# wildsonbbl/gnnepcsaft

Hardware: AMD Instinct MI355X
Metric: molecular graphs/sec (fwd+bwd) (higher is better)
Workload: dtype f32; 1 GPU; BASELINE configs[1]: PNA hidden=128 L=6 towers=1 pre=2 post=4, 4096 graphs/GPU (81920 atoms, 163840 directed bonds), fwd+loss+bwd incl. CSR packing; graphs_per_gpu=4096, parallelism=dp1, hip_graph=False, launch=auto, grad_allreduce_bytes=0, grad_exchange=none (1 rank)

## Files before the change

### gnnepcsaft_amd/_lib.py

```python
from __future__ import annotations

import ctypes as C
from pathlib import Path
from typing import Dict, Optional

import torch

_LIB_PATH = Path(__file__).resolve().parent / "libgnnepcsaft_hip.so"

ABI_VERSION = 7
GNX_OK, GNX_E_INVALID, GNX_E_HIP, GNX_E_RANGE, GNX_E_WORKSPACE = 0, -1, -2, -3, -4
OPT_GEMM_SPLIT, OPT_WGRAD_WGS, OPT_EMBED_BWD_MFMA, OPT_STD_BWD_CENTERED, OPT_GEMM_PIPE, OPT_WGRAD_PIPE, OPT_GEMM_AS, \
    OPT_GEMM_WS_FAST, OPT_GEMM_TILE_ROWS, OPT_GEMM_MID = range(10)
GEMM_RELU, GEMM_ACCUMULATE, GEMM_B_TRANS, GEMM_SPLIT_ONLY, GEMM_PRESPLIT = 1, 2, 4, 8, 16
POOL_ADD, POOL_MEAN, POOL_MAX = 0, 1, 2
K_NONE, K_PNA_AGG_FWD, K_PNA_AGG_BWD, K_GEMM_WS, K_GEMM_WGRAD, K_GINE_AGG_FWD, K_GINE_AGG_BWD, K_EDGE_COMBINE_FWD, \
    K_EDGE_COMBINE_BWD, K_BN_FWD, K_BN_BWD, K_GEMM_TILED, K_GEMM_SMALL, K_GEMM_WGRAD_BATCHED, K_KEY_SEGMENT_SUM, \
    K_EMBED, K_PNA_EDGE_FWD, K_PNA_EDGE_BWD, K_ATTN_FWD, K_ATTN_BWD, K_PCSAFT_RHO, K_PCSAFT_VP, \
    K_PCSAFT_MIX_STATE, K_PCSAFT_MIX_RHO = range(24)
K_COUNT = 24
KERNEL_GROUPS = {K_PNA_AGG_FWD: "pna_aggregate_fwd", K_PNA_AGG_BWD: "pna_aggregate_bwd", K_GEMM_WS: "gemm_weights_stationary",
                 K_GEMM_WGRAD: "weight_gradient", K_GINE_AGG_FWD: "gine_aggregate_fwd", K_GINE_AGG_BWD: "gine_aggregate_bwd",
                 K_EDGE_COMBINE_FWD: "edge_combine_fwd", K_EDGE_COMBINE_BWD: "edge_combine_bwd", K_BN_FWD: "batchnorm_fwd",
                 K_BN_BWD: "batchnorm_bwd", K_GEMM_TILED: "gemm_tiled", K_GEMM_SMALL: "gemm_small",
                 K_GEMM_WGRAD_BATCHED: "weight_gradient_batched", K_KEY_SEGMENT_SUM: "key_segment_sum", K_EMBED: "embedding",
                 K_PNA_EDGE_FWD: "pna_edge_fused_fwd", K_PNA_EDGE_BWD: "pna_edge_fused_bwd",
                 K_ATTN_FWD: "transformer_attn_fwd", K_ATTN_BWD: "transformer_attn_bwd",
                 K_PCSAFT_RHO: "pcsaft_density", K_PCSAFT_VP: "pcsaft_vapor_pressure",
                 K_PCSAFT_MIX_STATE: "pcsaft_mix_state", K_PCSAFT_MIX_RHO: "pcsaft_mix_density"}


class GnxError(RuntimeError):
    def __init__(self, status: int, msg: str):
        super().__init__(f"gnx status {status}: {msg}")
        self.status = status


class GemmSeg(C.Structure):
    _fields_ = [("a", C.c_void_p), ("lda", C.c_int64), ("rowscale", C.c_void_p), ("b", C.c_void_p),
                ("ldb", C.c_int64), ("k", C.c_int32), ("_pad", C.c_int32)]


class WgradProb(C.Structure):
    _fields_ = [("dC", C.c_void_p), ("lddc", C.c_int64), ("A", C.c_void_p), ("lda", C.c_int64),
                ("rowscale", C.c_void_p), ("dW", C.c_void_p), ("lddw", C.c_int64), ("dbias", C.c_void_p),
                ("M", C.c_int64), ("N", C.c_int32), ("K", C.c_int32)]


_vp, _i32, _i64, _f32, _sz = C.c_void_p, C.c_int32, C.c_int64, C.c_float, C.c_size_t

PNA_MAX_LAYERS, PNA_MAX_TOWERS = 8, 8
PNA_BWD_DEFER_SMALL, PNA_BWD_LAST_OF_PASS = 1, 2


class PnaFwdArgs(C.Structure):
    _fields_ = [("N", _i64), ("E", _i64), ("T", _i32), ("F", _i32), ("pre_layers", _i32), ("post_layers", _i32),
                ("D", _i32), ("merged", _i32),
                ("rowptr", _vp), ("src", _vp), ("dst", _vp), ("code", _vp), ("dperm", _vp), ("tiles", _vp), ("ntiles", _vp),
                ("max_tiles", _i64), ("x", _vp), ("Te", _vp), ("weff", _vp * PNA_MAX_TOWERS), ("Wm", _vp), ("bm", _vp),
                ("params", C.POINTER(_vp)), ("P", _vp), ("Q", _vp), ("A", _vp), ("hs", _vp * PNA_MAX_LAYERS),
                ("zs", _vp * PNA_MAX_LAYERS), ("ws", _vp), ("ws_bytes", _sz), ("out", _vp), ("etile_info", _vp),
                ("etile_w", _i32), ("tile_rows", _i32)]


class PnaBwdArgs(C.Structure):
    _fields_ = [("N", _i64), ("E", _i64), ("T", _i32), ("F", _i32), ("pre_layers", _i32), ("post_layers", _i32),
                ("R", _i32), ("D", _i32), ("avg_deg_log", _f32), ("merged", _i32), ("acc_first", _i32),
                ("use_side_streams", _i32), ("n_h", _i32), ("n_z", _i32),
                ("rowptr", _vp), ("colptr", _vp), ("cpos", _vp), ("code", _vp), ("code_pos", _vp), ("dperm", _vp),
                ("tiles", _vp), ("ntiles", _vp), ("chunks", _vp), ("nchunks", _vp),
                ("max_tiles", _i64), ("max_chunks", _i64),
                ("x", _vp), ("BE", _vp), ("EE", _vp), ("A", _vp),
                ("hs", _vp * PNA_MAX_LAYERS), ("zs", _vp * PNA_MAX_LAYERS), ("weff", _vp * PNA_MAX_TOWERS), ("Wm", _vp),
                ("params", C.POINTER(_vp)), ("grads", C.POINTER(_vp)), ("dout", _vp),
                ("gbuf", _vp * PNA_MAX_LAYERS), ("dA", _vp), ("gebuf", _vp * PNA_MAX_LAYERS), ("dP", _vp), ("dQ", _vp),
                ("dTe", _vp), ("dEE", _vp), ("dWm", _vp), ("dbm", _vp), ("dWeff", _vp), ("ws", _vp), ("ws_bytes", _sz),
                ("acc_buf", _vp), ("dx", _vp), ("flags", _i32), ("etile_w", _i32), ("etile_info", _vp)]


class PnaFinishArgs(C.Structure):
    _fields_ = [("L", _i32), ("T", _i32), ("F", _i32), ("pre_layers", _i32), ("post_layers", _i32), ("R", _i32), ("D", _i32),
                ("merged", _i32), ("use_side_streams", _i32), ("_pad", _i32),
                ("BE", _vp), ("acc_buf", _vp), ("ones", _vp), ("avg_deg_log", C.POINTER(_f32)),
                ("params", C.POINTER(_vp)), ("grads", C.POINTER(_vp)), ("EE", C.POINTER(_vp)), ("dTe", C.POINTER(_vp)),
                ("dEE", C.POINTER(_vp)), ("dWm", C.POINTER(_vp)), ("dbm", C.POINTER(_vp)), ("dWeff", C.POINTER(_vp))]


class SmallProb(C.Structure):
    _fields_ = [("A", _vp), ("lda", _i64), ("B", _vp), ("ldb", _i64), ("bias", _vp), ("C", _vp), ("ldc", _i64),
                ("M", _i32), ("N", _i32), ("K", _i32), ("flags", _i32)]


SB_A_TRANS, SB_B_TRANS, SB_ACCUMULATE, SB_ATOMIC, SB_RELU = 1, 2, 4, 8, 16

SIGNATURES = {
    "gnx_create": (_i32, [C.POINTER(_vp), _i32]),
    "gnx_destroy": (_i32, [_vp]),
    "gnx_set_stream": (_i32, [_vp, _vp]),
    "gnx_last_error": (C.c_char_p, []),
    "gnx_abi_version": (_i32, []),
    "gnx_set_option": (_i32, [_vp, _i32, _i32]),
    "gnx_get_option": (_i32, [_vp, _i32, C.POINTER(_i32)]),
    "gnx_prof_begin": (_i32, [_vp, C.c_uint32]),
    "gnx_prof_read": (_i32, [_vp, _i32, C.POINTER(_i64), C.POINTER(C.c_double), C.POINTER(C.c_double),
                             C.POINTER(C.c_double), C.POINTER(C.c_double)]),
    "gnx_prof_end": (_i32, [_vp]),
    "gnx_pack_csr_workspace_bytes": (_sz, [_i64, _i64]),
    "gnx_pack_csr": (_i32, [_vp, _vp, _i64, _i64, _vp, _vp, _vp, _vp, _vp, _vp, _vp, _sz]),
    "gnx_feature_code": (_i32, [_vp, _vp, _i64, _i32, C.POINTER(_i32), _vp, _vp, _vp, _sz]),
    "gnx_graph_ptr": (_i32, [_vp, _vp, _i64, _i64, _vp, _vp, _sz]),
    "gnx_degree_scalers": (_i32, [_vp, _vp, _i64, _f32, _vp, _vp]),
    "gnx_embed_sum_fwd": (_i32, [_vp, _vp, _i64, _i32, C.POINTER(_i32), _vp, _i32, _vp]),
    "gnx_table_scatter_workspace_bytes": (_sz, [_i64, _i32, _i32]),
    "gnx_embed_sum_bwd": (_i32, [_vp, _vp, _i64, _i32, C.POINTER(_i32), _i32, _vp, _i32, _vp, _vp, _sz]),
    "gnx_check_range": (_i32, [_vp]),
    "gnx_collate_ptr": (_i32, [_vp, _vp, _vp, _i64, _vp, _i64, _vp, _vp]),
    "gnx_collate_gather": (_i32, [_vp, _vp, _vp, _i64, _vp, _vp, _vp, _i64, _vp, _i64, _vp, _vp, _i64, _i64, _vp, _vp,
                                  _vp, _vp]),
    "gnx_collate_rows": (_i32, [_vp, _vp, _i64, _vp, _i64, _i32, _i32, _vp]),
    "gnx_gemm_workspace_bytes": (_sz, [_vp, _i32, C.POINTER(GemmSeg), C.POINTER(_i64), _i32, _i64, _i32, _vp, _i32,
                                       _i32]),
    "gnx_gemm": (_i32, [_vp, _i32, C.POINTER(GemmSeg), _i64, _i32, _vp, _vp, _i64, _vp, _i64, _i32, _vp, _sz]),
    "gnx_gemm_wgrad": (_i32, [_vp, _vp, _i64, _vp, _i64, _vp, _i64, _i32, _i32, _vp, _i64, _vp]),
    "gnx_gemm_wgrad_batched": (_i32, [_vp, _i32, C.POINTER(WgradProb)]),
    "gnx_degree_max": (_i32, [_vp, _vp, _i64, C.POINTER(_i32)]),
    "gnx_degree_classes_workspace_bytes": (_sz, [_i64, _i32]),
    "gnx_degree_classes": (_i32, [_vp, _vp, _i64, _i32, _vp, _vp, _vp, _sz]),
    "gnx_class_tiles": (_i32, [_vp, _vp, _i32, _i32, _vp, _vp]),
    "gnx_gemm_grouped": (_i32, [_vp, _i32, C.POINTER(GemmSeg), C.POINTER(_i64), _i32, _i64, _i32, _vp, _vp, _i64, _vp,
                                _i64, _i32, _vp, _vp, _vp, _i64, _vp, _sz]),
    "gnx_gemm_tile_rows": (_i32, [_vp, _i64, _i32]),
    "gnx_gemm_grouped_rows": (_i32, [_vp, _i32, C.POINTER(GemmSeg), C.POINTER(_i64), _i32, _i64, _i32, _vp, _vp, _i64, _vp,
                                     _i64, _i32, _vp, _vp, _vp, _i64, _vp, _sz, _i32]),
    "gnx_gemm_wgrad_grouped": (_i32, [_vp, _vp, _i64, _vp, _i64, _i64, _i32, _i32, _vp, _i64, _i64, _vp, _vp, _vp,
                                      _i64]),
    "gnx_pna_weff": (_i32, [_vp, _vp, _i64, _i32, _i32, _f32, _vp]),
    "gnx_pna_weff_bwd": (_i32, [_vp, _vp, _i32, _i32, _f32, _vp, _i64]),
    "gnx_group_by_small_key": (_i32, [_vp, _vp, _i64, _i32, _vp, _vp, _vp, _sz]),
    "gnx_key_segment_sum": (_i32, [_vp, _vp, _vp, _vp, _i64, _i32, _vp]),
    "gnx_edge_combine_fwd": (_i32, [_vp, _vp, _vp, _vp, _vp, _vp, _vp, _i64, _i32, _i32, _vp]),
    "gnx_edge_combine_bwd": (_i32, [_vp, _vp, _vp, _vp, _vp, _vp, _i64, _i64, _i32, _i32, _vp, _vp, _vp, _vp, _sz]),
    "gnx_pna_aggregate_fwd": (_i32, [_vp, _vp, _vp, _i64, _i64, _i32, _i32, _vp]),
    "gnx_pna_aggregate_bwd": (_i32, [_vp, _vp, _vp, _vp, _vp, _i64, _i64, _i32, _i32, _vp]),
    "gnx_edge_tiles_count": (_i32, [_i64, _i32]),
    "gnx_edge_tiles": (_i32, [_vp, _vp, _i64, _i64, _i32, _vp]),
    "gnx_pna_edge_fwd": (_i32, [_vp, _vp, _vp, _vp, _vp, _vp, _vp, _vp, _vp, _i32, _i64, _i64, _i32, _i32, C.POINTER(_vp),
                                C.POINTER(_vp), _vp, _vp, _vp]),
    "gnx_pna_edge_bwd": (_i32, [_vp, _vp, _vp, _vp, _vp, _vp, _i32, _i64, _i64, _i32, _i32, _i32, C.POINTER(_vp), _vp, _vp,
                                _vp]),
    "gnx_gine_aggregate_fwd": (_i32, [_vp, _vp, _vp, _vp, _vp, _vp, _i64, _i64, _i32, _f32, _vp]),
    "gnx_gine_aggregate_bwd": (_i32, [_vp, _vp, _vp, _vp, _vp, _vp, _vp, _vp, _vp, _vp, _i64, _i64, _i32, _i32, _f32,
                                      _vp, _vp]),
    "gnx_gine_dle": (_i32, [_vp, _vp, _vp, _vp, _vp, _vp, _vp, _vp, _i64, _i32, _i32, _vp]),
    "gnx_transformer_attn_fwd": (_i32, [_vp, _vp, _vp, _vp, _vp, _vp, _i64, _i64, _i32, _i32, _f32, C.c_uint64,
                                        C.c_uint64, _vp, _vp, _vp]),
    "gnx_transformer_attn_bwd": (_i32, [_vp, _vp, _vp, _vp, _vp, _vp, _vp, _vp, _vp, _vp, _vp, _vp, _i64, _i64, _i32,
                                        _i32, _i32, _f32, C.c_uint64, C.c_uint64, _vp, _vp, _vp]),
    "gnx_transformer_attn_dle": (_i32, [_vp, _vp, _vp, _vp, _vp, _vp, _vp, _i64, _i32, _i32, _i32, _vp]),
    "gnx_pcsaft_density": (_i32, [_vp, _vp, _i64, _vp, _vp, _vp, _i64, _vp, _vp]),
    "gnx_pcsaft_vapor_pressure": (_i32, [_vp, _vp, _i64, _vp, _vp, _i64, _vp, _vp, _vp, _vp]),
    "gnx_pcsaft_mix_state": (_i32, [_vp, _vp, _i64, _vp, _vp, _vp, _i64, _i32, _vp, _vp, _vp, _vp, _i64, _vp, _vp, _vp,
                                    _vp]),
    "gnx_pcsaft_mix_density": (_i32, [_vp, _vp, _i64, _vp, _vp, _vp, _i64, _i32, _vp, _vp, _vp, _vp, _i64, _vp, _vp]),
    "gnx_segment_pool_fwd": (_i32, [_vp, _vp, _vp, _i64, _i32, _i32, _vp]),
    "gnx_segment_pool_bwd": (_i32, [_vp, _vp, _vp, _vp, _vp, _i64, _i32, _i32, _vp]),
    "gnx_batchnorm_workspace_bytes": (_sz, [_i64, _i32]),
    "gnx_batchnorm_fwd": (_i32, [_vp, _vp, _i64, _i32, _vp, _vp, _vp, _vp, _vp, _f32, _f32, _i32, _i32, _vp, _vp, _vp,
                                 _vp, _sz]),
    "gnx_batchnorm_bwd": (_i32, [_vp, _vp, _vp, _vp, _i64, _i32, _vp, _vp, _vp, _i32, _vp, _vp, _vp, _vp, _sz]),
    "gnx_dropout": (_i32, [_vp, _vp, _i64, _f32, C.c_uint64, C.c_uint64, _vp]),
    "gnx_huber_ape": (_i32, [_vp, _vp, _vp, _i64, _f32, _vp, _vp]),
    "gnx_adamw_amsgrad": (_i32, [_vp, _vp, _vp, _vp, _vp, _vp, _i64, _f32, _f32, _f32, _f32, _f32, _i64]),
    "gnx_sgd": (_i32, [_vp, _vp, _vp, _i64, _f32]),
    "gnx_pna_weight_only": (_i32, [_vp, _vp, _i32, _i32, _i32, _i32, _i32, _i32, _f32, C.POINTER(_vp), _i32, _vp, _vp,
                                   C.POINTER(_vp), _vp, _vp]),
    "gnx_pna_conv_fwd": (_i32, [_vp, C.POINTER(PnaFwdArgs)]),
    "gnx_pna_weight_only_all": (_i32, [_vp, _i32, _vp, _i32, _i32, _i32, _i32, _i32, _i32, C.POINTER(_f32), C.POINTER(_vp),
                                       _i32, C.POINTER(_vp), C.POINTER(_vp), C.POINTER(_vp), C.POINTER(_vp), C.POINTER(_vp)]),
    "gnx_pna_stack_finish": (_i32, [_vp, C.POINTER(PnaFinishArgs)]),
    "gnx_gemm_small_batched": (_i32, [_vp, _i32, C.POINTER(SmallProb)]),
    "gnx_pna_weff_batched": (_i32, [_vp, _i32, C.POINTER(_vp), _i64, _i32, _i32, C.POINTER(_f32), C.POINTER(_vp)]),
    "gnx_pna_weff_bwd_batched": (_i32, [_vp, _i32, C.POINTER(_vp), _i32, _i32, C.POINTER(_f32), C.POINTER(_vp), _i64]),
    "gnx_pna_conv_bwd_workspace_bytes": (_sz, [_i32, _i32, _i32]),
    "gnx_pna_conv_bwd": (_i32, [_vp, C.POINTER(PnaBwdArgs)]),
    "gnx_fill": (_i32, [_vp, _vp, _i64, _f32]),
    "gnx_scale": (_i32, [_vp, _vp, _i64, _f32]),
    "gnx_axpy": (_i32, [_vp, _vp, _vp, _i64, _f32]),
    "gnx_side_stream": (_i32, [_vp, C.POINTER(_vp)]),
    "gnx_side_begin": (_i32, [_vp]),
    "gnx_side_end": (_i32, [_vp]),
    "gnx_side_join": (_i32, [_vp]),
    "gnx_side_stream_n": (_i32, [_vp, _i32, C.POINTER(_vp)]),
    "gnx_side_begin_n": (_i32, [_vp, _i32]),
    "gnx_side_join_n": (_i32, [_vp, _i32]),
    "gnx_clip_rows": (_i32, [_vp, _vp, _i64, _i32, _vp, _vp, _vp]),
}

_lib: Optional[C.CDLL] = None
_handles: Dict[int, int] = {}


def lib_path() -> Path:
    return _LIB_PATH


def load() -> C.CDLL:
    global _lib
    if _lib is not None:
        return _lib
    if not _LIB_PATH.exists():
        raise ImportError(f"{_LIB_PATH} is missing: build it with `python -m gnnepcsaft_amd.build` "
                          "(hipcc --offload-arch=gfx950). There is no CPU fallback.")
    lib = C.CDLL(str(_LIB_PATH))
    for name, (res, args) in SIGNATURES.items():
        fn = getattr(lib, name)
        fn.restype = res
        fn.argtypes = args
    if lib.gnx_abi_version() != ABI_VERSION:
        raise ImportError(f"ABI version mismatch: library {lib.gnx_abi_version()} != binding {ABI_VERSION}")
    _lib = lib
    return lib


def last_error() -> str:
    return load().gnx_last_error().decode(errors="replace")


def check(status: int) -> None:
    if status != GNX_OK:
        raise GnxError(status, last_error())


_bound_stream: dict = {}
try:
    _raw_stream = torch._C._cuda_getCurrentRawStream
except AttributeError:
    def _raw_stream(idx: int) -> int:
        return torch.cuda.current_stream(idx).cuda_stream


def handle(device: torch.device) -> int:
    if device.type != "cuda":
        raise GnxError(GNX_E_INVALID, f"gnnepcsaft_amd kernels need a HIP device tensor, got {device}; there is no CPU "
                                      "fallback")
    idx = device.index if device.index is not None else torch.cuda.current_device()
    lib = load()
    h = _handles.get(idx)
    if h is None:
        out = _vp()
        check(lib.gnx_create(C.byref(out), idx))
        h = out.value
        _handles[idx] = h
    stream = _raw_stream(idx)
    if _bound_stream.get(idx) != stream:
        check(lib.gnx_set_stream(h, stream))
        _bound_stream[idx] = stream
    return h
```

### gnnepcsaft_amd/csrc/gnx_pack.hip

```cpp
#include "gnx_common.hpp"

#define SCAN_ITEMS 4
#define SCAN_BLOCK 256
#define SCAN_TILE (SCAN_ITEMS * SCAN_BLOCK)

__global__ void __launch_bounds__(SCAN_BLOCK) k_scan_tile(const int* __restrict__ in, int* __restrict__ out,
                                                          int* __restrict__ sums, int64_t n) {
  __shared__ int s[SCAN_BLOCK];
  int64_t base = (int64_t)blockIdx.x * SCAN_TILE + (int64_t)threadIdx.x * SCAN_ITEMS;
  int v[SCAN_ITEMS];
  int t = 0;
#pragma unroll
  for (int i = 0; i < SCAN_ITEMS; ++i) {
    v[i] = (base + i < n) ? in[base + i] : 0;
    t += v[i];
  }
  s[threadIdx.x] = t;
  __syncthreads();
  for (int off = 1; off < SCAN_BLOCK; off <<= 1) {
    int add = (threadIdx.x >= off) ? s[threadIdx.x - off] : 0;
    __syncthreads();
    s[threadIdx.x] += add;
    __syncthreads();
  }
  int excl = s[threadIdx.x] - t;
#pragma unroll
  for (int i = 0; i < SCAN_ITEMS; ++i) {
    if (base + i < n) out[base + i] = excl;
    excl += v[i];
  }
  if (threadIdx.x == SCAN_BLOCK - 1) sums[blockIdx.x] = s[SCAN_BLOCK - 1];
}

__global__ void k_scan_add(int* __restrict__ out, const int* __restrict__ offs, int64_t n) {
  int64_t i = (int64_t)blockIdx.x * SCAN_TILE + threadIdx.x;
  int o = offs[blockIdx.x];
  for (int k = 0; k < SCAN_ITEMS; ++k, i += SCAN_BLOCK)
    if (i < n) out[i] += o;
}

__global__ void k_set_total(int* __restrict__ out, const int* __restrict__ in, int64_t n) {
  if (threadIdx.x == 0 && blockIdx.x == 0) out[n] = (n > 0) ? out[n - 1] + in[n - 1] : 0;
}

static int32_t exclusive_scan(gnx_handle* h, const int* in, int* out, int64_t n, int* ws, bool write_total) {
  if (n > 0) {
    int64_t blocks = gnx_cdiv(n, SCAN_TILE);
    hipLaunchKernelGGL(k_scan_tile, dim3((unsigned)blocks), dim3(SCAN_BLOCK), 0, h->stream, in, out, ws, n);
    GNX_LAUNCH_CHECK();
    if (blocks > 1) {
      int* sums_scanned = ws + blocks + 1;
      int32_t st = exclusive_scan(h, ws, sums_scanned, blocks, sums_scanned + blocks + 1, false);
      if (st != GNX_OK) return st;
      hipLaunchKernelGGL(k_scan_add, dim3((unsigned)blocks), dim3(SCAN_BLOCK), 0, h->stream, out, sums_scanned, n);
      GNX_LAUNCH_CHECK();
    }
  }
  if (write_total) {
    hipLaunchKernelGGL(k_set_total, dim3(1), dim3(64), 0, h->stream, out, in, n);
    GNX_LAUNCH_CHECK();
  }
  return GNX_OK;
}

static size_t scan_ws_ints_total(int64_t n) {
  size_t tot = 0;
  int64_t m = n;
  while (m > 1) {
    int64_t b = gnx_cdiv(m, SCAN_TILE);
    tot += 2 * ((size_t)b + 1);
    m = b;
  }
  return tot + 16;
}

__global__ void k_convert_edges(const int64_t* __restrict__ ei, int64_t E, int64_t N, int* __restrict__ src0,
                                int* __restrict__ dst0, int* __restrict__ flag) {
  int64_t e = (int64_t)blockIdx.x * blockDim.x + threadIdx.x;
  if (e >= E) return;
  int64_t s = ei[e], d = ei[E + e];
  bool bad = (s < 0) | (s >= N) | (d < 0) | (d >= N);
  if (bad) {
    atomicOr(flag, 1);
    s = 0;
    d = 0;
  }
  src0[e] = (int)s;
  dst0[e] = (int)d;
}

__global__ void k_count_keys(const int* __restrict__ key, int64_t E, int* __restrict__ counts) {
  int64_t e = (int64_t)blockIdx.x * blockDim.x + threadIdx.x;
  if (e < E) atomicAdd(&counts[key[e]], 1);
}

__global__ void k_fill_groups(const int* __restrict__ key, int64_t E, const int* __restrict__ ptr,
                              int* __restrict__ cursor, int* __restrict__ items) {
  int64_t e = (int64_t)blockIdx.x * blockDim.x + threadIdx.x;
  if (e >= E) return;
  int k = key[e];
  int pos = ptr[k] + atomicAdd(&cursor[k], 1);
  items[pos] = (int)e;
}

__global__ void k_sort_groups(const int* __restrict__ ptr, int64_t N, int* __restrict__ items) {
  int64_t i = (int64_t)blockIdx.x * blockDim.x + threadIdx.x;
  if (i >= N) return;
  int b = ptr[i], e = ptr[i + 1];
  for (int a = b + 1; a < e; ++a) {
    int v = items[a];
    int c = a - 1;
    while (c >= b && items[c] > v) {
      items[c + 1] = items[c];
      --c;
    }
    items[c + 1] = v;
  }
}

__global__ void k_gather_endpoints(const int* __restrict__ perm, const int* __restrict__ src0,
                                   const int* __restrict__ dst0, int64_t E, int* __restrict__ src,
                                   int* __restrict__ dst) {
  int64_t p = (int64_t)blockIdx.x * blockDim.x + threadIdx.x;
  if (p >= E) return;
  int e = perm[p];
  src[p] = src0[e];
  dst[p] = dst0[e];
}

static int32_t group_by_key(gnx_handle* h, const int* key, int64_t E, int64_t N, int* ptr, int* items, int* cursor,
                            int* scan_ws) {
  gnx_zero_ints(h, cursor, N > 0 ? N : 1);
  if (E > 0) {
    hipLaunchKernelGGL(k_count_keys, dim3((unsigned)gnx_cdiv(E, 256)), dim3(256), 0, h->stream, key, E, cursor);
    GNX_LAUNCH_CHECK();
  }
  int32_t st = exclusive_scan(h, cursor, ptr, N, scan_ws, true);
  if (st != GNX_OK) return st;
  gnx_zero_ints(h, cursor, N > 0 ? N : 1);
  if (E > 0) {
    hipLaunchKernelGGL(k_fill_groups, dim3((unsigned)gnx_cdiv(E, 256)), dim3(256), 0, h->stream, key, E, ptr, cursor,
                       items);
    GNX_LAUNCH_CHECK();
    hipLaunchKernelGGL(k_sort_groups, dim3((unsigned)gnx_cdiv(N, 256)), dim3(256), 0, h->stream, ptr, N, items);
    GNX_LAUNCH_CHECK();
  }
  return GNX_OK;
}

extern "C" size_t gnx_pack_csr_workspace_bytes(int64_t N, int64_t E) {
  if (N < 0) N = 0;
  if (E < 0) E = 0;
  size_t ints = 2 * (size_t)E + (size_t)N + 1 + scan_ws_ints_total(N) + 64;
  return ints * sizeof(int);
}

extern "C" int32_t gnx_pack_csr(gnx_handle* h, const int64_t* edge_index, int64_t E, int64_t N, int32_t* rowptr,
                                int32_t* perm, int32_t* src, int32_t* dst, int32_t* colptr, int32_t* cpos, void* ws,
                                size_t ws_bytes) {
  GNX_CHECK_ARG(h != nullptr, "gnx_pack_csr: handle is NULL");
  GNX_CHECK_ARG(N >= 0 && E >= 0 && N < (1ll << 31) - 1 && E < (1ll << 31) - 1, "gnx_pack_csr: N=%lld E=%lld out of int32 range",
                (long long)N, (long long)E);
  GNX_CHECK_ARG(rowptr && colptr, "gnx_pack_csr: rowptr/colptr NULL");
  GNX_CHECK_ARG(E == 0 || (edge_index && perm && src && dst && cpos), "gnx_pack_csr: NULL edge array with E>0");
  if (ws_bytes < gnx_pack_csr_workspace_bytes(N, E) || (!ws && ws_bytes)) {
    gnx_set_error("gnx_pack_csr: workspace %zu < %zu", ws_bytes, gnx_pack_csr_workspace_bytes(N, E));
    return GNX_E_WORKSPACE;
  }
  GNX_CHECK_ARG(ws != nullptr, "gnx_pack_csr: workspace is NULL");
  int* w = reinterpret_cast<int*>(ws);
  int* src0 = w;
  int* dst0 = src0 + E;
  int* cursor = dst0 + E;
  int* scan_ws = cursor + N + 1;
  if (E > 0) {
    hipLaunchKernelGGL(k_convert_edges, dim3((unsigned)gnx_cdiv(E, 256)), dim3(256), 0, h->stream, edge_index, E, N,
                       src0, dst0, h->d_flag);
    GNX_LAUNCH_CHECK();
  }
  int32_t st = group_by_key(h, dst0, E, N, rowptr, perm, cursor, scan_ws);
  if (st != GNX_OK) return st;
  if (E > 0) {
    hipLaunchKernelGGL(k_gather_endpoints, dim3((unsigned)gnx_cdiv(E, 256)), dim3(256), 0, h->stream, perm, src0,
                       dst0, E, src, dst);
    GNX_LAUNCH_CHECK();
  }
  return group_by_key(h, src, E, N, colptr, cpos, cursor, scan_ws);
}

struct dims_t {
  int d[16];
};

__global__ void k_feature_code(const int64_t* __restrict__ feat, int64_t rows, int K, dims_t dims,
                               const int* __restrict__ perm, int* __restrict__ code, int* __restrict__ flag) {
  int64_t p = (int64_t)blockIdx.x * blockDim.x + threadIdx.x;
  if (p >= rows) return;
  int64_t r = perm ? perm[p] : p;
  int c = 0;
  bool bad = false;
  for (int k = 0; k < K; ++k) {
    int64_t f = feat[r * K + k];
    if (f < 0 || f >= dims.d[k]) {
      bad = true;
      f = 0;
    }
    c = c * dims.d[k] + (int)f;
  }
  if (bad) atomicOr(flag, 2);
  code[p] = c;
}

extern "C" int32_t gnx_feature_code(gnx_handle* h, const int64_t* feat, int64_t rows, int32_t K, const int32_t* dims,
                                    const int32_t* perm, int32_t* code, void* ws, size_t ws_bytes) {
  (void)ws;
  (void)ws_bytes;
  GNX_CHECK_ARG(h && dims && K > 0 && K <= 16 && rows >= 0, "gnx_feature_code: bad argument");
  GNX_CHECK_ARG(rows == 0 || (feat && code), "gnx_feature_code: NULL array with rows>0");
  dims_t d;
  int64_t prod = 1;
  for (int k = 0; k < 16; ++k) d.d[k] = (k < K) ? dims[k] : 1;
  for (int k = 0; k < K; ++k) {
    GNX_CHECK_ARG(dims[k] > 0, "gnx_feature_code: dims[%d] <= 0", k);
    prod *= dims[k];
  }
  GNX_CHECK_ARG(prod < (1ll << 31), "gnx_feature_code: code space overflows int32");
  if (rows > 0) {
    hipLaunchKernelGGL(k_feature_code, dim3((unsigned)gnx_cdiv(rows, 256)), dim3(256), 0, h->stream, feat, rows, (int)K,
                       d, perm, code, h->d_flag);
    GNX_LAUNCH_CHECK();
  }
  return GNX_OK;
}

__global__ void k_graph_ptr(const int64_t* __restrict__ batch, int64_t N, int64_t B, int* __restrict__ ptr,
                            int* __restrict__ flag) {
  int64_t n = (int64_t)blockIdx.x * blockDim.x + threadIdx.x;
  if (n > N) return;
  int64_t prev = (n == 0) ? -1 : batch[n - 1];
  int64_t cur = (n == N) ? B : batch[n];
  if (n < N && (cur < 0 || cur >= B)) {
    atomicOr(flag, 4);
    return;
  }
  if (cur < prev) {
    atomicOr(flag, 8);
    return;
  }
  for (int64_t g = prev + 1; g <= cur; ++g) ptr[g] = (int)n;
}

extern "C" int32_t gnx_graph_ptr(gnx_handle* h, const int64_t* batch, int64_t N, int64_t B, int32_t* graph_ptr,
                                 void* ws, size_t ws_bytes) {
  (void)ws;
  (void)ws_bytes;
  GNX_CHECK_ARG(h && graph_ptr && N >= 0 && B >= 0 && (batch || N == 0), "gnx_graph_ptr: bad argument");
  hipLaunchKernelGGL(k_graph_ptr, dim3((unsigned)gnx_cdiv(N + 1, 256)), dim3(256), 0, h->stream, batch, N, B,
                     graph_ptr, h->d_flag);
  GNX_LAUNCH_CHECK();
  return GNX_OK;
}

__global__ void k_degree_scalers(const int* __restrict__ rowptr, int64_t N, float avg_log, float* __restrict__ amp,
                                 float* __restrict__ att) {
  int64_t n = (int64_t)blockIdx.x * blockDim.x + threadIdx.x;
  if (n >= N) return;
  float d = (float)(rowptr[n + 1] - rowptr[n]);
  amp[n] = logf(d + 1.0f) / avg_log;
  att[n] = avg_log / logf(fmaxf(d, 1.0f) + 1.0f);
}

extern "C" int32_t gnx_degree_scalers(gnx_handle* h, const int32_t* rowptr, int64_t N, float avg_deg_log, float* amp,
                                      float* att) {
  GNX_CHECK_ARG(h && N >= 0 && (N == 0 || (rowptr && amp && att)), "gnx_degree_scalers: bad argument");
  if (N == 0) return GNX_OK;
  hipLaunchKernelGGL(k_degree_scalers, dim3((unsigned)gnx_cdiv(N, 256)), dim3(256), 0, h->stream, rowptr, N,
                     avg_deg_log, amp, att);
  GNX_LAUNCH_CHECK();
  return GNX_OK;
}

struct weff_batch_args {
  const float* W[GNX_SMALL_BATCH];
  float* out[GNX_SMALL_BATCH];
  float avg_log[GNX_SMALL_BATCH];
  int64_t ldw;
  int F, D;
};

__global__ void k_pna_weff_batched(weff_batch_args a) {
  const int b = blockIdx.y;
  const int F = a.F;
  int64_t i = (int64_t)blockIdx.x * blockDim.x + threadIdx.x;
  int64_t per = (int64_t)F * 4 * F;
  if (i >= per * a.D) return;
  int d = (int)(i / per);
  int o = (int)((i % per) / (4 * F)), j = (int)(i % (4 * F));
  float dd = (float)d;
  float amp = logf(dd + 1.0f) / a.avg_log[b];
  float att = a.avg_log[b] / logf(fmaxf(dd, 1.0f) + 1.0f);
  const float* w = a.W[b] + (int64_t)o * a.ldw;
  a.out[b][i] = w[F + j] + amp * w[5 * F + j] + att * w[9 * F + j];
}

struct weff_bwd_batch_args {
  const float* dWeff[GNX_SMALL_BATCH];
  float* dW[GNX_SMALL_BATCH];
  float avg_log[GNX_SMALL_BATCH];
  int64_t lddw;
  int F, D;
};

__global__ void k_pna_weff_bwd_batched(weff_bwd_batch_args a) {
  const int b = blockIdx.y;
  const int F = a.F;
  int64_t i = (int64_t)blockIdx.x * blockDim.x + threadIdx.x;
  int64_t per = (int64_t)F * 4 * F;
  if (i >= per) return;
  int o = (int)(i / (4 * F)), j = (int)(i % (4 * F));
  float s1 = 0.f, s2 = 0.f, s3 = 0.f;
  const float avg_log = a.avg_log[b];
  const float* dWeff = a.dWeff[b];
  for (int d = 0; d < a.D; ++d) {
    float dd = (float)d;
    float amp = logf(dd + 1.0f) / avg_log;
    float att = avg_log / logf(fmaxf(dd, 1.0f) + 1.0f);
    float v = dWeff[(int64_t)d * per + i];
    s1 += v;
    s2 += amp * v;
    s3 += att * v;
  }
  float* w = a.dW[b] + (int64_t)o * a.lddw;
  w[F + j] += s1;
  w[5 * F + j] += s2;
  w[9 * F + j] += s3;
}

extern "C" int32_t gnx_pna_weff_bwd_batched(gnx_handle* h, int32_t n, const float* const* dWeff, int32_t F, int32_t D,
                                            const float* avg_deg_log, float* const* dW, int64_t lddw) {
  GNX_CHECK_ARG(h && dWeff && dW && avg_deg_log && n >= 0 && F > 0 && D > 0 && lddw >= 13 * F,
                "gnx_pna_weff_bwd_batched: bad argument");
  const int64_t cnt = (int64_t)F * 4 * F;
  for (int32_t i0 = 0; i0 < n; i0 += GNX_SMALL_BATCH) {
    weff_bwd_batch_args a;
    const int m = n - i0 < GNX_SMALL_BATCH ? n - i0 : GNX_SMALL_BATCH;
    for (int i = 0; i < GNX_SMALL_BATCH; ++i) {
      const int k = i < m ? i0 + i : i0;
      a.dWeff[i] = dWeff[k];
      a.dW[i] = dW[k];
      a.avg_log[i] = avg_deg_log[k];
      GNX_CHECK_ARG(a.dWeff[i] && a.dW[i], "gnx_pna_weff_bwd_batched: NULL pointer at %d", k);
    }
    a.lddw = lddw;
    a.F = F;
    a.D = D;
    hipLaunchKernelGGL(k_pna_weff_bwd_batched, dim3((unsigned)gnx_cdiv(cnt, 256), (unsigned)m), dim3(256), 0, h->stream, a);
    GNX_LAUNCH_CHECK();
  }
  return GNX_OK;
}

extern "C" int32_t gnx_pna_weff_batched(gnx_handle* h, int32_t n, const float* const* W, int64_t ldw, int32_t F, int32_t D,
                                        const float* avg_deg_log, float* const* Weff) {
  GNX_CHECK_ARG(h && W && Weff && avg_deg_log && n >= 0 && F > 0 && D > 0 && ldw >= 13 * F, "gnx_pna_weff_batched: bad argument");
  const int64_t cnt = (int64_t)F * 4 * F * D;
  for (int32_t i0 = 0; i0 < n; i0 += GNX_SMALL_BATCH) {
    weff_batch_args a;
    const int m = n - i0 < GNX_SMALL_BATCH ? n - i0 : GNX_SMALL_BATCH;
    for (int i = 0; i < GNX_SMALL_BATCH; ++i) {
      const int k = i < m ? i0 + i : i0;
      a.W[i] = W[k];
      a.out[i] = Weff[k];
      a.avg_log[i] = avg_deg_log[k];
      GNX_CHECK_ARG(a.W[i] && a.out[i], "gnx_pna_weff_batched: NULL pointer at %d", k);
    }
    a.ldw = ldw;
    a.F = F;
    a.D = D;
    hipLaunchKernelGGL(k_pna_weff_batched, dim3((unsigned)gnx_cdiv(cnt, 256), (unsigned)m), dim3(256), 0, h->stream, a);
    GNX_LAUNCH_CHECK();
  }
  return GNX_OK;
}

extern "C" int32_t gnx_pna_weff(gnx_handle* h, const float* W, int64_t ldw, int32_t F, int32_t D, float avg_deg_log,
                                float* Weff) {
  GNX_CHECK_ARG(h && W && Weff && F > 0 && D > 0 && ldw >= 13 * F, "gnx_pna_weff: bad argument");
  return gnx_pna_weff_batched(h, 1, &W, ldw, F, D, &avg_deg_log, &Weff);
}

extern "C" int32_t gnx_pna_weff_bwd(gnx_handle* h, const float* dWeff, int32_t F, int32_t D, float avg_deg_log,
                                    float* dW, int64_t lddw) {
  GNX_CHECK_ARG(h && dWeff && dW && F > 0 && D > 0 && lddw >= 13 * F, "gnx_pna_weff_bwd: bad argument");
  return gnx_pna_weff_bwd_batched(h, 1, &dWeff, F, D, &avg_deg_log, &dW, lddw);
}

__global__ void k_degree_max(const int* __restrict__ rowptr, int64_t N, int* __restrict__ out) {
  int64_t n = (int64_t)blockIdx.x * blockDim.x + threadIdx.x;
  int d = (n < N) ? rowptr[n + 1] - rowptr[n] : 0;
  for (int off = 32; off > 0; off >>= 1) d = max(d, __shfl_xor(d, off));
  if ((threadIdx.x & 63) == 0) atomicMax(out, d);
}

extern "C" int32_t gnx_degree_max(gnx_handle* h, const int32_t* rowptr, int64_t N, int32_t* max_degree_host) {
  GNX_CHECK_ARG(h && max_degree_host && N >= 0 && (N == 0 || rowptr), "gnx_degree_max: bad argument");
  int* d_out = h->d_flag + 8;
  gnx_zero_ints(h, d_out, 1);
  if (N > 0) {
    hipLaunchKernelGGL(k_degree_max, dim3((unsigned)gnx_cdiv(N, 256)), dim3(256), 0, h->stream, rowptr, N, d_out);
    GNX_LAUNCH_CHECK();
  }
  int v = 0;
  GNX_HIP(hipMemcpyAsync(&v, d_out, sizeof(int), hipMemcpyDeviceToHost, h->stream));
  GNX_HIP(hipStreamSynchronize(h->stream));
  *max_degree_host = v;
  return GNX_OK;
}

#define DC_BLOCK 256
#define DC_MAX_CLASSES 64

__global__ void __launch_bounds__(DC_BLOCK) k_dc_hist(const int* __restrict__ rowptr, const int* __restrict__ keys,
                                                       int64_t N, int D, int nblocks, int* __restrict__ blockhist,
                                                       int* __restrict__ flag) {
  __shared__ int hist[DC_MAX_CLASSES];
  if (threadIdx.x < DC_MAX_CLASSES) hist[threadIdx.x] = 0;
  __syncthreads();
  int64_t n = (int64_t)blockIdx.x * DC_BLOCK + threadIdx.x;
  if (n < N) {
    int d = keys ? keys[n] : rowptr[n + 1] - rowptr[n];
    if (d < 0) d = 0;
    if (d >= D) {
      atomicOr(flag, 32);
      d = D - 1;
    }
    atomicAdd(&hist[d], 1);
  }
  __syncthreads();
  if (threadIdx.x < D) blockhist[threadIdx.x * nblocks + blockIdx.x] = hist[threadIdx.x];
}

__global__ void __launch_bounds__(DC_BLOCK) k_dc_fill(const int* __restrict__ rowptr, const int* __restrict__ keys,
                                                       int64_t N, int D, int nblocks,
                                                       const int* __restrict__ blockoff, int* __restrict__ dperm,
                                                       int* __restrict__ cls_ptr) {
  __shared__ int degs[DC_BLOCK];
  int64_t n = (int64_t)blockIdx.x * DC_BLOCK + threadIdx.x;
  int d = -1;
  if (n < N) {
    d = keys ? keys[n] : rowptr[n + 1] - rowptr[n];
    if (d < 0) d = 0;
    if (d >= D) d = D - 1;
  }
  degs[threadIdx.x] = d;
  __syncthreads();
  if (n < N) {
    int rank = 0;
    for (int t = 0; t < (int)threadIdx.x; ++t) rank += (degs[t] == d) ? 1 : 0;
    dperm[blockoff[d * nblocks + blockIdx.x] + rank] = (int)n;
  }
  if (blockIdx.x == 0 && (int)threadIdx.x <= D)
    cls_ptr[threadIdx.x] = ((int)threadIdx.x == D) ? (int)N : blockoff[threadIdx.x * nblocks];
}

extern "C" size_t gnx_degree_classes_workspace_bytes(int64_t N, int32_t D) {
  if (N < 0) N = 0;
  int64_t nblocks = gnx_cdiv(N > 0 ? N : 1, DC_BLOCK);
  size_t ints = 2 * (size_t)(D * nblocks + 1) + scan_ws_ints_total(D * nblocks) + 64;
  return ints * sizeof(int);
}

extern "C" int32_t gnx_degree_classes(gnx_handle* h, const int32_t* rowptr, int64_t N, int32_t D, int32_t* dperm,
                                      int32_t* cls_ptr, void* ws, size_t ws_bytes) {
  GNX_CHECK_ARG(h && rowptr && cls_ptr && N >= 0 && D >= 1 && D <= DC_MAX_CLASSES && (N == 0 || dperm),
                "gnx_degree_classes: bad argument (D must be in [1,%d])", DC_MAX_CLASSES);
  if (ws_bytes < gnx_degree_classes_workspace_bytes(N, D) || !ws) {
    gnx_set_error("gnx_degree_classes: workspace %zu < %zu", ws_bytes, gnx_degree_classes_workspace_bytes(N, D));
    return GNX_E_WORKSPACE;
  }
  int nblocks = (int)gnx_cdiv(N > 0 ? N : 1, DC_BLOCK);
  int* blockhist = reinterpret_cast<int*>(ws);
  int* blockoff = blockhist + (size_t)D * nblocks + 1;
  int* scan_ws = blockoff + (size_t)D * nblocks + 1;
  hipLaunchKernelGGL(k_dc_hist, dim3(nblocks), dim3(DC_BLOCK), 0, h->stream, rowptr, (const int*)nullptr, N, (int)D,
                     nblocks, blockhist, h->d_flag);
  GNX_LAUNCH_CHECK();
  int32_t st = exclusive_scan(h, blockhist, blockoff, (int64_t)D * nblocks, scan_ws, false);
  if (st != GNX_OK) return st;
  hipLaunchKernelGGL(k_dc_fill, dim3(nblocks), dim3(DC_BLOCK), 0, h->stream, rowptr, (const int*)nullptr, N, (int)D,
                     nblocks, blockoff, dperm, cls_ptr);
  GNX_LAUNCH_CHECK();
  return GNX_OK;
}

extern "C" int32_t gnx_group_by_small_key(gnx_handle* h, const int32_t* keys, int64_t E, int32_t R, int32_t* pos,
                                          int32_t* ptr, void* ws, size_t ws_bytes) {
  GNX_CHECK_ARG(h && ptr && E >= 0 && R >= 1 && R <= DC_MAX_CLASSES && (E == 0 || (keys && pos)),
                "gnx_group_by_small_key: bad argument (R must be in [1,%d])", DC_MAX_CLASSES);
  if (ws_bytes < gnx_degree_classes_workspace_bytes(E, R) || !ws) {
    gnx_set_error("gnx_group_by_small_key: workspace %zu < %zu", ws_bytes, gnx_degree_classes_workspace_bytes(E, R));
    return GNX_E_WORKSPACE;
  }
  int nblocks = (int)gnx_cdiv(E > 0 ? E : 1, DC_BLOCK);
  int* blockhist = reinterpret_cast<int*>(ws);
  int* blockoff = blockhist + (size_t)R * nblocks + 1;
  int* scan_ws = blockoff + (size_t)R * nblocks + 1;
  hipLaunchKernelGGL(k_dc_hist, dim3(nblocks), dim3(DC_BLOCK), 0, h->stream, (const int*)nullptr, keys, E, (int)R,
                     nblocks, blockhist, h->d_flag);
  GNX_LAUNCH_CHECK();
  int32_t st = exclusive_scan(h, blockhist, blockoff, (int64_t)R * nblocks, scan_ws, false);
  if (st != GNX_OK) return st;
  hipLaunchKernelGGL(k_dc_fill, dim3(nblocks), dim3(DC_BLOCK), 0, h->stream, (const int*)nullptr, keys, E, (int)R,
                     nblocks, blockoff, pos, ptr);
  GNX_LAUNCH_CHECK();
  return GNX_OK;
}

__global__ void __launch_bounds__(256) k_class_tiles(const int* __restrict__ cls_ptr, int D, int tile_rows,
                                                     int* __restrict__ tile_info, int* __restrict__ ntiles) {
  int total = 0;
  for (int c = 0; c < D; ++c) total += (cls_ptr[c + 1] - cls_ptr[c] + tile_rows - 1) / tile_rows;
  if (blockIdx.x == 0 && threadIdx.x == 0) ntiles[0] = total;
  for (int t = blockIdx.x * blockDim.x + threadIdx.x; t < total; t += gridDim.x * blockDim.x) {
    int first = 0, c = 0;
    for (; c < D; ++c) {
      const int nt = (cls_ptr[c + 1] - cls_ptr[c] + tile_rows - 1) / tile_rows;
      if (t < first + nt) break;
      first += nt;
    }
    const int r = cls_ptr[c] + (t - first) * tile_rows;
    const int rows = cls_ptr[c + 1] - r;
    tile_info[3 * t + 0] = r;
    tile_info[3 * t + 1] = rows < tile_rows ? rows : tile_rows;
    tile_info[3 * t + 2] = c;
  }
}

extern "C" int32_t gnx_class_tiles(gnx_handle* h, const int32_t* cls_ptr, int32_t D, int32_t tile_rows,
                                   int32_t* tile_info, int32_t* ntiles) {
  GNX_CHECK_ARG(h && cls_ptr && tile_info && ntiles && D >= 1 && tile_rows > 0, "gnx_class_tiles: bad argument");
  hipLaunchKernelGGL(k_class_tiles, dim3(16), dim3(256), 0, h->stream, cls_ptr, (int)D, (int)tile_rows, tile_info, ntiles);
  GNX_LAUNCH_CHECK();
  return GNX_OK;
}
```

### gnnepcsaft_amd/functional.py

```python
from __future__ import annotations

from typing import Optional, Sequence

import torch

from . import ops
from .ops import GraphPack


_GRAD_IN_PLACE = False
_USE_DEGREE_CLASSES = True
_NATIVE_LAYER_BWD = True
_FUSED_EDGE = True
_BATCH_WEIGHT_ONLY = True


def set_grad_in_place(enabled: bool) -> None:
    global _GRAD_IN_PLACE
    _GRAD_IN_PLACE = bool(enabled)


def grad_in_place_enabled() -> bool:
    return _GRAD_IN_PLACE


def set_degree_classes(enabled: bool) -> None:
    global _USE_DEGREE_CLASSES
    _USE_DEGREE_CLASSES = bool(enabled)


def degree_classes_enabled() -> bool:
    return _USE_DEGREE_CLASSES


def set_native_layer_backward(enabled: bool) -> None:
    global _NATIVE_LAYER_BWD
    _NATIVE_LAYER_BWD = bool(enabled)


def set_fused_edge(enabled: bool) -> None:
    global _FUSED_EDGE
    _FUSED_EDGE = bool(enabled)


def set_batch_weight_only(enabled: bool) -> None:
    global _BATCH_WEIGHT_ONLY
    _BATCH_WEIGHT_ONLY = bool(enabled)


def batch_weight_only_enabled() -> bool:
    return _BATCH_WEIGHT_ONLY


def grad_sinks(params: Sequence[torch.Tensor]) -> tuple:
    if not _GRAD_IN_PLACE:
        return tuple(None for _ in params)
    out = []
    for p in params:
        g = p.grad
        ok = g is not None and g.dtype == torch.float32 and g.is_contiguous() and g.shape == p.shape and \
            g.device == p.device
        out.append(g if ok else None)
    return tuple(out)


def _tower_slices(T: int, F: int):
    return [None] if T == 1 else [slice(t * F, (t + 1) * F) for t in range(T)]


def _cols(t: torch.Tensor, sl_t):
    return t if sl_t is None else t[:, sl_t]


def _empty(rows: int, cols: int, like: torch.Tensor) -> torch.Tensor:
    return torch.empty(rows, cols, dtype=torch.float32, device=like.device)


def _zeros_like(t: torch.Tensor) -> torch.Tensor:
    return ops.zeros(*t.shape, device=t.device)


def adjacent_rows(tensors: Sequence[torch.Tensor]) -> Optional[torch.Tensor]:
    t0 = tensors[0]
    if t0.dim() != 2 or t0.dtype is not torch.float32 or not t0.is_contiguous():
        return None
    H = t0.size(1)
    ptr, rows = t0.data_ptr(), 0
    for t in tensors:
        if t.dim() != 2 or t.size(1) != H or t.dtype is not torch.float32 or not t.is_contiguous() or \
                t.device != t0.device or t.data_ptr() != ptr + rows * H * 4:
            return None
        rows += t.size(0)
    if t0.untyped_storage().nbytes() - t0.storage_offset() * 4 < rows * H * 4:
        return None
    return torch.as_strided(t0.detach(), (rows, H), (H, 1))


class EmbedSumFn(torch.autograd.Function):

    @staticmethod
    def forward(ctx, idx, offsets, *weights):
        table = adjacent_rows(weights)
        if table is None:
            table = torch.cat([w.detach() for w in weights], dim=0)
        ctx.save_for_backward(idx)
        ctx.offsets = tuple(offsets)
        ctx.sinks = grad_sinks(weights)
        return ops.embed_sum_fwd(idx, table, offsets)

    @staticmethod
    def backward(ctx, dout):
        (idx,) = ctx.saved_tensors
        sinks, offs = ctx.sinks, ctx.offsets
        if all(g is not None for g in sinks):
            gtable = adjacent_rows(sinks)
            if gtable is not None:
                ops.embed_sum_bwd(idx, offs, dout.contiguous(), out=gtable)
                return (None, None) + (None,) * len(sinks)
        dtable = ops.embed_sum_bwd(idx, offs, dout.contiguous())
        return (None, None) + tuple(dtable[offs[k]:offs[k + 1]] for k in range(len(sinks)))


class DropoutFn(torch.autograd.Function):

    @staticmethod
    def forward(ctx, x, p, seed, offset):
        ctx.key = (float(p), int(seed), int(offset))
        return ops.dropout(x, p, seed, offset)

    @staticmethod
    def backward(ctx, dy):
        p, seed, offset = ctx.key
        return ops.dropout(dy, p, seed, offset), None, None, None


class LinearFn(torch.autograd.Function):

    @staticmethod
    def forward(ctx, x, weight, bias):
        x = x.contiguous()
        ctx.save_for_backward(x, weight)
        ctx.has_bias = bias is not None
        ctx.sinks = grad_sinks([weight] + ([bias] if bias is not None else []))
        y = _empty(x.size(0), weight.size(0), x)
        return ops.gemm([(x, None, weight)], y, bias=bias)

    @staticmethod
    def backward(ctx, dy):
        x, weight = ctx.saved_tensors
        dy = dy.contiguous()
        sw = ctx.sinks[0]
        sb = ctx.sinks[1] if ctx.has_bias else None
        dw = sw if sw is not None else _zeros_like(weight)
        db = None
        if ctx.has_bias:
            db = sb if sb is not None else ops.zeros(weight.size(0), device=dy.device)
        ops.gemm_wgrad(dy, x, dw, dbias=db)
        dx = None
        if ctx.needs_input_grad[0]:
            dx = ops.gemm([(dy, None, weight)], _empty(x.size(0), x.size(1), x), b_trans=False)
        ops.finish_backward(dy.device, sw is not None and (sb is not None or not ctx.has_bias), ctx.sinks)
        return dx, (None if sw is not None else dw), (None if (sb is not None or not ctx.has_bias) else db)


class BatchNormFn(torch.autograd.Function):

    @staticmethod
    def forward(ctx, x, gamma, beta, running_mean, running_var, momentum, eps, training, relu, nbt=None):
        x = x.contiguous()
        y, mean, rstd = ops.batchnorm_fwd(x, gamma, beta, running_mean, running_var, momentum, eps, training, relu,
                                          num_batches_tracked=nbt)
        ctx.save_for_backward(x, y, gamma, mean, rstd)
        ctx.relu, ctx.training = relu, training
        ctx.sinks = grad_sinks([gamma, beta])
        return y

    @staticmethod
    def backward(ctx, dy):
        x, y, gamma, mean, rstd = ctx.saved_tensors
        if not ctx.training:
            raise NotImplementedError("BatchNorm backward in eval mode is not on the reference's training path")
        sg, sb = ctx.sinks
        dx, dgamma, dbeta = ops.batchnorm_bwd(dy.contiguous(), x, y, gamma, mean, rstd, ctx.relu, dgamma=sg, dbeta=sb)
        return dx, (None if sg is not None else dgamma), (None if sb is not None else dbeta), None, None, None, None, \
            None, None, None


class SegmentPoolFn(torch.autograd.Function):

    @staticmethod
    def forward(ctx, x, ptr, B, mode):
        x = x.contiguous()
        out = ops.segment_pool_fwd(x, ptr, B, mode)
        ctx.save_for_backward(x, out, ptr)
        ctx.B, ctx.mode = B, mode
        return out

    @staticmethod
    def backward(ctx, dout):
        x, out, ptr = ctx.saved_tensors
        return ops.segment_pool_bwd(dout.contiguous(), x, out, ptr, ctx.B, ctx.mode), None, None, None


class HuberAPEFn(torch.autograd.Function):

    @staticmethod
    def forward(ctx, pred, target, delta):
        out2, dpred = ops.huber_ape(pred, target, delta, need_grad=True)
        ctx.save_for_backward(dpred)
        ctx.mark_non_differentiable(out2)
        return out2[0], out2

    @staticmethod
    def backward(ctx, dloss, _):
        (dpred,) = ctx.saved_tensors
        return dpred * dloss, None, None


def _pna_weight_only(BE, T, F, pre_layers, post_layers, avg_deg_log, params, D):
    R, H = BE.size(0), T * F
    merged = post_layers > 1
    if _NATIVE_LAYER_BWD and BE.is_cuda and T <= 8:
        import ctypes as C
        from . import _lib
        EE, Te = _empty(R, F, BE), _empty(R, H, BE)
        weffs = [torch.empty(D, F, 4 * F, dtype=torch.float32, device=BE.device) for _ in range(T)] if D > 0 else []
        Wm = _empty(H, H, BE) if merged else None
        bm = torch.empty(H, dtype=torch.float32, device=BE.device) if merged else None
        n = len(params)
        parr = (C.c_void_p * n)(*[p.data_ptr() for p in params])
        warr = (C.c_void_p * max(T, 1))(*[w.data_ptr() for w in weffs]) if weffs else None
        ops.check(_lib.load().gnx_pna_weight_only(
            _lib.handle(BE.device), BE.data_ptr(), R, T, F, pre_layers, post_layers, D, float(avg_deg_log),
            C.cast(parr, C.POINTER(C.c_void_p)), int(merged), EE.data_ptr(), Te.data_ptr(),
            None if warr is None else C.cast(warr, C.POINTER(C.c_void_p)), None if Wm is None else Wm.data_ptr(),
            None if bm is None else bm.data_ptr()))
        return EE, Te, weffs, Wm, bm
    enc_w, enc_b, lin_w, lin_b = params[:4]
    per = 2 * (pre_layers + post_layers)
    sl = _tower_slices(T, F)
    EE = ops.gemm([(BE, None, enc_w)], _empty(R, F, BE), bias=enc_b)
    Te = _empty(R, H, BE)
    weffs, last = [], []
    for t in range(T):
        W0, b0 = params[4 + t * per], params[4 + t * per + 1]
        ops.gemm([(EE, None, W0[:, 2 * F:3 * F])], _cols(Te, sl[t]), bias=b0)
        Wp = params[4 + t * per + 2 * pre_layers]
        if D > 0:
            weffs.append(ops.pna_weff(Wp, F, D, avg_deg_log))
        k = 4 + t * per + 2 * (pre_layers + post_layers - 1)
        last.append((params[k], params[k + 1]))
    Wm = bm = None
    if merged:
        Wm, bm = _merge_last_post_with_lin(lin_w, lin_b, last, sl, BE)
    return EE, Te, weffs, Wm, bm


class BondGradAccumulator:

    def __init__(self, R: int, H: int, device, depth: int):
        self.buf = torch.empty(R, H, dtype=torch.float32, device=device)
        self.depth = depth
        self.encoder = None
        self.defer = False
        self.slab = None
        self.deferred = []

    def layer_slab(self, layer_index: int, R: int, H: int, F: int, T: int, D: int, device):
        per = R * H + R * F + H * H + H + T * D * F * 4 * F
        if self.slab is None:
            self.slab = ops.zeros(R * H + self.depth * per, device=device)
            self.buf = self.slab[:R * H].view(R, H)
        o = R * H + layer_index * per
        out = []
        for n in (R * H, R * F, H * H, H, T * D * F * 4 * F):
            out.append(self.slab[o:o + n])
            o += n
        return out

    def finish_deferred(self, device) -> None:
        if not self.deferred:
            return
        import ctypes as C
        from . import _lib
        d0 = self.deferred[0]
        L = len(self.deferred)
        T, F, pre, post, R, D, merged = d0["T"], d0["F"], d0["pre"], d0["post"], d0["R"], d0["D"], d0["merged"]
        np_ = 4 + T * 2 * (pre + post)
        a = _lib.PnaFinishArgs()
        a.L, a.T, a.F, a.pre_layers, a.post_layers, a.R, a.D, a.merged = L, T, F, pre, post, R, D, int(merged)
        a.use_side_streams = int(ops.wgrad_stream_enabled())
        ones = ops.ones_vector(device, max(R, 1))
        a.BE, a.acc_buf, a.ones = d0["BE"].data_ptr(), self.buf.data_ptr(), ones.data_ptr()
        avg = (C.c_float * L)(*[d["avg"] for d in self.deferred])
        vp = C.c_void_p
        params = (vp * (L * np_))(*[p.data_ptr() for d in self.deferred for p in d["params"]])
        grads = (vp * (L * np_))(*[g.data_ptr() for d in self.deferred for g in d["sinks"]])
        EE = (vp * L)(*[d["EE"].data_ptr() for d in self.deferred])
        dTe = (vp * L)(*[d["dTe"].data_ptr() for d in self.deferred])
        dEE = (vp * L)(*[d["dEE"].data_ptr() for d in self.deferred])
        dWm = (vp * L)(*[d["dWm"].data_ptr() for d in self.deferred])
        dbm = (vp * L)(*[d["dbm"].data_ptr() for d in self.deferred])
        per_w = D * F * 4 * F
        dWeff = (vp * (L * T))(*[d["dWeff"].data_ptr() + 4 * t * per_w for d in self.deferred for t in range(T)])
        a.avg_deg_log = C.cast(avg, C.POINTER(C.c_float))
        for name, arr in (("params", params), ("grads", grads), ("EE", EE), ("dTe", dTe), ("dEE", dEE), ("dWm", dWm),
                          ("dbm", dbm), ("dWeff", dWeff)):
            setattr(a, name, C.cast(arr, C.POINTER(vp)))
        ops.check(_lib.load().gnx_pna_stack_finish(_lib.handle(device), C.byref(a)))
        ops.keep_until_join(device, [self.slab, ones] + [t for d in self.deferred for t in (d["BE"], d["EE"], *d["params"], *d["sinks"])])
        self.deferred = []

    def first_in_backward(self, layer_index: int) -> bool:
        return layer_index == self.depth - 1

    def handoff(self, device) -> Optional[torch.Tensor]:
        if self.encoder is not None:
            idx, offs, weights = self.encoder
            sinks = grad_sinks(weights)
            gtable = adjacent_rows(sinks) if all(g is not None for g in sinks) else None
            if gtable is not None:
                buf = self.buf
                ops.run_on_second_side_stream(buf, [buf, idx, gtable], lambda: ops.embed_sum_bwd(idx, offs, buf, out=gtable))
                return None
        ops.join_side_stream(device, 1)
        return self.buf


class WeightOnlyAhead:

    def __init__(self, BE, T, F, pre_layers, post_layers, avg_deg_log, params, D):
        self.device = BE.device
        box = []
        ops.run_after_wgrads(BE, (), lambda: box.append(_pna_weight_only(BE, T, F, pre_layers, post_layers, avg_deg_log,
                                                                        params, D)))
        self.value = box[0]

    def wait(self):
        ops.join_side_stream(self.device)
        return self.value


class WeightOnlyAll:

    def __init__(self, BE, T, F, pre_layers, post_layers, layers, D):
        import ctypes as C
        from . import _lib
        self.device = BE.device
        L, R, H = len(layers), BE.size(0), T * F
        merged = post_layers > 1
        f32 = dict(dtype=torch.float32, device=BE.device)
        EE = torch.empty(L, R, F, **f32)
        Te = torch.empty(L, R, H, **f32)
        weff = torch.empty(L, T, D, F, 4 * F, **f32) if D > 0 else None
        Wm = torch.empty(L, H, H, **f32) if merged else None
        bm = torch.empty(L, H, **f32) if merged else None
        vp = C.c_void_p
        np_ = len(layers[0][1])
        avg = (C.c_float * L)(*[float(a_) for a_, _ in layers])
        params = (vp * (L * np_))(*[p.data_ptr() for _, ps in layers for p in ps])
        ptrs = lambda t_, n: (vp * n)(*[t_[i].data_ptr() for i in range(n)]) if t_ is not None else None
        a_EE, a_Te, a_Wm, a_bm = ptrs(EE, L), ptrs(Te, L), ptrs(Wm, L), ptrs(bm, L)
        a_weff = (vp * (L * T))(*[weff[l, t].data_ptr() for l in range(L) for t in range(T)]) if weff is not None else None
        cast = lambda arr: None if arr is None else C.cast(arr, C.POINTER(vp))

        def launch():
            ops.check(_lib.load().gnx_pna_weight_only_all(
                _lib.handle(BE.device), L, BE.data_ptr(), R, T, F, pre_layers, post_layers, D,
                C.cast(avg, C.POINTER(C.c_float)), cast(params), int(merged), cast(a_EE), cast(a_Te), cast(a_weff),
                cast(a_Wm), cast(a_bm)))

        keep = [BE, EE, Te, weff, Wm, bm] + [p for _, ps in layers for p in ps]
        ops.run_after_wgrads(BE, keep, launch)
        self.values = [(EE[l], Te[l], [weff[l, t] for t in range(T)] if weff is not None else [],
                        Wm[l] if merged else None, bm[l] if merged else None) for l in range(L)]
        self._joined = False

    def get(self, l: int):
        if not self._joined:
            ops.join_side_stream(self.device)
            self._joined = True
        return self.values[l]


def _merge_last_post_with_lin(lin_w, lin_b, last, sl, like):
    H = lin_w.size(0)
    Wm, bm = _empty(H, H, like), _empty(1, H, like)
    for t, (Wt, _) in enumerate(last):
        ops.gemm([(_cols(lin_w, sl[t]), None, Wt)], _cols(Wm, sl[t]), b_trans=False)
    for t, (_, bt) in enumerate(last):
        ops.gemm([(bt.view(1, -1), None, _cols(lin_w, sl[t]))], bm, bias=lin_b if t == 0 else None, accumulate=t > 0)
    return Wm, bm.view(-1)


def _unmerge_last_post_and_lin(dWm, dbm, lin_w, d_lin_w, d_lin_b, last, last_bias, sl):
    row, col = dbm.view(1, -1), dbm.view(-1, 1)
    for t, (Wt, dWt, dbt) in enumerate(last):
        bt = last_bias[t]
        ops.gemm([(_cols(dWm, sl[t]), None, Wt)], _cols(d_lin_w, sl[t]), accumulate=True)
        ops.gemm([(col, None, bt.view(-1, 1))], _cols(d_lin_w, sl[t]), accumulate=True)
        ops.gemm_wgrad_inline(_cols(lin_w, sl[t]), _cols(dWm, sl[t]), dWt)
        ops.gemm([(row, None, _cols(lin_w, sl[t]))], dbt.view(1, -1), b_trans=False, accumulate=True)
    ops.axpy_(d_lin_b, dbm)


def _pna_forward_native(ctx, x, BE, pack, cfg, params, dc, prep):
    import ctypes as C
    from . import _lib
    T, F, pre_layers, post_layers, avg_deg_log = cfg[:5]
    EE, Te, weffs, Wm, bm = prep
    N, H = x.shape
    E, D = pack.E, dc.D
    dev = x.device
    merged = Wm is not None
    n_z = post_layers - 1 if merged else post_layers
    f32 = dict(dtype=torch.float32, device=dev)
    PQ = torch.empty(2, N, H, **f32)
    hs_all = torch.empty(pre_layers, max(E, 1), H, **f32)
    zs_all = torch.empty(max(n_z, 1), N, H, **f32)
    A = torch.empty(N, T * 4 * F, **f32)
    out = torch.empty(N, H, **f32)
    lib = _lib.load()
    ws_bytes = lib.gnx_pna_conv_bwd_workspace_bytes(T, F, D)
    ws = torch.empty(ws_bytes, dtype=torch.uint8, device=dev)
    a = _lib.PnaFwdArgs()
    a.N, a.E, a.T, a.F, a.pre_layers, a.post_layers, a.D, a.merged = N, E, T, F, pre_layers, post_layers, D, int(merged)
    a.rowptr, a.src, a.dst, a.code = pack.rowptr.data_ptr(), pack.src.data_ptr(), pack.dst.data_ptr(), pack.code.data_ptr()
    a.dperm, a.tiles, a.ntiles, a.max_tiles = dc.dperm.data_ptr(), dc.tiles_p.data_ptr(), dc.ntiles_p.data_ptr(), dc.max_tiles_p
    a.tile_rows = dc.tile_rows_p
    a.x, a.Te = x.data_ptr(), Te.data_ptr()
    for i, w in enumerate(weffs):
        a.weff[i] = w.data_ptr()
    a.Wm, a.bm = (Wm.data_ptr(), bm.data_ptr()) if merged else (None, None)
    n = len(params)
    parr = (C.c_void_p * n)(*[p.data_ptr() for p in params])
    a.params = C.cast(parr, C.POINTER(C.c_void_p))
    a.P, a.Q, a.A = PQ[0].data_ptr(), PQ[1].data_ptr(), A.data_ptr()
    hs = [hs_all[i][:E] if E != hs_all.size(1) else hs_all[i] for i in range(pre_layers)]
    zs = [zs_all[i] for i in range(n_z)]
    for i, t_ in enumerate(hs):
        a.hs[i] = t_.data_ptr()
    for i, t_ in enumerate(zs):
        a.zs[i] = t_.data_ptr()
    a.ws, a.ws_bytes, a.out = ws.data_ptr(), ws_bytes, out.data_ptr()
    etiles = pack.edge_tiles(D - 1) if (_FUSED_EDGE and pre_layers == 2) else None
    a.etile_info, a.etile_w = (etiles[0].data_ptr(), etiles[1]) if etiles is not None else (None, 0)
    ops.check(lib.gnx_pna_conv_fwd(_lib.handle(dev), C.byref(a)))
    amp, att = pack.degree_scalers(avg_deg_log)
    ctx.pack, ctx.cfg = pack, cfg[:5]
    ctx.n_h, ctx.n_z = len(hs), len(zs)
    ctx.sinks = grad_sinks(params)
    ctx.dc, ctx.weffs, ctx.Wm = dc, weffs, Wm
    ctx.save_for_backward(x, BE, EE, A, amp, att, *hs, *zs, *params)
    return out


def _pna_backward_native(ctx, dout, x, BE, EE, A, hs, zs, params, sinks, code_pos):
    import ctypes as C
    from . import _lib
    T, F, pre_layers, post_layers, avg_deg_log = ctx.cfg
    pack, dc, acc = ctx.pack, ctx.dc, ctx.bond_acc
    N, H = x.shape
    E, R, D = pack.E, BE.size(0), dc.D
    dev = x.device
    dout = dout.contiguous()
    merged = ctx.Wm is not None
    n_g = post_layers - 1 if merged else post_layers
    f32 = dict(dtype=torch.float32, device=dev)
    gbuf = torch.empty(max(n_g, 1), N, H, **f32)
    gebuf = torch.empty(pre_layers, max(E, 1), H, **f32)
    dA = torch.empty(N, T * 4 * F, **f32)
    pq = torch.empty(2, N, H, **f32)
    defer = _BATCH_WEIGHT_ONLY and acc is not None and not ops.wgrad_done_hook_set() and \
        (acc.slab is not None or acc.first_in_backward(ctx.layer_index))
    if defer:
        dTe_t, dEE_t, dWm_t, dbm_t, dWeff_t = acc.layer_slab(ctx.layer_index, R, H, F, T, D, dev)
        small = None
    else:
        small = torch.empty(R * H + R * F + H * H + H + T * D * F * 4 * F, **f32)
    dx = torch.empty(N, H, **f32)
    lib = _lib.load()
    ws_bytes = lib.gnx_pna_conv_bwd_workspace_bytes(T, F, D)
    ws = torch.empty(ws_bytes, dtype=torch.uint8, device=dev)
    a = _lib.PnaBwdArgs()
    a.N, a.E, a.T, a.F, a.pre_layers, a.post_layers, a.R, a.D = N, E, T, F, pre_layers, post_layers, R, D
    a.avg_deg_log, a.merged = float(avg_deg_log), int(merged)
    a.acc_first, a.use_side_streams = int(acc.first_in_backward(ctx.layer_index)), int(ops.wgrad_stream_enabled())
    a.n_h, a.n_z = len(hs), len(zs)
    a.rowptr, a.colptr, a.cpos, a.code = pack.rowptr.data_ptr(), pack.colptr.data_ptr(), pack.cpos.data_ptr(), pack.code.data_ptr()
    a.code_pos = None if code_pos is None else code_pos.data_ptr()
    a.dperm, a.tiles, a.ntiles = dc.dperm.data_ptr(), dc.tiles.data_ptr(), dc.ntiles.data_ptr()
    a.chunks, a.nchunks, a.max_tiles, a.max_chunks = dc.chunks.data_ptr(), dc.nchunks.data_ptr(), dc.max_tiles, dc.max_chunks
    a.x, a.BE, a.EE, a.A = x.data_ptr(), BE.data_ptr(), EE.data_ptr(), A.data_ptr()
    for i, t_ in enumerate(hs):
        a.hs[i] = t_.data_ptr()
    for i, t_ in enumerate(zs):
        a.zs[i] = t_.data_ptr()
    for i, t_ in enumerate(ctx.weffs):
        a.weff[i] = t_.data_ptr()
    a.Wm = ctx.Wm.data_ptr() if merged else None
    n = len(params)
    parr = (C.c_void_p * n)(*[p.data_ptr() for p in params])
    garr = (C.c_void_p * n)(*[g_.data_ptr() for g_ in sinks])
    a.params, a.grads, a.dout = C.cast(parr, C.POINTER(C.c_void_p)), C.cast(garr, C.POINTER(C.c_void_p)), dout.data_ptr()
    for i in range(gbuf.size(0)):
        a.gbuf[i] = gbuf[i].data_ptr()
    for i in range(pre_layers):
        a.gebuf[i] = gebuf[i].data_ptr()
    a.dA, a.dP, a.dQ = dA.data_ptr(), pq[0].data_ptr(), pq[1].data_ptr()
    if defer:
        a.dTe, a.dEE, a.dWm, a.dbm, a.dWeff = (t_.data_ptr() for t_ in (dTe_t, dEE_t, dWm_t, dbm_t, dWeff_t))
        a.flags = _lib.PNA_BWD_DEFER_SMALL
        acc.deferred.append(dict(T=T, F=F, pre=pre_layers, post=post_layers, R=R, D=D, merged=merged, avg=float(avg_deg_log),
                                 BE=BE, EE=EE, params=list(params), sinks=list(sinks), dTe=dTe_t, dEE=dEE_t, dWm=dWm_t,
                                 dbm=dbm_t, dWeff=dWeff_t))
    else:
        base, o = small.data_ptr(), 0
        a.dTe, o = base + 4 * o, o + R * H
        a.dEE, o = base + 4 * o, o + R * F
        a.dWm, o = base + 4 * o, o + H * H
        a.dbm, o = base + 4 * o, o + H
        a.dWeff = base + 4 * o
        a.flags = 0
    if ctx.layer_index == 0:
        a.flags |= _lib.PNA_BWD_LAST_OF_PASS
    a.ws, a.ws_bytes, a.acc_buf, a.dx = ws.data_ptr(), ws_bytes, acc.buf.data_ptr(), dx.data_ptr()
    etiles = pack.edge_tiles(D - 1) if (_FUSED_EDGE and pre_layers == 2) else None
    a.etile_info, a.etile_w = (etiles[0].data_ptr(), etiles[1]) if etiles is not None else (None, 0)
    ops.pna_conv_bwd(a, dev)
    ops.keep_until_join(dev, [dout, x, BE, EE, A, *hs, *zs, *ctx.weffs, ctx.Wm, gbuf, gebuf, dA, pq, small, ws, acc.buf,
                              acc.slab, *params, *sinks])
    dBE = None
    if ctx.layer_index == 0:
        acc.finish_deferred(dev)
        dBE = acc.handoff(dev)
    ops.finish_backward(dev, True, sinks)
    return (dx, dBE, None, None, *([None] * len(params)))


class PNAConvFn(torch.autograd.Function):

    @staticmethod
    def forward(ctx, x, BE, pack: GraphPack, cfg, *params):
        T, F, pre_layers, post_layers, avg_deg_log, prep = cfg[:6]
        ctx.bond_acc, ctx.layer_index = (cfg[6], cfg[7]) if len(cfg) > 6 else (None, 0)
        x = x.contiguous()
        N, H = x.shape
        E, R = pack.E, BE.size(0)
        enc_w, enc_b, lin_w, lin_b = params[:4]
        per = 2 * (pre_layers + post_layers)
        pre = [[(params[4 + t * per + 2 * i], params[4 + t * per + 2 * i + 1]) for i in range(pre_layers)]
               for t in range(T)]
        post = [[(params[4 + t * per + 2 * (pre_layers + i)], params[4 + t * per + 2 * (pre_layers + i) + 1])
                 for i in range(post_layers)] for t in range(T)]
        sl = _tower_slices(T, F)
        dc = pack.degree_classes(pack.max_degree_hint) if _USE_DEGREE_CLASSES else None
        if prep is None:
            prep = _pna_weight_only(BE, T, F, pre_layers, post_layers, avg_deg_log, params, dc.D if dc is not None else 0)
        EE, Te, weffs, Wm, bm = prep
        if _NATIVE_LAYER_BWD and dc is not None and x.is_cuda and pre_layers <= 8 and post_layers <= 8 and T <= 8:
            return _pna_forward_native(ctx, x, BE, pack, cfg, params, dc, prep)
        P, Q = _empty(N, H, x), _empty(N, H, x)
        for t in range(T):
            W0 = pre[t][0][0]
            xt = _cols(x, sl[t])
            ops.gemm([(xt, None, W0[:, 0:F])], _cols(P, sl[t]))
            ops.gemm([(xt, None, W0[:, F:2 * F])], _cols(Q, sl[t]))
        h = ops.edge_combine_fwd(P, Q, Te, pack, relu=pre_layers > 1)
        hs = [h]
        for i in range(1, pre_layers):
            hn = _empty(E, H, x)
            for t in range(T):
                Wi, bi = pre[t][i]
                ops.gemm([(_cols(h, sl[t]), None, Wi)], _cols(hn, sl[t]), bias=bi, relu=i < pre_layers - 1)
            h = hn
            hs.append(h)
        A = ops.pna_aggregate_fwd(h, pack, T, F)
        amp, att = pack.degree_scalers(avg_deg_log)
        z = _empty(N, H, x)
        for t in range(T):
            Wp, bp = post[t][0]
            At = A[:, t * 4 * F:(t + 1) * 4 * F]
            if dc is not None:
                ops.gemm_grouped([(_cols(x, sl[t]), None, Wp[:, 0:F], 0), (At, None, weffs[t][0], 4 * F * F)], _cols(z, sl[t]), dc,
                                 bias=bp, relu=post_layers > 1)
            else:
                ops.gemm([(_cols(x, sl[t]), None, Wp[:, 0:F]), (At, None, Wp[:, F:5 * F]), (At, amp, Wp[:, 5 * F:9 * F]),
                          (At, att, Wp[:, 9 * F:13 * F])], _cols(z, sl[t]), bias=bp, relu=post_layers > 1)
        zs = [z]
        merged = Wm is not None
        for i in range(1, post_layers - 1 if merged else post_layers):
            zn = _empty(N, H, x)
            for t in range(T):
                Wi, bi = post[t][i]
                ops.gemm([(_cols(z, sl[t]), None, Wi)], _cols(zn, sl[t]), bias=bi, relu=i < post_layers - 1)
            z = zn
            zs.append(z)
        if merged:
            out = ops.gemm([(z, None, Wm)], _empty(N, H, x), bias=bm)
        else:
            out = ops.gemm([(z, None, lin_w)], _empty(N, H, x), bias=lin_b)
        ctx.pack, ctx.cfg = pack, cfg[:5]
        ctx.n_h, ctx.n_z = len(hs), len(zs)
        ctx.sinks = grad_sinks(params)
        ctx.dc, ctx.weffs, ctx.Wm = dc, weffs, Wm
        ctx.save_for_backward(x, BE, EE, A, amp, att, *hs, *zs, *params)
        return out

    @staticmethod
    def backward(ctx, dout):
        T, F, pre_layers, post_layers, _ = ctx.cfg
        pack: GraphPack = ctx.pack
        saved = ctx.saved_tensors
        x, BE, EE, A, amp, att = saved[:6]
        hs = list(saved[6:6 + ctx.n_h])
        zs = list(saved[6 + ctx.n_h:6 + ctx.n_h + ctx.n_z])
        params = saved[6 + ctx.n_h + ctx.n_z:]
        N, H = x.shape
        E, R = pack.E, BE.size(0)
        enc_w, enc_b, lin_w, lin_b = params[:4]
        per = 2 * (pre_layers + post_layers)
        sinks = ctx.sinks
        if _NATIVE_LAYER_BWD and ctx.bond_acc is not None and ctx.dc is not None and x.is_cuda and \
                all(sk is not None for sk in sinks) and pre_layers <= 8 and post_layers <= 8 and T <= 8:
            code_pos = ops.bond_code_index(pack, R, H)
            if code_pos is not None or E == 0:
                return _pna_backward_native(ctx, dout, x, BE, EE, A, hs, zs, params, sinks, code_pos)
        grads = [sk if sk is not None else _zeros_like(p) for p, sk in zip(params, sinks)]
        d_enc_w, d_enc_b, d_lin_w, d_lin_b = grads[:4]

        def pidx(t, kind, i):
            return 4 + t * per + 2 * (i if kind == "pre" else pre_layers + i)

        sl = _tower_slices(T, F)
        dout = dout.contiguous()
        merged = None
        if ctx.Wm is not None:
            dWm, dbm = _zeros_like(ctx.Wm), ops.zeros(H, device=x.device)
            ops.queue_wgrad(dout, zs[-1], dWm, dbias=dbm)
            g = ops.gemm([(dout, None, ctx.Wm)], _empty(N, H, x), b_trans=False, mask=zs[-1])
            merged = (dWm, dbm)
            last_hidden = post_layers - 2
        else:
            ops.queue_wgrad(dout, zs[-1], d_lin_w, dbias=d_lin_b)
            g = ops.gemm([(dout, None, lin_w)], _empty(N, H, x), b_trans=False)
            last_hidden = post_layers - 1
        for i in range(last_hidden, 0, -1):
            a_prev = zs[i - 1]
            gn = _empty(N, H, x)
            for t in range(T):
                k = pidx(t, "post", i)
                ops.queue_wgrad(_cols(g, sl[t]), _cols(a_prev, sl[t]), grads[k], dbias=grads[k + 1])
                ops.gemm([(_cols(g, sl[t]), None, params[k])], _cols(gn, sl[t]), b_trans=False, mask=_cols(a_prev, sl[t]))
            g = gn
        dA = _empty(N, T * 4 * F, x)
        for t in range(T):
            k = pidx(t, "post", 0)
            Wp, dWp = params[k], grads[k]
            gt = _cols(g, sl[t])
            At = A[:, t * 4 * F:(t + 1) * 4 * F]
            ops.queue_wgrad(gt, _cols(x, sl[t]), dWp[:, 0:F], dbias=grads[k + 1])
            if ctx.dc is not None:
                ops.pna_post0_wgrad_classes(gt, At, ctx.dc, F, ctx.cfg[4], dWp)
                ops.gemm_grouped([(gt, None, ctx.weffs[t][0], 4 * F * F)], dA[:, t * 4 * F:(t + 1) * 4 * F], ctx.dc,
                                 b_trans=False)
            else:
                ops.queue_wgrad(gt, At, dWp[:, F:5 * F])
                ops.queue_wgrad(gt, At, dWp[:, 5 * F:9 * F], rowscale=amp)
                ops.queue_wgrad(gt, At, dWp[:, 9 * F:13 * F], rowscale=att)
                ops.gemm([(gt, None, Wp[:, F:5 * F]), (gt, amp, Wp[:, 5 * F:9 * F]), (gt, att, Wp[:, 9 * F:13 * F])],
                         dA[:, t * 4 * F:(t + 1) * 4 * F], b_trans=False)
        ge = ops.pna_aggregate_bwd(dA, hs[-1], A, pack, T, F)
        for i in range(pre_layers - 1, 0, -1):
            h_prev = hs[i - 1]
            gn = _empty(E, H, x)
            for t in range(T):
                k = pidx(t, "pre", i)
                ops.queue_wgrad(_cols(ge, sl[t]), _cols(h_prev, sl[t]), grads[k], dbias=grads[k + 1])
                ops.gemm([(_cols(ge, sl[t]), None, params[k])], _cols(gn, sl[t]), b_trans=False, mask=_cols(h_prev, sl[t]))
            ge = gn
        dP, dQ = ops.edge_combine_bwd_pq(ge, pack)
        dx = _empty(N, H, x)
        for t in range(T):
            k0 = pidx(t, "pre", 0)
            W0, dW0 = params[k0], grads[k0]
            kp = pidx(t, "post", 0)
            xt = _cols(x, sl[t])
            ops.queue_wgrad(_cols(dP, sl[t]), xt, dW0[:, 0:F])
            ops.queue_wgrad(_cols(dQ, sl[t]), xt, dW0[:, F:2 * F])
            ops.gemm([(_cols(g, sl[t]), None, params[kp][:, 0:F]), (_cols(dP, sl[t]), None, W0[:, 0:F]),
                      (_cols(dQ, sl[t]), None, W0[:, F:2 * F])], _cols(dx, sl[t]), b_trans=False)
        code_pos = ops.bond_code_index(pack, R, H)
        acc = ctx.bond_acc
        dBE_box = []
        keep = [ge, EE, BE] + ([acc.buf] if acc is not None else [])

        def bond_chain():
            dTe = ops.bond_table_grad(ge, pack, R, code_pos)
            dEE = _empty(R, F, x)
            for t in range(T):
                k0 = pidx(t, "pre", 0)
                ops.gemm_wgrad_inline(_cols(dTe, sl[t]), EE, grads[k0][:, 2 * F:3 * F], dbias=grads[k0 + 1])
                ops.gemm([(_cols(dTe, sl[t]), None, params[k0][:, 2 * F:3 * F])], dEE, b_trans=False, accumulate=t > 0)
            ops.gemm_wgrad_inline(dEE, BE, d_enc_w, dbias=d_enc_b)
            if acc is None:
                dBE_box.append(ops.gemm([(dEE, None, enc_w)], _empty(R, H, x), b_trans=False))
            else:
                if acc.first_in_backward(ctx.layer_index):
                    ops.zero_(acc.buf)
                ops.gemm([(dEE, None, enc_w)], acc.buf, b_trans=False, accumulate=True)
            keep.extend((dTe, dEE))

        if acc is None:
            bond_chain()
            dBE = dBE_box[0]
        else:
            ops.run_on_second_side_stream(ge, keep, bond_chain)
            dBE = None
            if ctx.layer_index == 0:
                dBE = acc.handoff(x.device)
        ops.flush_wgrads()
        if merged is not None:
            dWm, dbm = merged
            last = [(params[pidx(t, "post", post_layers - 1)], grads[pidx(t, "post", post_layers - 1)],
                     grads[pidx(t, "post", post_layers - 1) + 1]) for t in range(T)]
            last_bias = [params[pidx(t, "post", post_layers - 1) + 1] for t in range(T)]
            ops.run_after_wgrads(dout, (dWm, dbm, lin_w, d_lin_w, d_lin_b),
                                 lambda: _unmerge_last_post_and_lin(dWm, dbm, lin_w, d_lin_w, d_lin_b, last, last_bias, sl))
        ops.finish_backward(x.device, all(sk is not None for sk in sinks), sinks)
        return (dx, dBE, None, None, *[None if sk is not None else g_ for g_, sk in zip(grads, sinks)])


class GINEConvFn(torch.autograd.Function):

    @staticmethod
    def forward(ctx, x, BE, pack: GraphPack, eps, lin_w, lin_b, w0, b0, w2, b2, bond_acc=None, layer_index=0):
        ctx.bond_acc, ctx.layer_index = bond_acc, layer_index
        x = x.contiguous()
        N, H = x.shape
        R = BE.size(0)
        Le = ops.gemm([(BE, None, lin_w)], _empty(R, lin_w.size(0), x), bias=lin_b)
        agg = ops.gine_aggregate_fwd(x, Le, pack, eps)
        a1 = ops.gemm([(agg, None, w0)], _empty(N, w0.size(0), x), bias=b0, relu=True)
        out = ops.gemm([(a1, None, w2)], _empty(N, w2.size(0), x), bias=b2)
        ctx.pack, ctx.eps = pack, eps
        ctx.sinks = grad_sinks([lin_w, lin_b, w0, b0, w2, b2])
        ctx.save_for_backward(x, BE, Le, agg, a1, lin_w, w0, w2)
        return out

    @staticmethod
    def backward(ctx, dout):
        x, BE, Le, agg, a1, lin_w, w0, w2 = ctx.saved_tensors
        pack: GraphPack = ctx.pack
        dout = dout.contiguous()
        N, H = x.shape
        dev = dict(dtype=torch.float32, device=x.device)
        sk = ctx.sinks
        dlw = sk[0] if sk[0] is not None else _zeros_like(lin_w)
        dlb = sk[1] if sk[1] is not None else ops.zeros(lin_w.size(0), device=x.device)
        dw0 = sk[2] if sk[2] is not None else _zeros_like(w0)
        db0 = sk[3] if sk[3] is not None else ops.zeros(w0.size(0), device=x.device)
        dw2 = sk[4] if sk[4] is not None else _zeros_like(w2)
        db2 = sk[5] if sk[5] is not None else ops.zeros(w2.size(0), device=x.device)
        ops.gemm_wgrad(dout, a1, dw2, dbias=db2)
        g1 = ops.gemm([(dout, None, w2)], _empty(N, a1.size(1), x), b_trans=False, mask=a1)
        ops.gemm_wgrad(g1, agg, dw0, dbias=db0)
        dagg = ops.gemm([(g1, None, w0)], _empty(N, H, x), b_trans=False)
        acc = ctx.bond_acc
        if acc is None:
            dx, dLe = ops.gine_aggregate_bwd(dagg, x, Le, pack, ctx.eps)
            ops.gemm_wgrad(dLe, BE, dlw, dbias=dlb)
            dBE = ops.gemm([(dLe, None, lin_w)], _empty(BE.size(0), BE.size(1), x), b_trans=False)
        else:
            dx, _ = ops.gine_aggregate_bwd(dagg, x, Le, pack, ctx.eps, want_dle=False)
            code_pos = pack.code_index(Le.size(0)) if pack.E > 0 else None
            keep = [dagg, x, Le, BE, acc.buf]

            def bond_chain():
                dLe_ = ops.gine_dle(dagg, x, Le, pack, code_pos)
                ops.gemm_wgrad_inline(dLe_, BE, dlw, dbias=dlb)
                if acc.first_in_backward(ctx.layer_index):
                    ops.zero_(acc.buf)
                ops.gemm([(dLe_, None, lin_w)], acc.buf, b_trans=False, accumulate=True)
                keep.append(dLe_)

            ops.run_on_second_side_stream(dagg, keep, bond_chain)
            dBE = None
            if ctx.layer_index == 0:
                dBE = acc.handoff(x.device)
        ops.finish_backward(x.device, all(k is not None for k in sk), sk)
        outs = [None if k is not None else g_ for g_, k in zip((dlw, dlb, dw0, db0, dw2, db2), sk)]
        return (dx, dBE, None, None, *outs, None, None)


def _stacked(tensors: Sequence[torch.Tensor]) -> torch.Tensor:
    t = adjacent_rows(tensors)
    return t if t is not None else torch.cat([w.detach() for w in tensors], dim=0)


class TransformerConvFn(torch.autograd.Function):

    @staticmethod
    def forward(ctx, x, BE, pack: GraphPack, cfg, wq, bq, wk, bk, wv, bv, we, ws, bs):
        heads, p, seed, offset, bond_acc, layer_index = cfg
        x = x.contiguous()
        N, H = x.shape
        R = BE.size(0)
        Le = ops.gemm([(BE, None, we)], _empty(R, we.size(0), x))
        W4 = _stacked([wq, wk, wv, ws])
        b4 = _stacked([b.view(1, -1) for b in (bq, bk, bv, bs)])
        qkvs = ops.gemm([(x, None, W4)], _empty(N, 4 * H, x), bias=b4)
        out, alpha, _ = ops.transformer_attn_fwd(qkvs, Le, pack, heads, p, seed, offset)
        ctx.pack, ctx.key = pack, (int(heads), float(p), int(seed), int(offset))
        ctx.bond_acc, ctx.layer_index = bond_acc, layer_index
        ctx.sinks = grad_sinks([wq, bq, wk, bk, wv, bv, we, ws, bs])
        ctx.save_for_backward(x, BE, Le, qkvs, alpha, W4, we)
        return out

    @staticmethod
    def backward(ctx, dout):
        x, BE, Le, qkvs, alpha, W4, we = ctx.saved_tensors
        pack: GraphPack = ctx.pack
        heads, p, seed, offset = ctx.key
        dout = dout.contiguous()
        N, H = x.shape
        sk = ctx.sinks
        shapes = [(H, H), (H,), (H, H), (H,), (H, H), (H,), tuple(we.shape), (H, H), (H,)]
        grads = [g_ if g_ is not None else ops.zeros(*s, device=x.device) for g_, s in zip(sk, shapes)]
        acc = ctx.bond_acc
        dqkv, scratch, dLe = ops.transformer_attn_bwd(dout, qkvs, Le, alpha, pack, heads, p, seed, offset,
                                                      want_dle=acc is None)
        for t in range(3):
            ops.queue_wgrad(dqkv[:, t * H:(t + 1) * H], x, grads[2 * t], dbias=grads[2 * t + 1])
        ops.queue_wgrad(dout, x, grads[7], dbias=grads[8])
        ops.flush_wgrads()
        dx = None
        if ctx.needs_input_grad[0]:
            dx = ops.gemm([(dqkv, None, W4[:3 * H]), (dout, None, W4[3 * H:])], _empty(N, H, x), b_trans=False)
        if acc is None:
            ops.gemm_wgrad(dLe, BE, grads[6])
            dBE = ops.gemm([(dLe, None, we)], _empty(BE.size(0), BE.size(1), x), b_trans=False)
        else:
            code_pos = pack.code_index(Le.size(0)) if pack.E > 0 else None
            keep = [dout, qkvs, scratch, Le, BE, we, grads[6], acc.buf]

            def bond_chain():
                dLe_ = ops.transformer_attn_dle(dout, qkvs, scratch, Le, pack, heads, code_pos)
                ops.gemm_wgrad_inline(dLe_, BE, grads[6])
                if acc.first_in_backward(ctx.layer_index):
                    ops.zero_(acc.buf)
                ops.gemm([(dLe_, None, we)], acc.buf, b_trans=False, accumulate=True)
                keep.append(dLe_)

            ops.run_on_second_side_stream(dout, keep, bond_chain)
            dBE = None
            if ctx.layer_index == 0:
                dBE = acc.handoff(x.device)
        ops.finish_backward(x.device, all(k is not None for k in sk), sk)
        outs = [None if k is not None else g_ for g_, k in zip(grads, sk)]
        return (dx, dBE, None, None, *outs)
```

### gnnepcsaft_amd/ops.py

```python
from __future__ import annotations

import ctypes as C
import threading
from typing import List, Optional, Sequence, Tuple

import torch

from . import _lib
from ._lib import GemmSeg, check, handle

_I32 = C.c_int32


def _f32(t: torch.Tensor, name: str) -> torch.Tensor:
    if t.dtype != torch.float32:
        raise _lib.GnxError(_lib.GNX_E_INVALID, f"{name}: expected float32, got {t.dtype}")
    return t


def _mat(t: torch.Tensor, name: str) -> Tuple[int, int]:
    if t.dtype is not torch.float32:
        raise _lib.GnxError(_lib.GNX_E_INVALID, f"{name}: expected float32, got {t.dtype}")
    shape, strides = t.shape, t.stride()
    if len(shape) != 2 or (shape[1] > 1 and strides[1] != 1):
        raise _lib.GnxError(_lib.GNX_E_INVALID, f"{name}: need a 2-D view with unit column stride, got "
                                                f"shape {tuple(shape)} strides {strides}")
    ld = strides[0]
    return t.data_ptr(), (ld if ld > shape[1] else shape[1])


def _ptr(t: Optional[torch.Tensor]) -> Optional[int]:
    return None if t is None else t.data_ptr()


def _carr(vals: Sequence[int]):
    return (_I32 * len(vals))(*vals)


def zeros(*shape: int, device: torch.device) -> torch.Tensor:
    t = torch.empty(*shape, dtype=torch.float32, device=device)
    return zero_(t)


_ONES: dict = {}


def ones_vector(device: torch.device, n: int) -> torch.Tensor:
    key = device.index if device.index is not None else torch.cuda.current_device()
    t = _ONES.get(key)
    if t is None or t.numel() < n:
        t = torch.empty(max(n, 256), dtype=torch.float32, device=device)
        check(_lib.load().gnx_fill(handle(device), t.data_ptr(), t.numel(), 1.0))
        _ONES[key] = t
    return t


def zero_(t: torch.Tensor) -> torch.Tensor:
    if t.is_cuda and t.dtype is torch.float32 and t.is_contiguous():
        if t.numel():
            check(_lib.load().gnx_fill(handle(t.device), t.data_ptr(), t.numel(), 0.0))
        return t
    return t.zero_()


class GraphPack:

    __slots__ = ("N", "E", "B", "rowptr", "perm", "src", "dst", "colptr", "cpos", "code", "graph_ptr", "device",
                 "_scalers", "has_batch", "_classes", "_code_index", "max_degree_hint", "_edge_tiles")

    EDGE_TILE_ROWS = 64
    EDGE_TILE_MAX_DEG = 16

    def edge_tiles(self, max_degree: int) -> Optional[Tuple[torch.Tensor, int]]:
        if max_degree > GraphPack.EDGE_TILE_MAX_DEG or self.E == 0 or self.N == 0:
            return None
        w = GraphPack.EDGE_TILE_ROWS + 1 - max(int(max_degree), 1)
        hit = self._edge_tiles
        if hit is None or hit[1] != w:
            lib = _lib.load()
            count = lib.gnx_edge_tiles_count(self.E, w)
            info = torch.empty(2 * (count + 1), dtype=torch.int32, device=self.device)
            check(lib.gnx_edge_tiles(handle(self.device), self.rowptr.data_ptr(), self.N, self.E, w, info.data_ptr()))
            hit = self._edge_tiles = (info, w)
        return hit

    def code_index(self, R: int) -> Optional[torch.Tensor]:
        if R > 64:
            return None
        if self._code_index is None or self._code_index[0] != R:
            lib, h = _lib.load(), handle(self.device)
            pos = torch.empty(max(self.E, 1), dtype=torch.int32, device=self.device)
            ptr = torch.empty(R + 1, dtype=torch.int32, device=self.device)
            nbytes = lib.gnx_degree_classes_workspace_bytes(self.E, R)
            ws = torch.empty(nbytes, dtype=torch.uint8, device=self.device)
            check(lib.gnx_group_by_small_key(h, self.code.data_ptr(), self.E, R, pos.data_ptr(), ptr.data_ptr(),
                                             ws.data_ptr(), nbytes))
            self._code_index = (R, pos, ptr)
        return self._code_index[1]

    def degree_classes(self, max_degree_hint: Optional[int] = None) -> Optional["DegreeClasses"]:
        if self._classes is None:
            self._classes = DegreeClasses.build(self, max_degree_hint)
        return self._classes if self._classes.D <= DegreeClasses.MAX_D else None

    def degree_scalers(self, avg_deg_log: float) -> Tuple[torch.Tensor, torch.Tensor]:
        key = float(avg_deg_log)
        hit = self._scalers.get(key)
        if hit is None:
            amp = torch.empty(self.N, dtype=torch.float32, device=self.device)
            att = torch.empty(self.N, dtype=torch.float32, device=self.device)
            check(_lib.load().gnx_degree_scalers(handle(self.device), self.rowptr.data_ptr(), self.N, key,
                                                 amp.data_ptr(), att.data_ptr()))
            hit = (amp, att)
            self._scalers[key] = hit
        return hit


class DegreeClasses:
    MAX_D = 64
    GEMM_ROWS = 128
    WGRAD_ROWS = 1024

    __slots__ = ("D", "dperm", "cls_ptr", "tiles", "ntiles", "max_tiles", "chunks", "nchunks", "max_chunks",
                 "tiles_p", "ntiles_p", "max_tiles_p", "tile_rows_p")

    @staticmethod
    def build(g: "GraphPack", max_degree_hint: Optional[int] = None) -> "DegreeClasses":
        lib, h = _lib.load(), handle(g.device)
        dc = DegreeClasses()
        if max_degree_hint is None:
            mx = _I32(0)
            check(lib.gnx_degree_max(h, g.rowptr.data_ptr(), g.N, C.byref(mx)))
            dc.D = int(mx.value) + 1
        else:
            dc.D = int(max_degree_hint) + 1
        if dc.D > DegreeClasses.MAX_D:
            return dc
        i32 = dict(dtype=torch.int32, device=g.device)
        dc.dperm = torch.empty(max(g.N, 1), **i32)
        dc.cls_ptr = torch.empty(dc.D + 1, **i32)
        nbytes = lib.gnx_degree_classes_workspace_bytes(g.N, dc.D)
        ws = torch.empty(nbytes, dtype=torch.uint8, device=g.device)
        check(lib.gnx_degree_classes(h, g.rowptr.data_ptr(), g.N, dc.D, dc.dperm.data_ptr(), dc.cls_ptr.data_ptr(),
                                     ws.data_ptr(), nbytes))
        dc.max_tiles = g.N // DegreeClasses.GEMM_ROWS + dc.D
        dc.max_chunks = g.N // DegreeClasses.WGRAD_ROWS + dc.D
        dc.tiles = torch.empty(3 * dc.max_tiles, **i32)
        dc.chunks = torch.empty(3 * dc.max_chunks, **i32)
        dc.ntiles = torch.empty(1, **i32)
        dc.nchunks = torch.empty(1, **i32)
        check(lib.gnx_class_tiles(h, dc.cls_ptr.data_ptr(), dc.D, DegreeClasses.GEMM_ROWS, dc.tiles.data_ptr(),
                                  dc.ntiles.data_ptr()))
        check(lib.gnx_class_tiles(h, dc.cls_ptr.data_ptr(), dc.D, DegreeClasses.WGRAD_ROWS, dc.chunks.data_ptr(),
                                  dc.nchunks.data_ptr()))
        dc.tile_rows_p = int(lib.gnx_gemm_tile_rows(h, g.N, 128))
        if dc.tile_rows_p == DegreeClasses.GEMM_ROWS:
            dc.tiles_p, dc.ntiles_p, dc.max_tiles_p = dc.tiles, dc.ntiles, dc.max_tiles
        else:
            dc.max_tiles_p = g.N // dc.tile_rows_p + dc.D
            dc.tiles_p = torch.empty(3 * dc.max_tiles_p, **i32)
            dc.ntiles_p = torch.empty(1, **i32)
            check(lib.gnx_class_tiles(h, dc.cls_ptr.data_ptr(), dc.D, dc.tile_rows_p, dc.tiles_p.data_ptr(),
                                      dc.ntiles_p.data_ptr()))
        return dc


def set_option(device: torch.device, opt: int, value: int) -> int:
    lib, h = _lib.load(), handle(device)
    old = _I32(0)
    check(lib.gnx_get_option(h, opt, C.byref(old)))
    check(lib.gnx_set_option(h, opt, int(value)))
    return int(old.value)


def check_range(device: torch.device) -> None:
    check(_lib.load().gnx_check_range(handle(device)))


def pack_graph(edge_index: torch.Tensor, edge_attr: Optional[torch.Tensor], batch: Optional[torch.Tensor],
               num_nodes: int, num_graphs: Optional[int] = None, bond_dims: Sequence[int] = (5, 6, 2),
               validate: bool = True) -> GraphPack:
    dev = edge_index.device
    lib, h = _lib.load(), handle(dev)
    if edge_index.dtype != torch.int64 or edge_index.dim() != 2 or edge_index.size(0) != 2:
        raise _lib.GnxError(_lib.GNX_E_INVALID, f"edge_index must be int64[2,E], got {edge_index.dtype} "
                                                f"{tuple(edge_index.shape)}")
    edge_index = edge_index.contiguous()
    N, E = int(num_nodes), int(edge_index.size(1))
    i32 = dict(dtype=torch.int32, device=dev)
    g = GraphPack()
    g.N, g.E, g.device, g._scalers, g._classes, g._code_index = N, E, dev, {}, None, None
    g._edge_tiles = None
    g.max_degree_hint = None
    g.rowptr = torch.empty(N + 1, **i32)
    g.colptr = torch.empty(N + 1, **i32)
    g.perm = torch.empty(E, **i32)
    g.src = torch.empty(E, **i32)
    g.dst = torch.empty(E, **i32)
    g.cpos = torch.empty(E, **i32)
    ws_bytes = lib.gnx_pack_csr_workspace_bytes(N, E)
    ws = torch.empty(ws_bytes, dtype=torch.uint8, device=dev)
    check(lib.gnx_pack_csr(h, edge_index.data_ptr(), E, N, g.rowptr.data_ptr(), g.perm.data_ptr(), g.src.data_ptr(),
                           g.dst.data_ptr(), g.colptr.data_ptr(), g.cpos.data_ptr(), ws.data_ptr(), ws_bytes))
    g.code = torch.empty(E, **i32)
    if edge_attr is not None:
        if edge_attr.dtype != torch.int64 or edge_attr.dim() != 2 or edge_attr.size(0) != E or \
                edge_attr.size(1) != len(bond_dims):
            raise _lib.GnxError(_lib.GNX_E_INVALID, f"edge_attr must be int64[E,{len(bond_dims)}], got "
                                                    f"{edge_attr.dtype} {tuple(edge_attr.shape)}")
        edge_attr = edge_attr.contiguous()
        check(lib.gnx_feature_code(h, edge_attr.data_ptr(), E, len(bond_dims), _carr(list(bond_dims)),
                                   g.perm.data_ptr(), g.code.data_ptr(), None, 0))
    else:
        g.code.zero_()
    if batch is not None:
        if batch.dtype != torch.int64 or batch.dim() != 1 or batch.size(0) != N:
            raise _lib.GnxError(_lib.GNX_E_INVALID, f"batch must be int64[N], got {batch.dtype} {tuple(batch.shape)}")
        if num_graphs is None:
            num_graphs = int(batch.max()) + 1 if N > 0 else 0
        g.B = int(num_graphs)
        g.has_batch = True
        g.graph_ptr = torch.empty(g.B + 1, **i32)
        check(lib.gnx_graph_ptr(h, batch.contiguous().data_ptr(), N, g.B, g.graph_ptr.data_ptr(), None, 0))
    else:
        g.B = 1
        g.has_batch = False
        g.graph_ptr = torch.arange(2, **i32) * N
    if validate:
        check_range(dev)
    return g


def _i64c(t: torch.Tensor, name: str, shape: Sequence[Optional[int]]) -> torch.Tensor:
    if not isinstance(t, torch.Tensor) or t.dtype != torch.int64 or t.dim() != len(shape) or not t.is_contiguous() or \
            any(s is not None and int(d) != s for d, s in zip(t.shape, shape)):
        want = ",".join("*" if s is None else str(s) for s in shape)
        got = f"{t.dtype} {tuple(t.shape)}" if isinstance(t, torch.Tensor) else type(t).__name__
        raise _lib.GnxError(_lib.GNX_E_INVALID, f"{name}: expected contiguous int64[{want}], got {got}")
    return t


def _on(dev: torch.device, *tensors: torch.Tensor) -> None:
    for t in tensors:
        if t.device != dev:
            raise _lib.GnxError(_lib.GNX_E_INVALID, f"collate: every tensor must be on {dev}, got one on {t.device}")


def collate_ptr(node_ptr: torch.Tensor, edge_ptr: torch.Tensor, idx: torch.Tensor) -> Tuple[torch.Tensor, torch.Tensor]:
    _i64c(node_ptr, "node_ptr", (None,))
    G = node_ptr.size(0) - 1
    _i64c(edge_ptr, "edge_ptr", (G + 1,))
    _i64c(idx, "idx", (None,))
    B = idx.size(0)
    if G < 1 or B < 1:
        raise _lib.GnxError(_lib.GNX_E_INVALID, f"collate_ptr: need at least one graph and one index, got G={G} B={B}")
    dev = node_ptr.device
    _on(dev, edge_ptr, idx)
    out = torch.empty(2, B + 1, dtype=torch.int64, device=dev)
    check(_lib.load().gnx_collate_ptr(handle(dev), node_ptr.data_ptr(), edge_ptr.data_ptr(), G, idx.data_ptr(), B,
                                      out[0].data_ptr(), out[1].data_ptr()))
    return out[0], out[1]


def collate_gather(node_ptr: torch.Tensor, edge_ptr: torch.Tensor, x: torch.Tensor, edge_index: torch.Tensor,
                   edge_attr: torch.Tensor, idx: torch.Tensor, ptr: torch.Tensor, eptr: torch.Tensor, N: int, E: int
                   ) -> Tuple[torch.Tensor, torch.Tensor, torch.Tensor, torch.Tensor]:
    _i64c(node_ptr, "node_ptr", (None,))
    G = node_ptr.size(0) - 1
    _i64c(edge_ptr, "edge_ptr", (G + 1,))
    _i64c(x, "x", (None, 9))
    _i64c(edge_index, "edge_index", (2, None))
    E_src = edge_index.size(1)
    _i64c(edge_attr, "edge_attr", (E_src, 3))
    _i64c(idx, "idx", (None,))
    B = idx.size(0)
    _i64c(ptr, "ptr", (B + 1,))
    _i64c(eptr, "eptr", (B + 1,))
    N, E = int(N), int(E)
    if G < 1 or B < 1 or N < 0 or E < 0:
        raise _lib.GnxError(_lib.GNX_E_INVALID, f"collate_gather: bad sizes G={G} B={B} N={N} E={E}")
    dev = x.device
    _on(dev, node_ptr, edge_ptr, edge_index, edge_attr, idx, ptr, eptr)
    i64 = dict(dtype=torch.int64, device=dev)
    x_out, ei_out, ea_out = torch.empty(N, 9, **i64), torch.empty(2, E, **i64), torch.empty(E, 3, **i64)
    batch = torch.empty(N, **i64)
    check(_lib.load().gnx_collate_gather(handle(dev), node_ptr.data_ptr(), edge_ptr.data_ptr(), G, x.data_ptr(),
                                         edge_index.data_ptr(), edge_attr.data_ptr(), E_src, idx.data_ptr(), B,
                                         ptr.data_ptr(), eptr.data_ptr(), N, E, x_out.data_ptr(), ei_out.data_ptr(),
                                         ea_out.data_ptr(), batch.data_ptr()))
    return x_out, ei_out, ea_out, batch


def collate_rows(src: torch.Tensor, idx: torch.Tensor) -> torch.Tensor:
    if not isinstance(src, torch.Tensor) or src.dim() < 1 or not src.is_contiguous() or src.element_size() not in (4, 8):
        got = f"{src.dtype} {tuple(src.shape)}" if isinstance(src, torch.Tensor) else type(src).__name__
        raise _lib.GnxError(_lib.GNX_E_INVALID, f"collate_rows: expected a contiguous [G, ...] tensor of a 4- or 8-byte "
                                                f"dtype, got {got}")
    _i64c(idx, "idx", (None,))
    G, B = src.size(0), idx.size(0)
    if G < 1 or B < 1:
        raise _lib.GnxError(_lib.GNX_E_INVALID, f"collate_rows: need at least one row and one index, got G={G} B={B}")
    K = src.numel() // G
    _on(src.device, idx)
    dst = torch.empty((B,) + tuple(src.shape[1:]), dtype=src.dtype, device=src.device)
    check(_lib.load().gnx_collate_rows(handle(src.device), src.data_ptr(), G, idx.data_ptr(), B, src.element_size(), K,
                                       dst.data_ptr()))
    return dst


def embed_sum_fwd(idx: torch.Tensor, table: torch.Tensor, offsets: Sequence[int]) -> torch.Tensor:
    K = len(offsets) - 1
    if idx.dtype != torch.int64 or idx.dim() != 2 or idx.size(1) != K:
        raise _lib.GnxError(_lib.GNX_E_INVALID, f"embedding index must be int64[N,{K}], got {idx.dtype} "
                                                f"{tuple(idx.shape)}")
    idx = idx.contiguous()
    table = _f32(table, "table").contiguous()
    N, H = idx.size(0), table.size(1)
    out = torch.empty(N, H, dtype=torch.float32, device=table.device)
    check(_lib.load().gnx_embed_sum_fwd(handle(table.device), idx.data_ptr(), N, K, _carr(list(offsets)),
                                        table.data_ptr(), H, out.data_ptr()))
    return out


def embed_sum_bwd(idx: torch.Tensor, offsets: Sequence[int], dout: torch.Tensor,
                  out: Optional[torch.Tensor] = None) -> torch.Tensor:
    K, R = len(offsets) - 1, offsets[-1]
    dout = _f32(dout, "dout").contiguous()
    idx = idx.contiguous()
    H = dout.size(1)
    if out is not None:
        if out.shape != (R, H) or not out.is_contiguous() or out.dtype is not torch.float32:
            raise _lib.GnxError(_lib.GNX_E_INVALID, f"embed_sum_bwd: out must be contiguous fp32 [{R},{H}]")
        dtable = out
    else:
        dtable = zeros(R, H, device=dout.device)
    lib = _lib.load()
    nbytes = lib.gnx_table_scatter_workspace_bytes(idx.size(0), R, H)
    ws = torch.empty(max(nbytes, 1), dtype=torch.uint8, device=dout.device)
    check(lib.gnx_embed_sum_bwd(handle(dout.device), idx.data_ptr(), idx.size(0), K, _carr(list(offsets)), R,
                                dout.data_ptr(), H, dtable.data_ptr(), ws.data_ptr(), nbytes))
    return dtable


Seg = Tuple[torch.Tensor, Optional[torch.Tensor], torch.Tensor]


class _SegArrays(threading.local):

    def __init__(self):
        self.by_len = {n: (GemmSeg * n)() for n in range(1, 5)}


_SEG_ARRAYS = _SegArrays()


def gemm(segs: Sequence[Seg], out: torch.Tensor, *, bias: Optional[torch.Tensor] = None,
         mask: Optional[torch.Tensor] = None, relu: bool = False, accumulate: bool = False,
         b_trans: bool = True) -> torch.Tensor:
    M, N = out.shape
    if M == 0:
        return out
    cptr, ldc = _mat(out, "out")
    arr = _SEG_ARRAYS.by_len[len(segs)]
    for i, (a, rs, b) in enumerate(segs):
        ap, lda = _mat(a, "A")
        bp, ldb = _mat(b, "B")
        (am, k), (b0, b1) = a.shape, b.shape
        if am != M or (b_trans and (b0 != N or b1 != k)) or (not b_trans and (b0 != k or b1 != N)):
            raise _lib.GnxError(_lib.GNX_E_INVALID, f"gemm segment {i}: A {tuple(a.shape)} B {tuple(b.shape)} "
                                                    f"out {tuple(out.shape)} b_trans={b_trans}")
        e = arr[i]
        e.a, e.lda, e.rowscale = ap, lda, (None if rs is None else rs.data_ptr())
        e.b, e.ldb, e.k = bp, ldb, k
    flags = (_lib.GEMM_RELU if relu else 0) | (_lib.GEMM_ACCUMULATE if accumulate else 0) | \
            (_lib.GEMM_B_TRANS if b_trans else 0)
    mp, ldm = (None, 0) if mask is None else _mat(mask, "mask")
    lib, h = _lib.load(), handle(out.device)
    nbytes = lib.gnx_gemm_workspace_bytes(h, len(segs), arr, None, 1, M, N, mp, flags, 0) if M >= 4096 else 0
    ws = torch.empty(nbytes, dtype=torch.uint8, device=out.device) if nbytes else None
    check(lib.gnx_gemm(h, len(segs), arr, M, N, _ptr(bias), mp, ldm, cptr, ldc, flags, _ptr(ws), nbytes))
    return out


GSeg = Tuple[torch.Tensor, Optional[torch.Tensor], torch.Tensor, int]


def gemm_grouped(segs: Sequence[GSeg], out: torch.Tensor, dc: DegreeClasses, *, bias: Optional[torch.Tensor] = None,
                 mask: Optional[torch.Tensor] = None, relu: bool = False, b_trans: bool = True,
                 forward_tiles: bool = False) -> torch.Tensor:
    M, N = out.shape
    if M == 0:
        return out
    cptr, ldc = _mat(out, "out")
    arr = (GemmSeg * len(segs))()
    strides = (C.c_int64 * len(segs))()
    for i, (a, rs, b, stride) in enumerate(segs):
        ap, lda = _mat(a, f"A[{i}]")
        bp, ldb = _mat(b, f"B[{i}]")
        arr[i].a, arr[i].lda, arr[i].rowscale = ap, lda, _ptr(rs)
        arr[i].b, arr[i].ldb, arr[i].k = bp, ldb, a.size(1)
        strides[i] = stride
    flags = (_lib.GEMM_RELU if relu else 0) | (_lib.GEMM_B_TRANS if b_trans else 0)
    mp, ldm = (None, 0) if mask is None else _mat(mask, "mask")
    lib, h = _lib.load(), handle(out.device)
    nbytes = lib.gnx_gemm_workspace_bytes(h, len(segs), arr, strides, dc.D, M, N, mp, flags, 1)
    ws = torch.empty(nbytes, dtype=torch.uint8, device=out.device) if nbytes else None
    if forward_tiles:
        check(lib.gnx_gemm_grouped_rows(h, len(segs), arr, strides, dc.D, M, N, _ptr(bias), mp, ldm, cptr, ldc, flags,
                                        dc.dperm.data_ptr(), dc.tiles_p.data_ptr(), dc.ntiles_p.data_ptr(), dc.max_tiles_p,
                                        _ptr(ws), nbytes, dc.tile_rows_p))
        return out
    check(lib.gnx_gemm_grouped(h, len(segs), arr, strides, dc.D, M, N, _ptr(bias), mp, ldm, cptr, ldc, flags,
                               dc.dperm.data_ptr(), dc.tiles.data_ptr(), dc.ntiles.data_ptr(), dc.max_tiles, _ptr(ws),
                               nbytes))
    return out


def gemm_wgrad_grouped(dC: torch.Tensor, A: torch.Tensor, dW_cls: torch.Tensor, dc: DegreeClasses) -> None:
    M, N = dC.shape
    if M == 0:
        return
    xp, ldx = _mat(dC, "dC")
    ap, lda = _mat(A, "A")
    K = A.size(1)
    if dW_cls.shape != (dc.D, N, K) or not dW_cls.is_contiguous():
        raise _lib.GnxError(_lib.GNX_E_INVALID, f"dW_cls must be contiguous [{dc.D},{N},{K}], got {tuple(dW_cls.shape)}")
    check(_lib.load().gnx_gemm_wgrad_grouped(handle(dC.device), xp, ldx, ap, lda, M, N, K, dW_cls.data_ptr(), K, N * K,
                                             dc.dperm.data_ptr(), dc.chunks.data_ptr(), dc.nchunks.data_ptr(),
                                             dc.max_chunks))


def pna_weff(W: torch.Tensor, F: int, D: int, avg_deg_log: float) -> torch.Tensor:
    wp, ldw = _mat(W, "W")
    out = torch.empty(D, F, 4 * F, dtype=torch.float32, device=W.device)
    check(_lib.load().gnx_pna_weff(handle(W.device), wp, ldw, F, D, float(avg_deg_log), out.data_ptr()))
    return out


def pna_weff_bwd(dWeff: torch.Tensor, F: int, D: int, avg_deg_log: float, dW: torch.Tensor) -> None:
    wp, ldw = _mat(dW, "dW")
    check(_lib.load().gnx_pna_weff_bwd(handle(dW.device), dWeff.data_ptr(), F, D, float(avg_deg_log), wp, ldw))


_SIDE_ENABLED = False
_SIDE_PENDING = set()
_SIDE_KEEP: dict = {}


def set_wgrad_side_stream(enabled: bool) -> None:
    global _SIDE_ENABLED
    _SIDE_ENABLED = bool(enabled)


_JOIN_QUEUED = False


_SIDE_USED: dict = {}


def _join(idx: int, which: Optional[int] = None) -> None:
    dev = torch.device("cuda", idx)
    used = _SIDE_USED.get(idx, set())
    for w in sorted(used if which is None else (used & {which})):
        check(_lib.load().gnx_side_join_n(handle(dev), w))
        used.discard(w)
    if not used:
        _SIDE_PENDING.discard(idx)
        _SIDE_KEEP.pop(idx, None)


def _join_all_side_streams() -> None:
    global _JOIN_QUEUED
    _JOIN_QUEUED = False
    for idx in list(_SIDE_PENDING):
        _join(idx)


def join_side_stream_at_end_of_backward() -> None:
    global _JOIN_QUEUED
    if _SIDE_PENDING and not _JOIN_QUEUED:
        _JOIN_QUEUED = True
        torch.autograd.Variable._execution_engine.queue_callback(_join_all_side_streams)


_WGRAD_DONE_HOOK = None


def set_wgrad_done_hook(fn) -> None:
    global _WGRAD_DONE_HOOK
    _WGRAD_DONE_HOOK = fn


def wgrad_done_hook_set() -> bool:
    return _WGRAD_DONE_HOOK is not None


def side_stream(device: torch.device, which: int = 0) -> "torch.cuda.Stream":
    out = C.c_void_p()
    check(_lib.load().gnx_side_stream_n(handle(device), which, C.byref(out)))
    return torch.cuda.ExternalStream(out.value, device=device)


def second_side_stream_in_use(device: torch.device) -> bool:
    idx = device.index if device.index is not None else torch.cuda.current_device()
    return 1 in _SIDE_USED.get(idx, set())


def wgrad_stream_enabled() -> bool:
    return _SIDE_ENABLED


def scale_(t: torch.Tensor, v: float) -> torch.Tensor:
    if t.is_cuda and t.dtype is torch.float32 and t.is_contiguous():
        if t.numel():
            check(_lib.load().gnx_scale(handle(t.device), t.data_ptr(), t.numel(), float(v)))
        return t
    return t.mul_(v)


def finish_backward(device: torch.device, all_in_place: bool, sinks=None) -> None:
    if all_in_place:
        if _WGRAD_DONE_HOOK is not None and sinks:
            _WGRAD_DONE_HOOK(sinks)
        join_side_stream_at_end_of_backward()
    else:
        join_side_stream(device)


_WGRAD_QUEUE: List[tuple] = []
_WGRAD_BATCHING = True


def set_wgrad_batching(enabled: bool) -> None:
    global _WGRAD_BATCHING
    _WGRAD_BATCHING = bool(enabled)


def queue_wgrad(dC: torch.Tensor, A: torch.Tensor, dW: torch.Tensor, *, rowscale: Optional[torch.Tensor] = None,
                dbias: Optional[torch.Tensor] = None) -> None:
    if dC.size(0) == 0:
        return
    if not _WGRAD_BATCHING:
        gemm_wgrad(dC, A, dW, rowscale=rowscale, dbias=dbias)
        return
    _WGRAD_QUEUE.append((dC, A, dW, rowscale, dbias))


def flush_wgrads() -> None:
    global _WGRAD_QUEUE
    jobs, _WGRAD_QUEUE = _WGRAD_QUEUE, []
    if not jobs:
        return
    batchable, rest = [], []
    for j in jobs:
        dC, A, dW, rs, db = j
        ok = all(t is None or t.data_ptr() % 16 == 0 for t in (dC, A)) and dC.stride(0) % 4 == 0 and \
            A.stride(0) % 4 == 0 and dC.size(1) % 4 == 0 and A.size(1) % 4 == 0 and dC.size(0) > 1 and \
            (dC.size(1) == 1 or dC.stride(1) == 1) and (A.size(1) == 1 or A.stride(1) == 1)
        (batchable if ok else rest).append(j)
    for dC, A, dW, rs, db in rest:
        gemm_wgrad(dC, A, dW, rowscale=rs, dbias=db)
    batchable.sort(key=lambda j: -j[0].size(0))
    for i in range(0, len(batchable), 8):
        chunk = batchable[i:i + 8]
        arr = (_lib.WgradProb * len(chunk))()
        keep = []
        for k, (dC, A, dW, rs, db) in enumerate(chunk):
            xp, ldx = _mat(dC, "dC")
            ap, lda = _mat(A, "A")
            wp, ldw = _mat(dW, "dW")
            M, N = dC.shape
            K = A.size(1)
            if A.size(0) != M or dW.size(0) != N or dW.size(1) != K:
                raise _lib.GnxError(_lib.GNX_E_INVALID, f"wgrad shapes dC {tuple(dC.shape)} A {tuple(A.shape)} "
                                                        f"dW {tuple(dW.shape)}")
            arr[k].dC, arr[k].lddc, arr[k].A, arr[k].lda = xp, ldx, ap, lda
            arr[k].rowscale, arr[k].dW, arr[k].lddw, arr[k].dbias = _ptr(rs), wp, ldw, _ptr(db)
            arr[k].M, arr[k].N, arr[k].K = M, N, K
            keep += [dC, A, rs, dW, db]
        ref = chunk[0][0]
        n = len(chunk)
        _run_on_side(ref, keep, lambda arr=arr, n=n, ref=ref: check(
            _lib.load().gnx_gemm_wgrad_batched(handle(ref.device), n, arr)))


def join_side_stream(device: torch.device, which: Optional[int] = None) -> None:
    idx = device.index if device.index is not None else torch.cuda.current_device()
    if idx in _SIDE_PENDING:
        _join(idx, which)


def _run_on_side(ref: torch.Tensor, tensors, fn, which: int = 0) -> None:
    if _SIDE_ENABLED and ref.is_cuda:
        idx = ref.device.index
        lib, h = _lib.load(), handle(ref.device)
        check(lib.gnx_side_begin_n(h, which))
        try:
            fn()
        finally:
            check(lib.gnx_side_end(h))
        _SIDE_KEEP.setdefault(idx, []).extend(t for t in tensors if t is not None)
        _SIDE_PENDING.add(idx)
        _SIDE_USED.setdefault(idx, set()).add(which)
        return
    fn()


def run_after_wgrads(ref: torch.Tensor, tensors, fn) -> None:
    _run_on_side(ref, tensors, fn)


def keep_until_join(device: torch.device, tensors, whichs=(0, 1)) -> None:
    if not _SIDE_ENABLED:
        return
    idx = device.index if device.index is not None else torch.cuda.current_device()
    _SIDE_KEEP.setdefault(idx, []).extend(t for t in tensors if t is not None)
    _SIDE_PENDING.add(idx)
    _SIDE_USED.setdefault(idx, set()).update(whichs)


def pna_conv_bwd(args: "_lib.PnaBwdArgs", device: torch.device) -> None:
    check(_lib.load().gnx_pna_conv_bwd(handle(device), C.byref(args)))


def run_on_second_side_stream(ref: torch.Tensor, tensors, fn) -> None:
    _run_on_side(ref, tensors, fn, which=1)


def gemm_wgrad_inline(dC: torch.Tensor, A: torch.Tensor, dW: torch.Tensor, dbias: Optional[torch.Tensor] = None) -> None:
    _gemm_wgrad_launch(dC, A, dW, None, dbias)


def axpy_(y: torch.Tensor, x: torch.Tensor, alpha: float = 1.0) -> torch.Tensor:
    if y.numel() != x.numel() or not (y.is_contiguous() and x.is_contiguous()):
        raise _lib.GnxError(_lib.GNX_E_INVALID, "axpy_: need contiguous tensors of equal size")
    check(_lib.load().gnx_axpy(handle(y.device), _f32(y, "y").data_ptr(), _f32(x, "x").data_ptr(), y.numel(),
                               float(alpha)))
    return y


def gemm_wgrad(dC: torch.Tensor, A: torch.Tensor, dW: torch.Tensor, *, rowscale: Optional[torch.Tensor] = None,
               dbias: Optional[torch.Tensor] = None) -> None:
    if dC.size(0) == 0:
        return
    _run_on_side(dC, (dC, A, rowscale, dW, dbias), lambda: _gemm_wgrad_launch(dC, A, dW, rowscale, dbias))


def pna_post0_wgrad_classes(g: torch.Tensor, A: torch.Tensor, dc: "DegreeClasses", F: int, avg_deg_log: float,
                            dW: torch.Tensor) -> None:
    if g.size(0) == 0:
        return
    dWeff = zeros(dc.D, F, 4 * F, device=g.device)

    def run():
        gemm_wgrad_grouped(g, A, dWeff, dc)
        pna_weff_bwd(dWeff, F, dc.D, avg_deg_log, dW)

    _run_on_side(g, (g, A, dWeff, dW), run)


def _gemm_wgrad_launch(dC, A, dW, rowscale, dbias) -> None:
    M, N = dC.shape
    xp, ldx = _mat(dC, "dC")
    ap, lda = _mat(A, "A")
    wp, ldw = _mat(dW, "dW")
    K = A.size(1)
    if A.size(0) != M or dW.size(0) != N or dW.size(1) != K:
        raise _lib.GnxError(_lib.GNX_E_INVALID, f"wgrad shapes dC {tuple(dC.shape)} A {tuple(A.shape)} "
                                                f"dW {tuple(dW.shape)}")
    check(_lib.load().gnx_gemm_wgrad(handle(dW.device), xp, ldx, ap, lda, _ptr(rowscale), M, N, K, wp, ldw,
                                     _ptr(dbias)))


def edge_combine_fwd(P: torch.Tensor, Q: torch.Tensor, Te: torch.Tensor, g: GraphPack, relu: bool) -> torch.Tensor:
    H = P.size(1)
    h1 = torch.empty(g.E, H, dtype=torch.float32, device=P.device)
    check(_lib.load().gnx_edge_combine_fwd(handle(P.device), P.data_ptr(), Q.data_ptr(), Te.data_ptr(),
                                           g.src.data_ptr(), g.dst.data_ptr(), g.code.data_ptr(), g.E, H, int(relu),
                                           h1.data_ptr()))
    return h1


def edge_combine_bwd_pq(gr: torch.Tensor, g: GraphPack) -> Tuple[torch.Tensor, torch.Tensor]:
    H = gr.size(1)
    dP = torch.empty(g.N, H, dtype=torch.float32, device=gr.device)
    dQ = torch.empty(g.N, H, dtype=torch.float32, device=gr.device)
    check(_lib.load().gnx_edge_combine_bwd(handle(gr.device), gr.data_ptr(), g.rowptr.data_ptr(), g.colptr.data_ptr(),
                                           g.cpos.data_ptr(), g.code.data_ptr(), g.N, g.E, H, 0, dP.data_ptr(),
                                           dQ.data_ptr(), None, None, 0))
    return dP, dQ


def bond_table_grad(gr: torch.Tensor, g: GraphPack, R: int, pos: Optional[torch.Tensor]) -> torch.Tensor:
    H = gr.size(1)
    dTe = zeros(R, H, device=gr.device)
    lib = _lib.load()
    if g.E == 0:
        return dTe
    if pos is not None:
        check(lib.gnx_key_segment_sum(handle(gr.device), gr.data_ptr(), pos.data_ptr(), g.code.data_ptr(), g.E, H,
                                      dTe.data_ptr()))
        return dTe
    nbytes = lib.gnx_table_scatter_workspace_bytes(g.E, R, H)
    ws = torch.empty(max(nbytes, 1), dtype=torch.uint8, device=gr.device)
    tmp = torch.empty(2, g.N, H, dtype=torch.float32, device=gr.device)
    check(lib.gnx_edge_combine_bwd(handle(gr.device), gr.data_ptr(), g.rowptr.data_ptr(), g.colptr.data_ptr(),
                                   g.cpos.data_ptr(), g.code.data_ptr(), g.N, g.E, H, R, tmp[0].data_ptr(),
                                   tmp[1].data_ptr(), dTe.data_ptr(), ws.data_ptr(), nbytes))
    return dTe


def bond_code_index(g: GraphPack, R: int, H: int) -> Optional[torch.Tensor]:
    return g.code_index(R) if ((H % 4 == 0 and H <= 1024) or H <= 256) and g.E > 0 else None


def edge_combine_bwd(gr: torch.Tensor, g: GraphPack, R: int) -> Tuple[torch.Tensor, torch.Tensor, torch.Tensor]:
    dP, dQ = edge_combine_bwd_pq(gr, g)
    return dP, dQ, bond_table_grad(gr, g, R, bond_code_index(g, R, gr.size(1)))


def pna_edge_fwd(P: torch.Tensor, Q: torch.Tensor, Te: torch.Tensor, g: GraphPack, T: int, F: int,
                 weights: Sequence[torch.Tensor], biases: Sequence[torch.Tensor], max_degree: int,
                 keep: bool = True) -> Tuple[Optional[torch.Tensor], Optional[torch.Tensor], torch.Tensor]:
    H = T * F
    tiles = g.edge_tiles(max_degree)
    if tiles is None and g.E > 0:
        raise _lib.GnxError(_lib.GNX_E_INVALID, f"pna_edge_fwd: in-degree bound {max_degree} too large for edge tiles")
    dev = P.device
    h1 = torch.empty(g.E, H, dtype=torch.float32, device=dev) if keep else None
    m = torch.empty(g.E, H, dtype=torch.float32, device=dev) if keep else None
    A = torch.empty(g.N, T * 4 * F, dtype=torch.float32, device=dev)
    warr = (C.c_void_p * T)(*[_f32(w, "W1").data_ptr() for w in weights])
    barr = (C.c_void_p * T)(*[_f32(b, "b1").data_ptr() for b in biases])
    for w in weights:
        if tuple(w.shape) != (F, F) or not w.is_contiguous():
            raise _lib.GnxError(_lib.GNX_E_INVALID, f"pna_edge_fwd: pre-layer 1 weight must be contiguous [{F},{F}]")
    info, w_ = tiles if tiles is not None else (None, 1)
    check(_lib.load().gnx_pna_edge_fwd(handle(dev), P.data_ptr(), Q.data_ptr(), Te.data_ptr(), g.src.data_ptr(),
                                       g.dst.data_ptr(), g.code.data_ptr(), g.rowptr.data_ptr(), _ptr(info), w_, g.N, g.E,
                                       T, F, C.cast(warr, C.POINTER(C.c_void_p)), C.cast(barr, C.POINTER(C.c_void_p)),
                                       _ptr(h1), _ptr(m), A.data_ptr()))
    return h1, m, A


def pna_edge_bwd(ge: torch.Tensor, h1: torch.Tensor, g: GraphPack, T: int, F: int, R: int,
                 weights: Sequence[torch.Tensor], max_degree: int) -> Tuple[torch.Tensor, torch.Tensor, torch.Tensor]:
    H = T * F
    tiles = g.edge_tiles(max_degree)
    if tiles is None and g.E > 0:
        raise _lib.GnxError(_lib.GNX_E_INVALID, f"pna_edge_bwd: in-degree bound {max_degree} too large for edge tiles")
    dev = ge.device
    gh1 = torch.empty(g.E, H, dtype=torch.float32, device=dev)
    dP = torch.empty(g.N, H, dtype=torch.float32, device=dev)
    dTe = zeros(R, H, device=dev)
    warr = (C.c_void_p * T)(*[_f32(w, "W1").data_ptr() for w in weights])
    info, w_ = tiles if tiles is not None else (None, 1)
    check(_lib.load().gnx_pna_edge_bwd(handle(dev), _f32(ge, "ge").contiguous().data_ptr(), _f32(h1, "h1").contiguous().data_ptr(),
                                       g.code.data_ptr(), g.rowptr.data_ptr(), _ptr(info), w_, g.N, g.E, T, F, R,
                                       C.cast(warr, C.POINTER(C.c_void_p)), gh1.data_ptr(), dP.data_ptr(), dTe.data_ptr()))
    return gh1, dP, dTe


def pna_aggregate_fwd(m: torch.Tensor, g: GraphPack, T: int, F: int) -> torch.Tensor:
    A = torch.empty(g.N, T * 4 * F, dtype=torch.float32, device=m.device)
    check(_lib.load().gnx_pna_aggregate_fwd(handle(m.device), m.data_ptr(), g.rowptr.data_ptr(), g.N, g.E, T, F,
                                            A.data_ptr()))
    return A


def pna_aggregate_bwd(dA: torch.Tensor, m: torch.Tensor, A: torch.Tensor, g: GraphPack, T: int, F: int) -> torch.Tensor:
    dm = torch.empty_like(m)
    check(_lib.load().gnx_pna_aggregate_bwd(handle(m.device), dA.data_ptr(), m.data_ptr(), A.data_ptr(),
                                            g.rowptr.data_ptr(), g.N, g.E, T, F, dm.data_ptr()))
    return dm


def gine_aggregate_fwd(x: torch.Tensor, Le: torch.Tensor, g: GraphPack, eps: float) -> torch.Tensor:
    out = torch.empty_like(x)
    check(_lib.load().gnx_gine_aggregate_fwd(handle(x.device), x.data_ptr(), Le.data_ptr(), g.rowptr.data_ptr(),
                                             g.src.data_ptr(), g.code.data_ptr(), g.N, g.E, x.size(1), float(eps),
                                             out.data_ptr()))
    return out


def gine_aggregate_bwd(dout: torch.Tensor, x: torch.Tensor, Le: torch.Tensor, g: GraphPack,
                       eps: float, want_dle: bool = True) -> Tuple[torch.Tensor, Optional[torch.Tensor]]:
    dx = torch.empty_like(x)
    dLe = zeros(*Le.shape, device=Le.device) if want_dle else None
    pos = g.code_index(Le.size(0)) if (g.E > 0 and want_dle) else None
    check(_lib.load().gnx_gine_aggregate_bwd(handle(x.device), dout.data_ptr(), x.data_ptr(), Le.data_ptr(),
                                             g.colptr.data_ptr(), g.cpos.data_ptr(), g.src.data_ptr(),
                                             g.dst.data_ptr(), g.code.data_ptr(), _ptr(pos), g.N, g.E, x.size(1),
                                             Le.size(0), float(eps), dx.data_ptr(), _ptr(dLe)))
    return dx, dLe


def gine_dle(dout: torch.Tensor, x: torch.Tensor, Le: torch.Tensor, g: GraphPack, pos: Optional[torch.Tensor]) -> torch.Tensor:
    dLe = zeros(*Le.shape, device=Le.device)
    check(_lib.load().gnx_gine_dle(handle(x.device), dout.data_ptr(), x.data_ptr(), Le.data_ptr(), g.src.data_ptr(),
                                   g.dst.data_ptr(), g.code.data_ptr(), _ptr(pos), g.E, x.size(1), Le.size(0),
                                   dLe.data_ptr()))
    return dLe


def transformer_attn_fwd(qkvs: torch.Tensor, Le: torch.Tensor, g: GraphPack, heads: int, p: float = 0.0,
                         seed: int = 0, offset: int = 0, want_mask: bool = False
                         ) -> Tuple[torch.Tensor, torch.Tensor, Optional[torch.Tensor]]:
    qkvs = _f32(qkvs, "qkvs").contiguous()
    Le = _f32(Le, "Le").contiguous()
    N, H = qkvs.size(0), qkvs.size(1) // 4
    if qkvs.size(1) != 4 * H or Le.size(1) != H or heads <= 0 or H % heads != 0:
        raise _lib.GnxError(_lib.GNX_E_INVALID, f"transformer_attn_fwd: qkvs {tuple(qkvs.shape)} Le {tuple(Le.shape)} "
                                                f"heads {heads}")
    dev = qkvs.device
    out = torch.empty(N, H, dtype=torch.float32, device=dev)
    alpha = torch.empty(g.E, heads, dtype=torch.float32, device=dev)
    keep = torch.empty(g.E, heads, dtype=torch.uint8, device=dev) if want_mask else None
    check(_lib.load().gnx_transformer_attn_fwd(handle(dev), qkvs.data_ptr(), Le.data_ptr(), g.rowptr.data_ptr(),
                                               g.src.data_ptr(), g.code.data_ptr(), N, g.E, int(heads), H // int(heads),
                                               float(p), int(seed) & (2 ** 64 - 1), int(offset) & (2 ** 64 - 1),
                                               out.data_ptr(), alpha.data_ptr(), _ptr(keep)))
    return out, alpha, keep


def transformer_attn_bwd(dout: torch.Tensor, qkvs: torch.Tensor, Le: torch.Tensor, alpha: torch.Tensor, g: GraphPack,
                         heads: int, p: float = 0.0, seed: int = 0, offset: int = 0, want_dle: bool = True
                         ) -> Tuple[torch.Tensor, torch.Tensor, Optional[torch.Tensor]]:
    dout = _f32(dout, "dout").contiguous()
    N, H = dout.shape
    dev = dout.device
    dqkv = torch.empty(N, 3 * H, dtype=torch.float32, device=dev)
    scratch = torch.empty(2, g.E, heads, dtype=torch.float32, device=dev)
    dLe = zeros(*Le.shape, device=dev) if want_dle else None
    pos = g.code_index(Le.size(0)) if (want_dle and g.E > 0) else None
    if want_dle and g.E > 0 and pos is None:
        raise _lib.GnxError(_lib.GNX_E_INVALID, f"transformer_attn_bwd: {Le.size(0)} bond codes exceed the inverted index")
    check(_lib.load().gnx_transformer_attn_bwd(handle(dev), dout.data_ptr(), qkvs.data_ptr(), Le.data_ptr(),
                                               alpha.data_ptr(), g.rowptr.data_ptr(), g.src.data_ptr(), g.dst.data_ptr(),
                                               g.code.data_ptr(), g.colptr.data_ptr(), g.cpos.data_ptr(), _ptr(pos), N,
                                               g.E, int(heads), H // int(heads), Le.size(0), float(p),
                                               int(seed) & (2 ** 64 - 1), int(offset) & (2 ** 64 - 1), dqkv.data_ptr(),
                                               scratch.data_ptr(), _ptr(dLe)))
    return dqkv, scratch, dLe


def transformer_attn_dle(dout: torch.Tensor, qkvs: torch.Tensor, scratch: torch.Tensor, Le: torch.Tensor, g: GraphPack,
                         heads: int, pos: Optional[torch.Tensor]) -> torch.Tensor:
    R, H = Le.shape
    dLe = zeros(R, H, device=dout.device)
    if g.E == 0:
        return dLe
    if pos is None:
        raise _lib.GnxError(_lib.GNX_E_INVALID, f"transformer_attn_dle: {R} bond codes exceed the inverted index")
    check(_lib.load().gnx_transformer_attn_dle(handle(dout.device), dout.data_ptr(), qkvs.data_ptr(), scratch.data_ptr(),
                                               g.dst.data_ptr(), g.code.data_ptr(), pos.data_ptr(), g.E, int(heads),
                                               H // int(heads), R, dLe.data_ptr()))
    return dLe


def _f64_on(t: torch.Tensor, name: str, dev: torch.device) -> torch.Tensor:
    if t.dtype != torch.float64 or t.device != dev:
        raise _lib.GnxError(_lib.GNX_E_INVALID, f"{name}: expected float64 on {dev}, got {t.dtype} on {t.device}")
    return t.contiguous()


def _pcsaft_args(params: torch.Tensor, owner: torch.Tensor, T: torch.Tensor, name: str):
    dev = params.device
    params = _f64_on(params, f"{name}: params", dev)
    if params.dim() != 2 or params.size(1) != 9:
        raise _lib.GnxError(_lib.GNX_E_INVALID, f"{name}: params must be [B, 9], got {tuple(params.shape)}")
    if owner.dtype != torch.int64 or owner.device != dev or owner.dim() != 1:
        raise _lib.GnxError(_lib.GNX_E_INVALID, f"{name}: owner must be a 1-D int64 tensor on {dev}")
    T = _f64_on(T, f"{name}: T", dev)
    if T.shape != owner.shape:
        raise _lib.GnxError(_lib.GNX_E_INVALID, f"{name}: T {tuple(T.shape)} and owner {tuple(owner.shape)} differ")
    return params, owner.contiguous(), T


def pcsaft_density(params: torch.Tensor, owner: torch.Tensor, T: torch.Tensor, P: torch.Tensor
                   ) -> Tuple[torch.Tensor, torch.Tensor]:
    params, owner, T = _pcsaft_args(params, owner, T, "pcsaft_density")
    P = _f64_on(P, "pcsaft_density: P", params.device)
    if P.shape != T.shape:
        raise _lib.GnxError(_lib.GNX_E_INVALID, f"pcsaft_density: P {tuple(P.shape)} and T {tuple(T.shape)} differ")
    n, dev = T.numel(), params.device
    rho = torch.empty(n, dtype=torch.float64, device=dev)
    status = torch.empty(n, dtype=torch.int32, device=dev)
    check(_lib.load().gnx_pcsaft_density(handle(dev), params.data_ptr(), params.size(0), owner.data_ptr(),
                                         T.data_ptr(), P.data_ptr(), n, rho.data_ptr(), status.data_ptr()))
    return rho, status


def pcsaft_vapor_pressure(params: torch.Tensor, owner: torch.Tensor, T: torch.Tensor
                          ) -> Tuple[torch.Tensor, torch.Tensor, torch.Tensor, torch.Tensor]:
    params, owner, T = _pcsaft_args(params, owner, T, "pcsaft_vapor_pressure")
    n, dev = T.numel(), params.device
    out = torch.empty(3, n, dtype=torch.float64, device=dev)
    status = torch.empty(n, dtype=torch.int32, device=dev)
    check(_lib.load().gnx_pcsaft_vapor_pressure(handle(dev), params.data_ptr(), params.size(0), owner.data_ptr(),
                                                T.data_ptr(), n, out[0].data_ptr(), out[1].data_ptr(),
                                                out[2].data_ptr(), status.data_ptr()))
    return out[0], out[1], out[2], status


def _pcsaft_mix_args(params, comp, kij, eab, owner, T, second, x, name):
    params, owner, T = _pcsaft_args(params, owner, T, name)
    dev = params.device
    if comp.dtype != torch.int64 or comp.device != dev or comp.dim() != 2 or not 1 <= comp.size(1) <= 4:
        raise _lib.GnxError(_lib.GNX_E_INVALID, f"{name}: comp must be an int64 [M, nc] tensor on {dev} with 1 <= nc <= 4")
    M, nc = comp.shape
    mats = []
    for label, t in (("kij", kij), ("eab", eab)):
        if t is not None:
            t = _f64_on(t, f"{name}: {label}", dev)
            if tuple(t.shape) != (M, nc, nc):
                raise _lib.GnxError(_lib.GNX_E_INVALID, f"{name}: {label} must be [{M}, {nc}, {nc}], got {tuple(t.shape)}")
        mats.append(t)
    second = _f64_on(second, f"{name}: state", dev)
    x = _f64_on(x, f"{name}: x", dev)
    if second.shape != T.shape or tuple(x.shape) != (T.numel(), nc):
        raise _lib.GnxError(_lib.GNX_E_INVALID, f"{name}: T {tuple(T.shape)}, state {tuple(second.shape)} and x "
                                                f"{tuple(x.shape)} do not describe n points of {nc} components")
    return params, comp.contiguous(), mats[0], mats[1], owner, T, second, x


def pcsaft_mix_state(params: torch.Tensor, comp: torch.Tensor, kij: Optional[torch.Tensor], eab: Optional[torch.Tensor],
                     owner: torch.Tensor, T: torch.Tensor, rho: torch.Tensor, x: torch.Tensor
                     ) -> Tuple[torch.Tensor, torch.Tensor, torch.Tensor, torch.Tensor]:
    params, comp, kij, eab, owner, T, rho, x = _pcsaft_mix_args(params, comp, kij, eab, owner, T, rho, x,
                                                                "pcsaft_mix_state")
    n, dev = T.numel(), params.device
    out = torch.empty(3, n, dtype=torch.float64, device=dev)
    status = torch.empty(n, dtype=torch.int32, device=dev)
    check(_lib.load().gnx_pcsaft_mix_state(handle(dev), params.data_ptr(), params.size(0), comp.data_ptr(), _ptr(kij),
                                           _ptr(eab), comp.size(0), comp.size(1), owner.data_ptr(), T.data_ptr(),
                                           rho.data_ptr(), x.data_ptr(), n, out[0].data_ptr(), out[1].data_ptr(),
                                           out[2].data_ptr(), status.data_ptr()))
    return out[0], out[1], out[2], status


def pcsaft_mix_density(params: torch.Tensor, comp: torch.Tensor, kij: Optional[torch.Tensor],
                       eab: Optional[torch.Tensor], owner: torch.Tensor, T: torch.Tensor, P: torch.Tensor,
                       x: torch.Tensor) -> Tuple[torch.Tensor, torch.Tensor]:
    params, comp, kij, eab, owner, T, P, x = _pcsaft_mix_args(params, comp, kij, eab, owner, T, P, x,
                                                              "pcsaft_mix_density")
    n, dev = T.numel(), params.device
    rho = torch.empty(n, dtype=torch.float64, device=dev)
    status = torch.empty(n, dtype=torch.int32, device=dev)
    check(_lib.load().gnx_pcsaft_mix_density(handle(dev), params.data_ptr(), params.size(0), comp.data_ptr(), _ptr(kij),
                                             _ptr(eab), comp.size(0), comp.size(1), owner.data_ptr(), T.data_ptr(),
                                             P.data_ptr(), x.data_ptr(), n, rho.data_ptr(), status.data_ptr()))
    return rho, status


_POOL = {"add": _lib.POOL_ADD, "sum": _lib.POOL_ADD, "mean": _lib.POOL_MEAN, "max": _lib.POOL_MAX}


def segment_pool_fwd(x: torch.Tensor, ptr: torch.Tensor, B: int, mode: str) -> torch.Tensor:
    out = torch.empty(B, x.size(1), dtype=torch.float32, device=x.device)
    check(_lib.load().gnx_segment_pool_fwd(handle(x.device), x.data_ptr(), ptr.data_ptr(), B, x.size(1), _POOL[mode],
                                           out.data_ptr()))
    return out


def segment_pool_bwd(dout: torch.Tensor, x: torch.Tensor, out: torch.Tensor, ptr: torch.Tensor, B: int,
                     mode: str) -> torch.Tensor:
    dx = torch.empty_like(x)
    check(_lib.load().gnx_segment_pool_bwd(handle(x.device), dout.data_ptr(), x.data_ptr(), out.data_ptr(),
                                           ptr.data_ptr(), B, x.size(1), _POOL[mode], dx.data_ptr()))
    return dx


def _bn_ws(M: int, H: int, dev) -> Tuple[torch.Tensor, int]:
    nbytes = _lib.load().gnx_batchnorm_workspace_bytes(M, H)
    return torch.empty(nbytes, dtype=torch.uint8, device=dev), nbytes


def batchnorm_fwd(x, gamma, beta, running_mean, running_var, momentum: float, eps: float, training: bool, relu: bool,
                  num_batches_tracked: Optional[torch.Tensor] = None):
    M, H = x.shape
    y = torch.empty_like(x)
    mean = torch.empty(H, dtype=torch.float32, device=x.device)
    rstd = torch.empty(H, dtype=torch.float32, device=x.device)
    ws, nbytes = _bn_ws(M, H, x.device)
    check(_lib.load().gnx_batchnorm_fwd(handle(x.device), x.data_ptr(), M, H, _ptr(gamma), _ptr(beta),
                                        _ptr(running_mean), _ptr(running_var), _ptr(num_batches_tracked),
                                        float(momentum), float(eps),
                                        int(training), int(relu), y.data_ptr(), mean.data_ptr(), rstd.data_ptr(),
                                        ws.data_ptr(), nbytes))
    return y, mean, rstd


def batchnorm_bwd(dy, x, y, gamma, mean, rstd, relu: bool, dgamma=None, dbeta=None):
    M, H = x.shape
    dx = torch.empty_like(x)
    if dgamma is None:
        dgamma = zeros(H, device=x.device)
    if dbeta is None:
        dbeta = zeros(H, device=x.device)
    ws, nbytes = _bn_ws(M, H, x.device)
    check(_lib.load().gnx_batchnorm_bwd(handle(x.device), dy.data_ptr(), x.data_ptr(), y.data_ptr(), M, H, _ptr(gamma),
                                        mean.data_ptr(), rstd.data_ptr(), int(relu), dx.data_ptr(), dgamma.data_ptr(),
                                        dbeta.data_ptr(), ws.data_ptr(), nbytes))
    return dx, dgamma, dbeta


def dropout(x: torch.Tensor, p: float, seed: int, offset: int) -> torch.Tensor:
    x = _f32(x, "x").contiguous()
    y = torch.empty_like(x)
    check(_lib.load().gnx_dropout(handle(x.device), x.data_ptr(), x.numel(), float(p), int(seed) & (2 ** 64 - 1),
                                  int(offset) & (2 ** 64 - 1), y.data_ptr()))
    return y


def huber_ape(pred: torch.Tensor, target: torch.Tensor, delta: float, need_grad: bool):
    pred = _f32(pred, "pred").contiguous()
    target = _f32(target, "target").contiguous()
    if pred.shape != target.shape:
        raise _lib.GnxError(_lib.GNX_E_INVALID, f"pred {tuple(pred.shape)} vs target {tuple(target.shape)}")
    out2 = torch.empty(2, dtype=torch.float32, device=pred.device)
    dpred = torch.empty_like(pred) if need_grad else None
    check(_lib.load().gnx_huber_ape(handle(pred.device), pred.data_ptr(), target.data_ptr(), pred.numel(), float(delta),
                                    out2.data_ptr(), _ptr(dpred)))
    return out2, dpred


def clip_rows(x: torch.Tensor, lo: torch.Tensor, hi: torch.Tensor) -> torch.Tensor:
    x = _f32(x, "x").contiguous()
    y = torch.empty_like(x)
    check(_lib.load().gnx_clip_rows(handle(x.device), x.data_ptr(), x.size(0), x.size(1), lo.data_ptr(), hi.data_ptr(),
                                    y.data_ptr()))
    return y


def prof_begin(device: torch.device, kernel_ids: Sequence[int]) -> None:
    mask = 0
    for k in kernel_ids:
        mask |= 1 << k
    check(_lib.load().gnx_prof_begin(handle(device), mask))


def prof_read(device: torch.device, kernel_id: int) -> Tuple[int, float]:
    d = prof_read_work(device, kernel_id)
    return d["launches"], d["ms"]


def prof_read_work(device: torch.device, kernel_id: int) -> dict:
    n, ms = C.c_int64(0), C.c_double(0.0)
    by, fl, mf = C.c_double(0.0), C.c_double(0.0), C.c_double(0.0)
    check(_lib.load().gnx_prof_read(handle(device), kernel_id, C.byref(n), C.byref(ms), C.byref(by), C.byref(fl),
                                    C.byref(mf)))
    return {"launches": n.value, "ms": ms.value, "bytes": by.value, "flops": fl.value, "mfma_bf16_flops": mf.value}


def prof_end(device: torch.device) -> None:
    check(_lib.load().gnx_prof_end(handle(device)))
```

### include/gnx.h

```cpp
#ifndef GNX_H_
#define GNX_H_

#include <stddef.h>
#include <stdint.h>

#ifdef __cplusplus
extern "C" {
#endif

#define GNX_ABI_VERSION 7

enum {
  GNX_OK = 0,
  GNX_E_INVALID = -1,
  GNX_E_HIP = -2,
  GNX_E_RANGE = -3,
  GNX_E_WORKSPACE = -4
};

typedef struct gnx_handle gnx_handle;

int32_t gnx_create(gnx_handle** out, int32_t device);
int32_t gnx_destroy(gnx_handle* h);
int32_t gnx_set_stream(gnx_handle* h, void* hip_stream);
const char* gnx_last_error(void);
int32_t gnx_abi_version(void);

enum {
  GNX_OPT_GEMM_SPLIT = 0,
  GNX_OPT_WGRAD_WGS = 1,
  GNX_OPT_EMBED_BWD_MFMA = 2,
  GNX_OPT_STD_BWD_CENTERED = 3,
  GNX_OPT_GEMM_PIPE = 4,
  GNX_OPT_WGRAD_PIPE = 5,
  GNX_OPT_GEMM_AS = 6,
  GNX_OPT_GEMM_WS_FAST = 7,
  GNX_OPT_GEMM_TILE_ROWS = 8,
  GNX_OPT_GEMM_MID = 9,
  GNX_OPT_COUNT = 10
};
int32_t gnx_set_option(gnx_handle* h, int32_t opt, int32_t value);
int32_t gnx_get_option(gnx_handle* h, int32_t opt, int32_t* value);

enum {
  GNX_K_NONE = 0,
  GNX_K_PNA_AGG_FWD = 1,
  GNX_K_PNA_AGG_BWD = 2,
  GNX_K_GEMM_WS = 3,
  GNX_K_GEMM_WGRAD = 4,
  GNX_K_GINE_AGG_FWD = 5,
  GNX_K_GINE_AGG_BWD = 6,
  GNX_K_EDGE_COMBINE_FWD = 7,
  GNX_K_EDGE_COMBINE_BWD = 8,
  GNX_K_BN_FWD = 9,
  GNX_K_BN_BWD = 10,
  GNX_K_GEMM_TILED = 11,
  GNX_K_GEMM_SMALL = 12,
  GNX_K_GEMM_WGRAD_BATCHED = 13,
  GNX_K_KEY_SEGMENT_SUM = 14,
  GNX_K_EMBED = 15,
  GNX_K_PNA_EDGE_FWD = 16,
  GNX_K_PNA_EDGE_BWD = 17,
  GNX_K_ATTN_FWD = 18,
  GNX_K_ATTN_BWD = 19,
  GNX_K_PCSAFT_RHO = 20,
  GNX_K_PCSAFT_VP = 21,
  GNX_K_PCSAFT_MIX_STATE = 22,
  GNX_K_PCSAFT_MIX_RHO = 23,
  GNX_K_COUNT = 24
};
int32_t gnx_prof_begin(gnx_handle* h, uint32_t kernel_mask);
int32_t gnx_prof_read(gnx_handle* h, int32_t kid, int64_t* launches, double* total_ms, double* alg_bytes,
                      double* alg_flops, double* mfma_bf16_flops);
int32_t gnx_prof_end(gnx_handle* h);

size_t gnx_pack_csr_workspace_bytes(int64_t N, int64_t E);
int32_t gnx_pack_csr(gnx_handle* h, const int64_t* edge_index, int64_t E, int64_t N, int32_t* rowptr, int32_t* perm,
                     int32_t* src, int32_t* dst, int32_t* colptr, int32_t* cpos, void* ws, size_t ws_bytes);
int32_t gnx_feature_code(gnx_handle* h, const int64_t* feat, int64_t rows, int32_t K, const int32_t* dims,
                         const int32_t* perm, int32_t* code, void* ws, size_t ws_bytes);
int32_t gnx_graph_ptr(gnx_handle* h, const int64_t* batch, int64_t N, int64_t B, int32_t* graph_ptr, void* ws,
                      size_t ws_bytes);
int32_t gnx_degree_scalers(gnx_handle* h, const int32_t* rowptr, int64_t N, float avg_deg_log, float* amp, float* att);

int32_t gnx_collate_ptr(gnx_handle* h, const int64_t* node_ptr, const int64_t* edge_ptr, int64_t G, const int64_t* idx,
                        int64_t B, int64_t* out_ptr, int64_t* out_eptr);
int32_t gnx_collate_gather(gnx_handle* h, const int64_t* node_ptr, const int64_t* edge_ptr, int64_t G, const int64_t* x,
                           const int64_t* edge_index, const int64_t* edge_attr, int64_t E_src, const int64_t* idx,
                           int64_t B, const int64_t* out_ptr, const int64_t* out_eptr, int64_t N, int64_t E,
                           int64_t* x_out, int64_t* edge_index_out, int64_t* edge_attr_out, int64_t* batch_out);
int32_t gnx_collate_rows(gnx_handle* h, const void* src, int64_t G, const int64_t* idx, int64_t B, int32_t elem_bytes,
                         int32_t K, void* dst);

int32_t gnx_embed_sum_fwd(gnx_handle* h, const int64_t* idx, int64_t N, int32_t K, const int32_t* offsets,
                          const float* table, int32_t H, float* out);
size_t gnx_table_scatter_workspace_bytes(int64_t rows, int32_t R, int32_t H);
int32_t gnx_embed_sum_bwd(gnx_handle* h, const int64_t* idx, int64_t N, int32_t K, const int32_t* offsets,
                          int32_t R, const float* dout, int32_t H, float* dtable, void* ws, size_t ws_bytes);
int32_t gnx_check_range(gnx_handle* h);

typedef struct {
  const float* a;
  int64_t lda;
  const float* rowscale;
  const float* b;
  int64_t ldb;
  int32_t k;
  int32_t _pad;
} gnx_gemm_seg;

enum {
  GNX_GEMM_RELU = 1,
  GNX_GEMM_ACCUMULATE = 2,
  GNX_GEMM_B_TRANS = 4,
  GNX_GEMM_SPLIT_ONLY = 8,
  GNX_GEMM_PRESPLIT = 16
};
size_t gnx_gemm_workspace_bytes(gnx_handle* h, int32_t nseg, const gnx_gemm_seg* segs, const int64_t* cls_strides,
                                int32_t num_classes, int64_t M, int32_t N, const float* mask, int32_t flags,
                                int32_t grouped);
int32_t gnx_gemm(gnx_handle* h, int32_t nseg, const gnx_gemm_seg* segs, int64_t M, int32_t N, const float* bias,
                 const float* mask, int64_t ldmask, float* C, int64_t ldc, int32_t flags, void* ws, size_t ws_bytes);
int32_t gnx_gemm_wgrad(gnx_handle* h, const float* dC, int64_t lddc, const float* A, int64_t lda,
                       const float* rowscale, int64_t M, int32_t N, int32_t K, float* dW, int64_t lddw, float* dbias);

typedef struct {
  const float* dC;
  int64_t lddc;
  const float* A;
  int64_t lda;
  const float* rowscale;
  float* dW;
  int64_t lddw;
  float* dbias;
  int64_t M;
  int32_t N, K;
} gnx_wgrad_prob;
int32_t gnx_gemm_wgrad_batched(gnx_handle* h, int32_t nprob, const gnx_wgrad_prob* probs);

enum { GNX_SB_A_TRANS = 1, GNX_SB_B_TRANS = 2, GNX_SB_ACCUMULATE = 4, GNX_SB_ATOMIC = 8, GNX_SB_RELU = 16 };
#define GNX_SMALL_BATCH 32
typedef struct {
  const float* A;
  int64_t lda;
  const float* B;
  int64_t ldb;
  const float* bias;
  float* C;
  int64_t ldc;
  int32_t M, N, K;
  int32_t flags;
} gnx_small_prob;
int32_t gnx_gemm_small_batched(gnx_handle* h, int32_t nprob, const gnx_small_prob* probs);

int32_t gnx_degree_max(gnx_handle* h, const int32_t* rowptr, int64_t N, int32_t* max_degree_host);
size_t gnx_degree_classes_workspace_bytes(int64_t N, int32_t D);
int32_t gnx_degree_classes(gnx_handle* h, const int32_t* rowptr, int64_t N, int32_t D, int32_t* dperm,
                           int32_t* cls_ptr, void* ws, size_t ws_bytes);
int32_t gnx_class_tiles(gnx_handle* h, const int32_t* cls_ptr, int32_t D, int32_t tile_rows, int32_t* tile_info,
                        int32_t* ntiles);
int32_t gnx_gemm_grouped(gnx_handle* h, int32_t nseg, const gnx_gemm_seg* segs, const int64_t* cls_strides,
                         int32_t num_classes, int64_t M, int32_t N, const float* bias, const float* mask,
                         int64_t ldmask, float* C, int64_t ldc, int32_t flags, const int32_t* row_index,
                         const int32_t* tile_info, const int32_t* ntiles, int64_t max_tiles, void* ws, size_t ws_bytes);
int32_t gnx_gemm_tile_rows(gnx_handle* h, int64_t M, int32_t N);
int32_t gnx_gemm_grouped_rows(gnx_handle* h, int32_t nseg, const gnx_gemm_seg* segs, const int64_t* cls_strides,
                              int32_t num_classes, int64_t M, int32_t N, const float* bias, const float* mask,
                              int64_t ldmask, float* C, int64_t ldc, int32_t flags, const int32_t* row_index,
                              const int32_t* tile_info, const int32_t* ntiles, int64_t max_tiles, void* ws,
                              size_t ws_bytes, int32_t tile_rows);
int32_t gnx_gemm_wgrad_grouped(gnx_handle* h, const float* dC, int64_t lddc, const float* A, int64_t lda, int64_t M,
                               int32_t N, int32_t K, float* dW_cls, int64_t lddw, int64_t dw_cls_stride,
                               const int32_t* row_index, const int32_t* chunk_info, const int32_t* nchunks,
                               int64_t max_chunks);
int32_t gnx_pna_weff(gnx_handle* h, const float* W, int64_t ldw, int32_t F, int32_t D, float avg_deg_log, float* Weff);
int32_t gnx_pna_weff_bwd(gnx_handle* h, const float* dWeff, int32_t F, int32_t D, float avg_deg_log, float* dW,
                         int64_t lddw);
int32_t gnx_pna_weff_batched(gnx_handle* h, int32_t n, const float* const* W, int64_t ldw, int32_t F, int32_t D,
                             const float* avg_deg_log, float* const* Weff);
int32_t gnx_pna_weff_bwd_batched(gnx_handle* h, int32_t n, const float* const* dWeff, int32_t F, int32_t D,
                                 const float* avg_deg_log, float* const* dW, int64_t lddw);

int32_t gnx_edge_combine_fwd(gnx_handle* h, const float* P, const float* Q, const float* Te, const int32_t* src,
                             const int32_t* dst, const int32_t* code, int64_t E, int32_t H, int32_t relu, float* h1);
int32_t gnx_edge_combine_bwd(gnx_handle* h, const float* g, const int32_t* rowptr, const int32_t* colptr,
                             const int32_t* cpos, const int32_t* code, int64_t N, int64_t E, int32_t H, int32_t R,
                             float* dP, float* dQ, float* dTe, void* ws, size_t ws_bytes);

int32_t gnx_group_by_small_key(gnx_handle* h, const int32_t* keys, int64_t E, int32_t R, int32_t* pos, int32_t* ptr,
                               void* ws, size_t ws_bytes);
int32_t gnx_key_segment_sum(gnx_handle* h, const float* g, const int32_t* pos, const int32_t* key, int64_t E, int32_t H,
                            float* dtable);

int32_t gnx_pna_aggregate_fwd(gnx_handle* h, const float* m, const int32_t* rowptr, int64_t N, int64_t E, int32_t T,
                              int32_t F, float* A);
int32_t gnx_pna_aggregate_bwd(gnx_handle* h, const float* dA, const float* m, const float* A, const int32_t* rowptr,
                              int64_t N, int64_t E, int32_t T, int32_t F, float* dm);

int32_t gnx_edge_tiles_count(int64_t E, int32_t tile_w);
int32_t gnx_edge_tiles(gnx_handle* h, const int32_t* rowptr, int64_t N, int64_t E, int32_t tile_w, int32_t* tile_info);
int32_t gnx_pna_edge_bwd(gnx_handle* h, const float* ge, const float* h1, const int32_t* code, const int32_t* rowptr,
                         const int32_t* tile_info, int32_t tile_w, int64_t N, int64_t E, int32_t T, int32_t F, int32_t R,
                         const float* const* W1, float* gh1, float* dP, float* dTe);
int32_t gnx_pna_edge_fwd(gnx_handle* h, const float* P, const float* Q, const float* Te, const int32_t* src,
                         const int32_t* dst, const int32_t* code, const int32_t* rowptr, const int32_t* tile_info,
                         int32_t tile_w, int64_t N, int64_t E, int32_t T, int32_t F, const float* const* W1,
                         const float* const* b1, float* h1, float* m, float* A);

int32_t gnx_gine_aggregate_fwd(gnx_handle* h, const float* x, const float* Le, const int32_t* rowptr,
                               const int32_t* src, const int32_t* code, int64_t N, int64_t E, int32_t H, float eps,
                               float* out);
int32_t gnx_gine_aggregate_bwd(gnx_handle* h, const float* dout, const float* x, const float* Le,
                               const int32_t* colptr, const int32_t* cpos, const int32_t* src, const int32_t* dst,
                               const int32_t* code, const int32_t* code_pos, int64_t N, int64_t E, int32_t H, int32_t R,
                               float eps, float* dx, float* dLe);

int32_t gnx_gine_dle(gnx_handle* h, const float* dout, const float* x, const float* Le, const int32_t* src,
                     const int32_t* dst, const int32_t* code, const int32_t* code_pos, int64_t E, int32_t H, int32_t R,
                     float* dLe);

int32_t gnx_transformer_attn_fwd(gnx_handle* h, const float* qkvs, const float* Le, const int32_t* rowptr,
                                 const int32_t* src, const int32_t* code, int64_t N, int64_t E, int32_t heads,
                                 int32_t C, float p, uint64_t seed, uint64_t offset, float* out, float* alpha,
                                 uint8_t* keep);
int32_t gnx_transformer_attn_bwd(gnx_handle* h, const float* dout, const float* qkvs, const float* Le,
                                 const float* alpha, const int32_t* rowptr, const int32_t* src, const int32_t* dst,
                                 const int32_t* code, const int32_t* colptr, const int32_t* cpos,
                                 const int32_t* code_pos, int64_t N, int64_t E, int32_t heads, int32_t C, int32_t R,
                                 float p, uint64_t seed, uint64_t offset, float* dqkv, float* scratch, float* dLe);
int32_t gnx_transformer_attn_dle(gnx_handle* h, const float* dout, const float* qkvs, const float* scratch,
                                 const int32_t* dst, const int32_t* code, const int32_t* code_pos, int64_t E,
                                 int32_t heads, int32_t C, int32_t R, float* dLe);

int32_t gnx_pcsaft_density(gnx_handle* h, const double* params, int64_t B, const int64_t* owner, const double* T,
                           const double* P, int64_t n, double* rho, int32_t* status);
int32_t gnx_pcsaft_vapor_pressure(gnx_handle* h, const double* params, int64_t B, const int64_t* owner, const double* T,
                                  int64_t n, double* psat, double* rho_l, double* rho_v, int32_t* status);

int32_t gnx_pcsaft_mix_state(gnx_handle* h, const double* params, int64_t B, const int64_t* mix_comp,
                             const double* mix_kij, const double* mix_eab, int64_t M, int32_t nc, const int64_t* owner,
                             const double* T, const double* rho, const double* x, int64_t n, double* a_res, double* p,
                             double* dpdrho, int32_t* status);
int32_t gnx_pcsaft_mix_density(gnx_handle* h, const double* params, int64_t B, const int64_t* mix_comp,
                               const double* mix_kij, const double* mix_eab, int64_t M, int32_t nc,
                               const int64_t* owner, const double* T, const double* P, const double* x, int64_t n,
                               double* rho, int32_t* status);

enum { GNX_POOL_ADD = 0, GNX_POOL_MEAN = 1, GNX_POOL_MAX = 2 };
int32_t gnx_segment_pool_fwd(gnx_handle* h, const float* x, const int32_t* ptr, int64_t B, int32_t H, int32_t mode,
                             float* out);
int32_t gnx_segment_pool_bwd(gnx_handle* h, const float* dout, const float* x, const float* out, const int32_t* ptr,
                             int64_t B, int32_t H, int32_t mode, float* dx);

size_t gnx_batchnorm_workspace_bytes(int64_t M, int32_t H);
int32_t gnx_batchnorm_fwd(gnx_handle* h, const float* x, int64_t M, int32_t H, const float* gamma, const float* beta,
                          float* running_mean, float* running_var, int64_t* num_batches_tracked, float momentum,
                          float eps, int32_t training, int32_t relu, float* y, float* save_mean, float* save_rstd,
                          void* ws, size_t ws_bytes);
int32_t gnx_batchnorm_bwd(gnx_handle* h, const float* dy, const float* x, const float* y, int64_t M, int32_t H,
                          const float* gamma, const float* save_mean, const float* save_rstd, int32_t relu,
                          float* dx, float* dgamma, float* dbeta, void* ws, size_t ws_bytes);

int32_t gnx_dropout(gnx_handle* h, const float* x, int64_t n, float p, uint64_t seed, uint64_t offset, float* y);

int32_t gnx_huber_ape(gnx_handle* h, const float* pred, const float* target, int64_t count, float delta, float* out2,
                      float* dpred);

int32_t gnx_adamw_amsgrad(gnx_handle* h, float* p, const float* g, float* m, float* v, float* vmax, int64_t n, float lr,
                          float beta1, float beta2, float eps, float weight_decay, int64_t step);
int32_t gnx_sgd(gnx_handle* h, float* p, const float* g, int64_t n, float lr);

#define GNX_PNA_MAX_LAYERS 8
#define GNX_PNA_MAX_TOWERS 8
enum {
  GNX_PNA_BWD_DEFER_SMALL = 1,
  GNX_PNA_BWD_LAST_OF_PASS = 2
};
typedef struct {
  int64_t N, E;
  int32_t T, F, pre_layers, post_layers, R, D;
  float avg_deg_log;
  int32_t merged;
  int32_t acc_first;
  int32_t use_side_streams;
  int32_t n_h, n_z;
  const int32_t *rowptr, *colptr, *cpos, *code, *code_pos, *dperm, *tiles, *ntiles, *chunks, *nchunks;
  int64_t max_tiles, max_chunks;
  const float *x, *BE, *EE, *A;
  const float* hs[GNX_PNA_MAX_LAYERS];
  const float* zs[GNX_PNA_MAX_LAYERS];
  const float* weff[GNX_PNA_MAX_TOWERS];
  const float* Wm;
  const float* const* params;
  float* const* grads;
  const float* dout;
  float* gbuf[GNX_PNA_MAX_LAYERS];
  float* dA;
  float* gebuf[GNX_PNA_MAX_LAYERS];
  float *dP, *dQ;
  float *dTe, *dEE;
  float *dWm, *dbm;
  float* dWeff;
  void* ws;
  size_t ws_bytes;
  float* acc_buf;
  float* dx;
  int32_t flags;
  int32_t etile_w;
  const int32_t* etile_info;
} gnx_pna_bwd_args;
size_t gnx_pna_conv_bwd_workspace_bytes(int32_t T, int32_t F, int32_t D);
int32_t gnx_pna_conv_bwd(gnx_handle* h, const gnx_pna_bwd_args* args);

typedef struct {
  int32_t L, T, F, pre_layers, post_layers, R, D, merged, use_side_streams, _pad;
  const float* BE;
  float* acc_buf;
  const float* ones;
  const float* avg_deg_log;
  const float* const* params;
  float* const* grads;
  const float* const* EE;
  float* const* dTe;
  float* const* dEE;
  const float* const* dWm;
  const float* const* dbm;
  const float* const* dWeff;
} gnx_pna_finish_args;
int32_t gnx_pna_stack_finish(gnx_handle* h, const gnx_pna_finish_args* args);
int32_t gnx_pna_weight_only_all(gnx_handle* h, int32_t L, const float* BE, int32_t R, int32_t T, int32_t F,
                                int32_t pre_layers, int32_t post_layers, int32_t D, const float* avg_deg_log,
                                const float* const* params, int32_t merged, float* const* EE, float* const* Te,
                                float* const* weff, float* const* Wm, float* const* bm);

int32_t gnx_pna_weight_only(gnx_handle* h, const float* BE, int32_t R, int32_t T, int32_t F, int32_t pre_layers,
                            int32_t post_layers, int32_t D, float avg_deg_log, const float* const* params, int32_t merged,
                            float* EE, float* Te, float* const* weff, float* Wm, float* bm);
typedef struct {
  int64_t N, E;
  int32_t T, F, pre_layers, post_layers, D, merged;
  const int32_t *rowptr, *src, *dst, *code, *dperm, *tiles, *ntiles;
  int64_t max_tiles;
  const float *x, *Te;
  const float* weff[GNX_PNA_MAX_TOWERS];
  const float *Wm, *bm;
  const float* const* params;
  float *P, *Q, *A;
  float* hs[GNX_PNA_MAX_LAYERS];
  float* zs[GNX_PNA_MAX_LAYERS];
  void* ws;
  size_t ws_bytes;
  float* out;
  const int32_t* etile_info;
  int32_t etile_w;
  int32_t tile_rows;
} gnx_pna_fwd_args;
int32_t gnx_pna_conv_fwd(gnx_handle* h, const gnx_pna_fwd_args* args);

int32_t gnx_fill(gnx_handle* h, float* p, int64_t n, float v);
int32_t gnx_scale(gnx_handle* h, float* p, int64_t n, float v);
int32_t gnx_axpy(gnx_handle* h, float* y, const float* x, int64_t n, float a);

int32_t gnx_side_begin(gnx_handle* h);
int32_t gnx_side_stream(gnx_handle* h, void** hip_stream);
int32_t gnx_side_end(gnx_handle* h);
int32_t gnx_side_join(gnx_handle* h);
int32_t gnx_side_stream_n(gnx_handle* h, int32_t which, void** hip_stream);
int32_t gnx_side_begin_n(gnx_handle* h, int32_t which);
int32_t gnx_side_join_n(gnx_handle* h, int32_t which);
int32_t gnx_clip_rows(gnx_handle* h, const float* x, int64_t M, int32_t P, const float* lo, const float* hi, float* y);

#ifdef __cplusplus
}
#endif
#endif
```

Baseline: 623,500 graphs/s.

## Fuse CSR packing, feature coding and graph_ptr into fewer batched kernel launches

Replaces the separate CSR pack, feature-code and graph_ptr launches with a single gnx_pack_graph entry point. Degree counting moves into edge conversion, the row and column scans run together in one two-job scan (a single tile pass plus a decoupled finish kernel), and column fill and feature codes come out of the same gather kernel. Class tile tables are built in one multi-table call, and degree scalers are skipped when degree classes are in use. The aim is to cut kernel launch count and host overhead in the per-step packing, in exchange for more complex kernels and a slightly larger workspace.

```diff
diff --git a/gnnepcsaft_amd/_lib.py b/gnnepcsaft_amd/_lib.py
--- a/gnnepcsaft_amd/_lib.py
+++ b/gnnepcsaft_amd/_lib.py
@@ -107,6 +107,8 @@
     "gnx_prof_end": (_i32, [_vp]),
     "gnx_pack_csr_workspace_bytes": (_sz, [_i64, _i64]),
     "gnx_pack_csr": (_i32, [_vp, _vp, _i64, _i64, _vp, _vp, _vp, _vp, _vp, _vp, _vp, _sz]),
+    "gnx_pack_graph": (_i32, [_vp, _vp, _i64, _i64, _vp, _i32, C.POINTER(_i32), _vp, _i64, _vp, _vp, _vp, _vp, _vp, _vp,
+                              _vp, _vp, _vp, _sz]),
     "gnx_feature_code": (_i32, [_vp, _vp, _i64, _i32, C.POINTER(_i32), _vp, _vp, _vp, _sz]),
     "gnx_graph_ptr": (_i32, [_vp, _vp, _i64, _i64, _vp, _vp, _sz]),
     "gnx_degree_scalers": (_i32, [_vp, _vp, _i64, _f32, _vp, _vp]),
@@ -127,6 +129,7 @@
     "gnx_degree_classes_workspace_bytes": (_sz, [_i64, _i32]),
     "gnx_degree_classes": (_i32, [_vp, _vp, _i64, _i32, _vp, _vp, _vp, _sz]),
     "gnx_class_tiles": (_i32, [_vp, _vp, _i32, _i32, _vp, _vp]),
+    "gnx_class_tiles_multi": (_i32, [_vp, _vp, _i32, _i32, C.POINTER(_i32), C.POINTER(_vp), C.POINTER(_vp)]),
     "gnx_gemm_grouped": (_i32, [_vp, _i32, C.POINTER(GemmSeg), C.POINTER(_i64), _i32, _i64, _i32, _vp, _vp, _i64, _vp,
                                 _i64, _i32, _vp, _vp, _vp, _i64, _vp, _sz]),
     "gnx_gemm_tile_rows": (_i32, [_vp, _i64, _i32]),
diff --git a/gnnepcsaft_amd/csrc/gnx_pack.hip b/gnnepcsaft_amd/csrc/gnx_pack.hip
--- a/gnnepcsaft_amd/csrc/gnx_pack.hip
+++ b/gnnepcsaft_amd/csrc/gnx_pack.hip
@@ -3,10 +3,26 @@
 #define SCAN_ITEMS 4
 #define SCAN_BLOCK 256
 #define SCAN_TILE (SCAN_ITEMS * SCAN_BLOCK)
-
-__global__ void __launch_bounds__(SCAN_BLOCK) k_scan_tile(const int* __restrict__ in, int* __restrict__ out,
-                                                          int* __restrict__ sums, int64_t n) {
+#define SCAN_JOBS 2
+
+struct scan_jobs {
+  const int* in[SCAN_JOBS];
+  int* out[SCAN_JOBS];
+  int* sums[SCAN_JOBS];
+  int64_t n[SCAN_JOBS];
+  int total[SCAN_JOBS];
+};
+
+static inline int64_t scan_tiles(int64_t n) { return n > 0 ? gnx_cdiv(n, SCAN_TILE) : 1; }
+
+__global__ void __launch_bounds__(SCAN_BLOCK) k_scan_tile(scan_jobs a) {
   __shared__ int s[SCAN_BLOCK];
+  const int j = blockIdx.y;
+  const int64_t n = a.n[j];
+  const int64_t tiles = n > 0 ? (n + SCAN_TILE - 1) / SCAN_TILE : 1;
+  if ((int64_t)blockIdx.x >= tiles) return;
+  const int* __restrict__ in = a.in[j];
+  int* __restrict__ out = a.out[j];
   int64_t base = (int64_t)blockIdx.x * SCAN_TILE + (int64_t)threadIdx.x * SCAN_ITEMS;
   int v[SCAN_ITEMS];
   int t = 0;
@@ -29,7 +45,33 @@
     if (base + i < n) out[base + i] = excl;
     excl += v[i];
   }
-  if (threadIdx.x == SCAN_BLOCK - 1) sums[blockIdx.x] = s[SCAN_BLOCK - 1];
+  if (threadIdx.x == SCAN_BLOCK - 1) {
+    a.sums[j][blockIdx.x] = s[SCAN_BLOCK - 1];
+    if (tiles == 1 && a.total[j]) out[n] = s[SCAN_BLOCK - 1];
+  }
+}
+
+__global__ void __launch_bounds__(SCAN_BLOCK) k_scan_finish(scan_jobs a) {
+  __shared__ int s[SCAN_BLOCK / 64];
+  const int j = blockIdx.y;
+  const int64_t n = a.n[j];
+  const int64_t tiles = (n + SCAN_TILE - 1) / SCAN_TILE;
+  if ((int64_t)blockIdx.x >= tiles) return;
+  const int* __restrict__ sums = a.sums[j];
+  int* __restrict__ out = a.out[j];
+  int o = 0;
+  for (int i = threadIdx.x; i < (int)blockIdx.x; i += SCAN_BLOCK) o += sums[i];
+  for (int off = 32; off > 0; off >>= 1) o += __shfl_xor(o, off);
+  if ((threadIdx.x & 63) == 0) s[threadIdx.x >> 6] = o;
+  __syncthreads();
+  o = 0;
+#pragma unroll
+  for (int w = 0; w < SCAN_BLOCK / 64; ++w) o += s[w];
+  int64_t i = (int64_t)blockIdx.x * SCAN_TILE + threadIdx.x;
+  if (o != 0)
+    for (int k = 0; k < SCAN_ITEMS; ++k, i += SCAN_BLOCK)
+      if (i < n) out[i] += o;
+  if ((int64_t)blockIdx.x == tiles - 1 && threadIdx.x == 0 && a.total[j]) out[n] = o + sums[blockIdx.x];
 }
 
 __global__ void k_scan_add(int* __restrict__ out, const int* __restrict__ offs, int64_t n) {
@@ -43,24 +85,51 @@
   if (threadIdx.x == 0 && blockIdx.x == 0) out[n] = (n > 0) ? out[n - 1] + in[n - 1] : 0;
 }
 
-static int32_t exclusive_scan(gnx_handle* h, const int* in, int* out, int64_t n, int* ws, bool write_total) {
-  if (n > 0) {
-    int64_t blocks = gnx_cdiv(n, SCAN_TILE);
-    hipLaunchKernelGGL(k_scan_tile, dim3((unsigned)blocks), dim3(SCAN_BLOCK), 0, h->stream, in, out, ws, n);
-    GNX_LAUNCH_CHECK();
-    if (blocks > 1) {
-      int* sums_scanned = ws + blocks + 1;
-      int32_t st = exclusive_scan(h, ws, sums_scanned, blocks, sums_scanned + blocks + 1, false);
-      if (st != GNX_OK) return st;
-      hipLaunchKernelGGL(k_scan_add, dim3((unsigned)blocks), dim3(SCAN_BLOCK), 0, h->stream, out, sums_scanned, n);
-      GNX_LAUNCH_CHECK();
-    }
-  }
+static int32_t exclusive_scan_multi(gnx_handle* h, const scan_jobs& a, int count);
+
+static int32_t exclusive_scan_long(gnx_handle* h, const int* in, int* out, int64_t n, int* sums, bool write_total) {
+  const int64_t tiles = scan_tiles(n);
+  scan_jobs a = {};
+  a.in[0] = in, a.out[0] = out, a.sums[0] = sums, a.n[0] = n, a.total[0] = 0;
+  hipLaunchKernelGGL(k_scan_tile, dim3((unsigned)tiles, 1), dim3(SCAN_BLOCK), 0, h->stream, a);
+  GNX_LAUNCH_CHECK();
+  int* sums_scanned = sums + tiles + 1;
+  scan_jobs b = {};
+  b.in[0] = sums, b.out[0] = sums_scanned, b.sums[0] = sums_scanned + tiles + 1, b.n[0] = tiles, b.total[0] = 0;
+  int32_t st = exclusive_scan_multi(h, b, 1);
+  if (st != GNX_OK) return st;
+  hipLaunchKernelGGL(k_scan_add, dim3((unsigned)tiles), dim3(SCAN_BLOCK), 0, h->stream, out, sums_scanned, n);
+  GNX_LAUNCH_CHECK();
   if (write_total) {
     hipLaunchKernelGGL(k_set_total, dim3(1), dim3(64), 0, h->stream, out, in, n);
     GNX_LAUNCH_CHECK();
   }
   return GNX_OK;
+}
+
+static int32_t exclusive_scan_multi(gnx_handle* h, const scan_jobs& a, int count) {
+  int64_t tiles = 1;
+  for (int j = 0; j < count; ++j) tiles = scan_tiles(a.n[j]) > tiles ? scan_tiles(a.n[j]) : tiles;
+  if (tiles > SCAN_TILE) {
+    for (int j = 0; j < count; ++j) {
+      int32_t st = exclusive_scan_long(h, a.in[j], a.out[j], a.n[j], a.sums[j], a.total[j] != 0);
+      if (st != GNX_OK) return st;
+    }
+    return GNX_OK;
+  }
+  hipLaunchKernelGGL(k_scan_tile, dim3((unsigned)tiles, (unsigned)count), dim3(SCAN_BLOCK), 0, h->stream, a);
+  GNX_LAUNCH_CHECK();
+  if (tiles > 1) {
+    hipLaunchKernelGGL(k_scan_finish, dim3((unsigned)tiles, (unsigned)count), dim3(SCAN_BLOCK), 0, h->stream, a);
+    GNX_LAUNCH_CHECK();
+  }
+  return GNX_OK;
+}
+
+static int32_t exclusive_scan(gnx_handle* h, const int* in, int* out, int64_t n, int* ws, bool write_total) {
+  scan_jobs a = {};
+  a.in[0] = in, a.out[0] = out, a.sums[0] = ws, a.n[0] = n, a.total[0] = write_total ? 1 : 0;
+  return exclusive_scan_multi(h, a, 1);
 }
 
 static size_t scan_ws_ints_total(int64_t n) {
@@ -74,8 +143,57 @@
   return tot + 16;
 }
 
+struct dims_t {
+  int d[16];
+};
+
+__device__ __forceinline__ int feature_code(const int64_t* __restrict__ feat, int64_t r, int K, const dims_t& dims,
+                                            int* __restrict__ flag) {
+  int c = 0;
+  bool bad = false;
+  for (int k = 0; k < K; ++k) {
+    int64_t f = feat[r * K + k];
+    if (f < 0 || f >= dims.d[k]) {
+      bad = true;
+      f = 0;
+    }
+    c = c * dims.d[k] + (int)f;
+  }
+  if (bad) atomicOr(flag, 2);
+  return c;
+}
+
+__device__ __forceinline__ void graph_ptr_at(const int64_t* __restrict__ batch, int64_t n, int64_t N, int64_t B,
+                                             int* __restrict__ ptr, int* __restrict__ flag) {
+  int64_t prev = (n == 0) ? -1 : batch[n - 1];
+  int64_t cur = (n == N) ? B : batch[n];
+  if (n < N && (cur < 0 || cur >= B)) {
+    atomicOr(flag, 4);
+    return;
+  }
+  if (cur < prev) {
+    atomicOr(flag, 8);
+    return;
+  }
+  for (int64_t g = prev + 1; g <= cur; ++g) ptr[g] = (int)n;
+}
+
+__device__ __forceinline__ void sort_group(const int* __restrict__ ptr, int64_t i, int* __restrict__ items) {
+  int b = ptr[i], e = ptr[i + 1];
+  for (int a = b + 1; a < e; ++a) {
+    int v = items[a];
+    int c = a - 1;
+    while (c >= b && items[c] > v) {
+      items[c + 1] = items[c];
+      --c;
+    }
+    items[c + 1] = v;
+  }
+}
+
 __global__ void k_convert_edges(const int64_t* __restrict__ ei, int64_t E, int64_t N, int* __restrict__ src0,
-                                int* __restrict__ dst0, int* __restrict__ flag) {
+                                int* __restrict__ dst0, int* __restrict__ cnt_dst, int* __restrict__ cnt_src,
+                                int* __restrict__ flag) {
   int64_t e = (int64_t)blockIdx.x * blockDim.x + threadIdx.x;
   if (e >= E) return;
   int64_t s = ei[e], d = ei[E + e];
@@ -87,11 +205,8 @@
   }
   src0[e] = (int)s;
   dst0[e] = (int)d;
-}
-
-__global__ void k_count_keys(const int* __restrict__ key, int64_t E, int* __restrict__ counts) {
-  int64_t e = (int64_t)blockIdx.x * blockDim.x + threadIdx.x;
-  if (e < E) atomicAdd(&counts[key[e]], 1);
+  atomicAdd(&cnt_dst[d], 1);
+  atomicAdd(&cnt_src[s], 1);
 }
 
 __global__ void k_fill_groups(const int* __restrict__ key, int64_t E, const int* __restrict__ ptr,
@@ -103,151 +218,140 @@
   items[pos] = (int)e;
 }
 
-__global__ void k_sort_groups(const int* __restrict__ ptr, int64_t N, int* __restrict__ items) {
+__global__ void k_sort_groups(const int* __restrict__ ptr, int64_t N, int* __restrict__ items,
+                              const int64_t* __restrict__ batch, int64_t B, int* __restrict__ graph_ptr,
+                              int* __restrict__ flag) {
   int64_t i = (int64_t)blockIdx.x * blockDim.x + threadIdx.x;
-  if (i >= N) return;
-  int b = ptr[i], e = ptr[i + 1];
-  for (int a = b + 1; a < e; ++a) {
-    int v = items[a];
-    int c = a - 1;
-    while (c >= b && items[c] > v) {
-      items[c + 1] = items[c];
-      --c;
-    }
-    items[c + 1] = v;
-  }
-}
-
-__global__ void k_gather_endpoints(const int* __restrict__ perm, const int* __restrict__ src0,
-                                   const int* __restrict__ dst0, int64_t E, int* __restrict__ src,
-                                   int* __restrict__ dst) {
+  if (items && i < N) sort_group(ptr, i, items);
+  if (graph_ptr && i <= N) graph_ptr_at(batch, i, N, B, graph_ptr, flag);
+}
+
+__global__ void k_gather_fill_cols(const int* __restrict__ perm, const int* __restrict__ src0,
+                                   const int* __restrict__ dst0, int64_t E, const int* __restrict__ colptr,
+                                   int* __restrict__ cursor, int* __restrict__ src, int* __restrict__ dst,
+                                   int* __restrict__ cpos, const int64_t* __restrict__ feat, int K, dims_t dims,
+                                   int* __restrict__ code, int* __restrict__ flag) {
   int64_t p = (int64_t)blockIdx.x * blockDim.x + threadIdx.x;
   if (p >= E) return;
   int e = perm[p];
-  src[p] = src0[e];
+  int s = src0[e];
+  src[p] = s;
   dst[p] = dst0[e];
-}
-
-static int32_t group_by_key(gnx_handle* h, const int* key, int64_t E, int64_t N, int* ptr, int* items, int* cursor,
-                            int* scan_ws) {
-  gnx_zero_ints(h, cursor, N > 0 ? N : 1);
-  if (E > 0) {
-    hipLaunchKernelGGL(k_count_keys, dim3((unsigned)gnx_cdiv(E, 256)), dim3(256), 0, h->stream, key, E, cursor);
-    GNX_LAUNCH_CHECK();
-  }
-  int32_t st = exclusive_scan(h, cursor, ptr, N, scan_ws, true);
-  if (st != GNX_OK) return st;
-  gnx_zero_ints(h, cursor, N > 0 ? N : 1);
-  if (E > 0) {
-    hipLaunchKernelGGL(k_fill_groups, dim3((unsigned)gnx_cdiv(E, 256)), dim3(256), 0, h->stream, key, E, ptr, cursor,
-                       items);
-    GNX_LAUNCH_CHECK();
-    hipLaunchKernelGGL(k_sort_groups, dim3((unsigned)gnx_cdiv(N, 256)), dim3(256), 0, h->stream, ptr, N, items);
-    GNX_LAUNCH_CHECK();
-  }
-  return GNX_OK;
+  cpos[colptr[s] + atomicAdd(&cursor[s], 1)] = (int)p;
+  if (feat) code[p] = feature_code(feat, e, K, dims, flag);
 }
 
 extern "C" size_t gnx_pack_csr_workspace_bytes(int64_t N, int64_t E) {
   if (N < 0) N = 0;
   if (E < 0) E = 0;
-  size_t ints = 2 * (size_t)E + (size_t)N + 1 + scan_ws_ints_total(N) + 64;
+  size_t ints = 2 * (size_t)E + 4 * ((size_t)N + 1) + 2 * scan_ws_ints_total(N) + 64;
   return ints * sizeof(int);
+}
+
+static int32_t feature_dims(const char* who, int32_t K, const int32_t* dims, dims_t* d) {
+  GNX_CHECK_ARG(dims && K > 0 && K <= 16, "%s: bad argument", who);
+  int64_t prod = 1;
+  for (int k = 0; k < 16; ++k) d->d[k] = (k < K) ? dims[k] : 1;
+  for (int k = 0; k < K; ++k) {
+    GNX_CHECK_ARG(dims[k] > 0, "%s: dims[%d] <= 0", who, k);
+    prod *= dims[k];
+    GNX_CHECK_ARG(prod < (1ll << 31), "%s: code space overflows int32", who);
+  }
+  return GNX_OK;
+}
+
+extern "C" int32_t gnx_pack_graph(gnx_handle* h, const int64_t* edge_index, int64_t E, int64_t N, const int64_t* feat,
+                                  int32_t K, const int32_t* dims, const int64_t* batch, int64_t B, int32_t* rowptr,
+                                  int32_t* perm, int32_t* src, int32_t* dst, int32_t* colptr, int32_t* cpos,
+                                  int32_t* code, int32_t* graph_ptr, void* ws, size_t ws_bytes) {
+  GNX_CHECK_ARG(h != nullptr, "gnx_pack_graph: handle is NULL");
+  GNX_CHECK_ARG(N >= 0 && E >= 0 && N < (1ll << 31) - 1 && E < (1ll << 31) - 1, "gnx_pack_graph: N=%lld E=%lld out of int32 range",
+                (long long)N, (long long)E);
+  GNX_CHECK_ARG(rowptr && colptr, "gnx_pack_graph: rowptr/colptr NULL");
+  GNX_CHECK_ARG(E == 0 || (edge_index && perm && src && dst && cpos), "gnx_pack_graph: NULL edge array with E>0");
+  GNX_CHECK_ARG(!feat || E == 0 || code, "gnx_pack_graph: code NULL with features");
+  GNX_CHECK_ARG(!graph_ptr || (B >= 0 && (batch || N == 0)), "gnx_pack_graph: graph_ptr without a batch vector, or B < 0");
+  dims_t d = {};
+  GNX_CHECK_ARG(!feat || dims, "gnx_pack_graph: dims NULL with features");
+  if (dims) {
+    int32_t st = feature_dims("gnx_pack_graph", K, dims, &d);
+    if (st != GNX_OK) return st;
+  }
+  if (ws_bytes < gnx_pack_csr_workspace_bytes(N, E) || (!ws && ws_bytes)) {
+    gnx_set_error("gnx_pack_graph: workspace %zu < %zu", ws_bytes, gnx_pack_csr_workspace_bytes(N, E));
+    return GNX_E_WORKSPACE;
+  }
+  GNX_CHECK_ARG(ws != nullptr, "gnx_pack_graph: workspace is NULL");
+  int* w = reinterpret_cast<int*>(ws);
+  int* src0 = w;
+  int* dst0 = src0 + E;
+  int* cnt_dst = dst0 + E;
+  int* cnt_src = cnt_dst + N + 1;
+  int* cur_dst = cnt_src + N + 1;
+  int* cur_src = cur_dst + N + 1;
+  int* scan_ws = cur_src + N + 1;
+  gnx_zero_ints(h, cnt_dst, 4 * (N + 1));
+  GNX_LAUNCH_CHECK();
+  if (E > 0) {
+    hipLaunchKernelGGL(k_convert_edges, dim3((unsigned)gnx_cdiv(E, 256)), dim3(256), 0, h->stream, edge_index, E, N,
+                       src0, dst0, cnt_dst, cnt_src, h->d_flag);
+    GNX_LAUNCH_CHECK();
+  }
+  scan_jobs a = {};
+  a.in[0] = cnt_dst, a.out[0] = rowptr, a.sums[0] = scan_ws, a.n[0] = N, a.total[0] = 1;
+  a.in[1] = cnt_src, a.out[1] = colptr, a.sums[1] = scan_ws + scan_ws_ints_total(N), a.n[1] = N, a.total[1] = 1;
+  int32_t st = exclusive_scan_multi(h, a, 2);
+  if (st != GNX_OK) return st;
+  if (E > 0) {
+    hipLaunchKernelGGL(k_fill_groups, dim3((unsigned)gnx_cdiv(E, 256)), dim3(256), 0, h->stream, dst0, E, rowptr, cur_dst,
+                       perm);
+    GNX_LAUNCH_CHECK();
+  }
+  if (E > 0 || graph_ptr) {
+    hipLaunchKernelGGL(k_sort_groups, dim3((unsigned)gnx_cdiv(N + 1, 256)), dim3(256), 0, h->stream, rowptr, N,
+                       E > 0 ? perm : (int*)nullptr, batch, B, graph_ptr, h->d_flag);
+    GNX_LAUNCH_CHECK();
+  }
+  if (E > 0) {
+    hipLaunchKernelGGL(k_gather_fill_cols, dim3((unsigned)gnx_cdiv(E, 256)), dim3(256), 0, h->stream, perm, src0, dst0, E,
+                       colptr, cur_src, src, dst, cpos, feat, (int)K, d, code, h->d_flag);
+    GNX_LAUNCH_CHECK();
+    hipLaunchKernelGGL(k_sort_groups, dim3((unsigned)gnx_cdiv(N + 1, 256)), dim3(256), 0, h->stream, colptr, N, cpos,
+                       (const int64_t*)nullptr, (int64_t)0, (int*)nullptr, h->d_flag);
+    GNX_LAUNCH_CHECK();
+  }
+  return GNX_OK;
 }
 
 extern "C" int32_t gnx_pack_csr(gnx_handle* h, const int64_t* edge_index, int64_t E, int64_t N, int32_t* rowptr,
                                 int32_t* perm, int32_t* src, int32_t* dst, int32_t* colptr, int32_t* cpos, void* ws,
                                 size_t ws_bytes) {
-  GNX_CHECK_ARG(h != nullptr, "gnx_pack_csr: handle is NULL");
-  GNX_CHECK_ARG(N >= 0 && E >= 0 && N < (1ll << 31) - 1 && E < (1ll << 31) - 1, "gnx_pack_csr: N=%lld E=%lld out of int32 range",
-                (long long)N, (long long)E);
-  GNX_CHECK_ARG(rowptr && colptr, "gnx_pack_csr: rowptr/colptr NULL");
-  GNX_CHECK_ARG(E == 0 || (edge_index && perm && src && dst && cpos), "gnx_pack_csr: NULL edge array with E>0");
-  if (ws_bytes < gnx_pack_csr_workspace_bytes(N, E) || (!ws && ws_bytes)) {
-    gnx_set_error("gnx_pack_csr: workspace %zu < %zu", ws_bytes, gnx_pack_csr_workspace_bytes(N, E));
-    return GNX_E_WORKSPACE;
-  }
-  GNX_CHECK_ARG(ws != nullptr, "gnx_pack_csr: workspace is NULL");
-  int* w = reinterpret_cast<int*>(ws);
-  int* src0 = w;
-  int* dst0 = src0 + E;
-  int* cursor = dst0 + E;
-  int* scan_ws = cursor + N + 1;
-  if (E > 0) {
-    hipLaunchKernelGGL(k_convert_edges, dim3((unsigned)gnx_cdiv(E, 256)), dim3(256), 0, h->stream, edge_index, E, N,
-                       src0, dst0, h->d_flag);
-    GNX_LAUNCH_CHECK();
-  }
-  int32_t st = group_by_key(h, dst0, E, N, rowptr, perm, cursor, scan_ws);
-  if (st != GNX_OK) return st;
-  if (E > 0) {
-    hipLaunchKernelGGL(k_gather_endpoints, dim3((unsigned)gnx_cdiv(E, 256)), dim3(256), 0, h->stream, perm, src0,
-                       dst0, E, src, dst);
-    GNX_LAUNCH_CHECK();
-  }
-  return group_by_key(h, src, E, N, colptr, cpos, cursor, scan_ws);
-}
-
-struct dims_t {
-  int d[16];
-};
+  return gnx_pack_graph(h, edge_index, E, N, nullptr, 0, nullptr, nullptr, 0, rowptr, perm, src, dst, colptr, cpos,
+                        nullptr, nullptr, ws, ws_bytes);
+}
 
 __global__ void k_feature_code(const int64_t* __restrict__ feat, int64_t rows, int K, dims_t dims,
                                const int* __restrict__ perm, int* __restrict__ code, int* __restrict__ flag) {
   int64_t p = (int64_t)blockIdx.x * blockDim.x + threadIdx.x;
   if (p >= rows) return;
-  int64_t r = perm ? perm[p] : p;
-  int c = 0;
-  bool bad = false;
-  for (int k = 0; k < K; ++k) {
-    int64_t f = feat[r * K + k];
-    if (f < 0 || f >= dims.d[k]) {
-      bad = true;
-      f = 0;
-    }
-    c = c * dims.d[k] + (int)f;
-  }
-  if (bad) atomicOr(flag, 2);
-  code[p] = c;
+  code[p] = feature_code(feat, perm ? perm[p] : p, K, dims, flag);
 }
 
 extern "C" int32_t gnx_feature_code(gnx_handle* h, const int64_t* feat, int64_t rows, int32_t K, const int32_t* dims,
                                     const int32_t* perm, int32_t* code, void* ws, size_t ws_bytes) {
   (void)ws;
   (void)ws_bytes;
-  GNX_CHECK_ARG(h && dims && K > 0 && K <= 16 && rows >= 0, "gnx_feature_code: bad argument");
+  GNX_CHECK_ARG(h && rows >= 0, "gnx_feature_code: bad argument");
   GNX_CHECK_ARG(rows == 0 || (feat && code), "gnx_feature_code: NULL array with rows>0");
   dims_t d;
-  int64_t prod = 1;
-  for (int k = 0; k < 16; ++k) d.d[k] = (k < K) ? dims[k] : 1;
-  for (int k = 0; k < K; ++k) {
-    GNX_CHECK_ARG(dims[k] > 0, "gnx_feature_code: dims[%d] <= 0", k);
-    prod *= dims[k];
-  }
-  GNX_CHECK_ARG(prod < (1ll << 31), "gnx_feature_code: code space overflows int32");
+  int32_t st = feature_dims("gnx_feature_code", K, dims, &d);
+  if (st != GNX_OK) return st;
   if (rows > 0) {
     hipLaunchKernelGGL(k_feature_code, dim3((unsigned)gnx_cdiv(rows, 256)), dim3(256), 0, h->stream, feat, rows, (int)K,
                        d, perm, code, h->d_flag);
     GNX_LAUNCH_CHECK();
   }
   return GNX_OK;
-}
-
-__global__ void k_graph_ptr(const int64_t* __restrict__ batch, int64_t N, int64_t B, int* __restrict__ ptr,
-                            int* __restrict__ flag) {
-  int64_t n = (int64_t)blockIdx.x * blockDim.x + threadIdx.x;
-  if (n > N) return;
-  int64_t prev = (n == 0) ? -1 : batch[n - 1];
-  int64_t cur = (n == N) ? B : batch[n];
-  if (n < N && (cur < 0 || cur >= B)) {
-    atomicOr(flag, 4);
-    return;
-  }
-  if (cur < prev) {
-    atomicOr(flag, 8);
-    return;
-  }
-  for (int64_t g = prev + 1; g <= cur; ++g) ptr[g] = (int)n;
 }
 
 extern "C" int32_t gnx_graph_ptr(gnx_handle* h, const int64_t* batch, int64_t N, int64_t B, int32_t* graph_ptr,
@@ -255,8 +359,8 @@
   (void)ws;
   (void)ws_bytes;
   GNX_CHECK_ARG(h && graph_ptr && N >= 0 && B >= 0 && (batch || N == 0), "gnx_graph_ptr: bad argument");
-  hipLaunchKernelGGL(k_graph_ptr, dim3((unsigned)gnx_cdiv(N + 1, 256)), dim3(256), 0, h->stream, batch, N, B,
-                     graph_ptr, h->d_flag);
+  hipLaunchKernelGGL(k_sort_groups, dim3((unsigned)gnx_cdiv(N + 1, 256)), dim3(256), 0, h->stream, (const int*)nullptr, N,
+                     (int*)nullptr, batch, B, graph_ptr, h->d_flag);
   GNX_LAUNCH_CHECK();
   return GNX_OK;
 }
@@ -419,6 +523,7 @@
 
 #define DC_BLOCK 256
 #define DC_MAX_CLASSES 64
+#define DC_FOLD_TILES 64
 
 __global__ void __launch_bounds__(DC_BLOCK) k_dc_hist(const int* __restrict__ rowptr, const int* __restrict__ keys,
                                                        int64_t N, int D, int nblocks, int* __restrict__ blockhist,
@@ -442,9 +547,11 @@
 
 __global__ void __launch_bounds__(DC_BLOCK) k_dc_fill(const int* __restrict__ rowptr, const int* __restrict__ keys,
                                                        int64_t N, int D, int nblocks,
-                                                       const int* __restrict__ blockoff, int* __restrict__ dperm,
+                                                       const int* __restrict__ blockoff,
+                                                       const int* __restrict__ tile_sums, int* __restrict__ dperm,
                                                        int* __restrict__ cls_ptr) {
   __shared__ int degs[DC_BLOCK];
+  __shared__ int coff[DC_MAX_CLASSES];
   int64_t n = (int64_t)blockIdx.x * DC_BLOCK + threadIdx.x;
   int d = -1;
   if (n < N) {
@@ -453,14 +560,36 @@
     if (d >= D) d = D - 1;
   }
   degs[threadIdx.x] = d;
+  if ((int)threadIdx.x < D) {
+    const int64_t idx = (int64_t)threadIdx.x * nblocks + blockIdx.x;
+    int o = blockoff[idx];
+    if (tile_sums) {
+      const int tile = (int)(idx / SCAN_TILE);
+#pragma unroll 8
+      for (int i = 0; i < tile; ++i) o += tile_sums[i];
+    }
+    coff[threadIdx.x] = o;
+  }
   __syncthreads();
   if (n < N) {
     int rank = 0;
     for (int t = 0; t < (int)threadIdx.x; ++t) rank += (degs[t] == d) ? 1 : 0;
-    dperm[blockoff[d * nblocks + blockIdx.x] + rank] = (int)n;
-  }
-  if (blockIdx.x == 0 && (int)threadIdx.x <= D)
-    cls_ptr[threadIdx.x] = ((int)threadIdx.x == D) ? (int)N : blockoff[threadIdx.x * nblocks];
+    dperm[coff[d] + rank] = (int)n;
+  }
+  if (blockIdx.x == 0 && (int)threadIdx.x <= D) cls_ptr[threadIdx.x] = ((int)threadIdx.x == D) ? (int)N : coff[threadIdx.x];
+}
+
+static int32_t scan_for_dc_fill(gnx_handle* h, const int* in, int* out, int64_t n, int* ws, const int** tile_sums) {
+  if (scan_tiles(n) > DC_FOLD_TILES) {
+    *tile_sums = nullptr;
+    return exclusive_scan(h, in, out, n, ws, false);
+  }
+  scan_jobs a = {};
+  a.in[0] = in, a.out[0] = out, a.sums[0] = ws, a.n[0] = n, a.total[0] = 0;
+  hipLaunchKernelGGL(k_scan_tile, dim3((unsigned)scan_tiles(n), 1), dim3(SCAN_BLOCK), 0, h->stream, a);
+  GNX_LAUNCH_CHECK();
+  *tile_sums = ws;
+  return GNX_OK;
 }
 
 extern "C" size_t gnx_degree_classes_workspace_bytes(int64_t N, int32_t D) {
@@ -485,10 +614,11 @@
   hipLaunchKernelGGL(k_dc_hist, dim3(nblocks), dim3(DC_BLOCK), 0, h->stream, rowptr, (const int*)nullptr, N, (int)D,
                      nblocks, blockhist, h->d_flag);
   GNX_LAUNCH_CHECK();
-  int32_t st = exclusive_scan(h, blockhist, blockoff, (int64_t)D * nblocks, scan_ws, false);
+  const int* tile_sums = nullptr;
+  int32_t st = scan_for_dc_fill(h, blockhist, blockoff, (int64_t)D * nblocks, scan_ws, &tile_sums);
   if (st != GNX_OK) return st;
   hipLaunchKernelGGL(k_dc_fill, dim3(nblocks), dim3(DC_BLOCK), 0, h->stream, rowptr, (const int*)nullptr, N, (int)D,
-                     nblocks, blockoff, dperm, cls_ptr);
+                     nblocks, blockoff, tile_sums, dperm, cls_ptr);
   GNX_LAUNCH_CHECK();
   return GNX_OK;
 }
@@ -508,19 +638,28 @@
   hipLaunchKernelGGL(k_dc_hist, dim3(nblocks), dim3(DC_BLOCK), 0, h->stream, (const int*)nullptr, keys, E, (int)R,
                      nblocks, blockhist, h->d_flag);
   GNX_LAUNCH_CHECK();
-  int32_t st = exclusive_scan(h, blockhist, blockoff, (int64_t)R * nblocks, scan_ws, false);
+  const int* tile_sums = nullptr;
+  int32_t st = scan_for_dc_fill(h, blockhist, blockoff, (int64_t)R * nblocks, scan_ws, &tile_sums);
   if (st != GNX_OK) return st;
   hipLaunchKernelGGL(k_dc_fill, dim3(nblocks), dim3(DC_BLOCK), 0, h->stream, (const int*)nullptr, keys, E, (int)R,
-                     nblocks, blockoff, pos, ptr);
-  GNX_LAUNCH_CHECK();
-  return GNX_OK;
-}
-
-__global__ void __launch_bounds__(256) k_class_tiles(const int* __restrict__ cls_ptr, int D, int tile_rows,
-                                                     int* __restrict__ tile_info, int* __restrict__ ntiles) {
+                     nblocks, blockoff, tile_sums, pos, ptr);
+  GNX_LAUNCH_CHECK();
+  return GNX_OK;
+}
+
+#define CLASS_TILE_TABLES 4
+struct class_tiles_args {
+  int tile_rows[CLASS_TILE_TABLES];
+  int* tile_info[CLASS_TILE_TABLES];
+  int* ntiles[CLASS_TILE_TABLES];
+};
+
+__global__ void __launch_bounds__(256) k_class_tiles(const int* __restrict__ cls_ptr, int D, class_tiles_args a) {
+  const int tile_rows = a.tile_rows[blockIdx.y];
+  int* __restrict__ tile_info = a.tile_info[blockIdx.y];
   int total = 0;
   for (int c = 0; c < D; ++c) total += (cls_ptr[c + 1] - cls_ptr[c] + tile_rows - 1) / tile_rows;
-  if (blockIdx.x == 0 && threadIdx.x == 0) ntiles[0] = total;
+  if (blockIdx.x == 0 && threadIdx.x == 0) a.ntiles[blockIdx.y][0] = total;
   for (int t = blockIdx.x * blockDim.x + threadIdx.x; t < total; t += gridDim.x * blockDim.x) {
     int first = 0, c = 0;
     for (; c < D; ++c) {
@@ -536,10 +675,24 @@
   }
 }
 
+extern "C" int32_t gnx_class_tiles_multi(gnx_handle* h, const int32_t* cls_ptr, int32_t D, int32_t n,
+                                         const int32_t* tile_rows, int32_t* const* tile_info, int32_t* const* ntiles) {
+  GNX_CHECK_ARG(h && cls_ptr && tile_rows && tile_info && ntiles && D >= 1 && n >= 1 && n <= CLASS_TILE_TABLES,
+                "gnx_class_tiles_multi: bad argument (1 to %d tables)", CLASS_TILE_TABLES);
+  class_tiles_args a = {};
+  for (int i = 0; i < n; ++i) {
+    GNX_CHECK_ARG(tile_rows[i] > 0 && tile_info[i] && ntiles[i], "gnx_class_tiles_multi: bad table %d", i);
+    a.tile_rows[i] = tile_rows[i];
+    a.tile_info[i] = tile_info[i];
+    a.ntiles[i] = ntiles[i];
+  }
+  hipLaunchKernelGGL(k_class_tiles, dim3(16, (unsigned)n), dim3(256), 0, h->stream, cls_ptr, (int)D, a);
+  GNX_LAUNCH_CHECK();
+  return GNX_OK;
+}
+
 extern "C" int32_t gnx_class_tiles(gnx_handle* h, const int32_t* cls_ptr, int32_t D, int32_t tile_rows,
                                    int32_t* tile_info, int32_t* ntiles) {
   GNX_CHECK_ARG(h && cls_ptr && tile_info && ntiles && D >= 1 && tile_rows > 0, "gnx_class_tiles: bad argument");
-  hipLaunchKernelGGL(k_class_tiles, dim3(16), dim3(256), 0, h->stream, cls_ptr, (int)D, (int)tile_rows, tile_info, ntiles);
-  GNX_LAUNCH_CHECK();
-  return GNX_OK;
-}
+  return gnx_class_tiles_multi(h, cls_ptr, D, 1, &tile_rows, &tile_info, &ntiles);
+}
diff --git a/gnnepcsaft_amd/functional.py b/gnnepcsaft_amd/functional.py
--- a/gnnepcsaft_amd/functional.py
+++ b/gnnepcsaft_amd/functional.py
@@ -446,7 +446,7 @@
     etiles = pack.edge_tiles(D - 1) if (_FUSED_EDGE and pre_layers == 2) else None
     a.etile_info, a.etile_w = (etiles[0].data_ptr(), etiles[1]) if etiles is not None else (None, 0)
     ops.check(lib.gnx_pna_conv_fwd(_lib.handle(dev), C.byref(a)))
-    amp, att = pack.degree_scalers(avg_deg_log)
+    amp = att = None
     ctx.pack, ctx.cfg = pack, cfg[:5]
     ctx.n_h, ctx.n_z = len(hs), len(zs)
     ctx.sinks = grad_sinks(params)
@@ -576,7 +576,7 @@
             h = hn
             hs.append(h)
         A = ops.pna_aggregate_fwd(h, pack, T, F)
-        amp, att = pack.degree_scalers(avg_deg_log)
+        amp, att = pack.degree_scalers(avg_deg_log) if dc is None else (None, None)
         z = _empty(N, H, x)
         for t in range(T):
             Wp, bp = post[t][0]
diff --git a/gnnepcsaft_amd/ops.py b/gnnepcsaft_amd/ops.py
--- a/gnnepcsaft_amd/ops.py
+++ b/gnnepcsaft_amd/ops.py
@@ -149,19 +149,18 @@
         dc.chunks = torch.empty(3 * dc.max_chunks, **i32)
         dc.ntiles = torch.empty(1, **i32)
         dc.nchunks = torch.empty(1, **i32)
-        check(lib.gnx_class_tiles(h, dc.cls_ptr.data_ptr(), dc.D, DegreeClasses.GEMM_ROWS, dc.tiles.data_ptr(),
-                                  dc.ntiles.data_ptr()))
-        check(lib.gnx_class_tiles(h, dc.cls_ptr.data_ptr(), dc.D, DegreeClasses.WGRAD_ROWS, dc.chunks.data_ptr(),
-                                  dc.nchunks.data_ptr()))
         dc.tile_rows_p = int(lib.gnx_gemm_tile_rows(h, g.N, 128))
+        tables = [(DegreeClasses.GEMM_ROWS, dc.tiles, dc.ntiles), (DegreeClasses.WGRAD_ROWS, dc.chunks, dc.nchunks)]
         if dc.tile_rows_p == DegreeClasses.GEMM_ROWS:
             dc.tiles_p, dc.ntiles_p, dc.max_tiles_p = dc.tiles, dc.ntiles, dc.max_tiles
         else:
             dc.max_tiles_p = g.N // dc.tile_rows_p + dc.D
             dc.tiles_p = torch.empty(3 * dc.max_tiles_p, **i32)
             dc.ntiles_p = torch.empty(1, **i32)
-            check(lib.gnx_class_tiles(h, dc.cls_ptr.data_ptr(), dc.D, dc.tile_rows_p, dc.tiles_p.data_ptr(),
-                                      dc.ntiles_p.data_ptr()))
+            tables.append((dc.tile_rows_p, dc.tiles_p, dc.ntiles_p))
+        check(lib.gnx_class_tiles_multi(h, dc.cls_ptr.data_ptr(), dc.D, len(tables), _carr([r for r, _, _ in tables]),
+                                        (C.c_void_p * len(tables))(*[t.data_ptr() for _, t, _ in tables]),
+                                        (C.c_void_p * len(tables))(*[n.data_ptr() for _, _, n in tables])))
         return dc
 
 
@@ -192,40 +191,41 @@
     g.N, g.E, g.device, g._scalers, g._classes, g._code_index = N, E, dev, {}, None, None
     g._edge_tiles = None
     g.max_degree_hint = None
+    if edge_attr is not None:
+        if edge_attr.dtype != torch.int64 or edge_attr.dim() != 2 or edge_attr.size(0) != E or \
+                edge_attr.size(1) != len(bond_dims):
+            raise _lib.GnxError(_lib.GNX_E_INVALID, f"edge_attr must be int64[E,{len(bond_dims)}], got "
+                                                    f"{edge_attr.dtype} {tuple(edge_attr.shape)}")
+        edge_attr = edge_attr.contiguous()
+    if batch is not None:
+        if batch.dtype != torch.int64 or batch.dim() != 1 or batch.size(0) != N:
+            raise _lib.GnxError(_lib.GNX_E_INVALID, f"batch must be int64[N], got {batch.dtype} {tuple(batch.shape)}")
+        if num_graphs is None:
+            num_graphs = int(batch.max()) + 1 if N > 0 else 0
+        batch = batch.contiguous()
+        g.B = int(num_graphs)
+        g.has_batch = True
+        g.graph_ptr = torch.empty(g.B + 1, **i32)
+    else:
+        g.B = 1
+        g.has_batch = False
+        g.graph_ptr = torch.arange(2, **i32) * N
     g.rowptr = torch.empty(N + 1, **i32)
     g.colptr = torch.empty(N + 1, **i32)
     g.perm = torch.empty(E, **i32)
     g.src = torch.empty(E, **i32)
     g.dst = torch.empty(E, **i32)
     g.cpos = torch.empty(E, **i32)
+    g.code = torch.empty(E, **i32)
     ws_bytes = lib.gnx_pack_csr_workspace_bytes(N, E)
     ws = torch.empty(ws_bytes, dtype=torch.uint8, device=dev)
-    check(lib.gnx_pack_csr(h, edge_index.data_ptr(), E, N, g.rowptr.data_ptr(), g.perm.data_ptr(), g.src.data_ptr(),
-                           g.dst.data_ptr(), g.colptr.data_ptr(), g.cpos.data_ptr(), ws.data_ptr(), ws_bytes))
-    g.code = torch.empty(E, **i32)
-    if edge_attr is not None:
-        if edge_attr.dtype != torch.int64 or edge_attr.dim() != 2 or edge_attr.size(0) != E or \
-                edge_attr.size(1) != len(bond_dims):
-            raise _lib.GnxError(_lib.GNX_E_INVALID, f"edge_attr must be int64[E,{len(bond_dims)}], got "
-                                                    f"{edge_attr.dtype} {tuple(edge_attr.shape)}")
-        edge_attr = edge_attr.contiguous()
-        check(lib.gnx_feature_code(h, edge_attr.data_ptr(), E, len(bond_dims), _carr(list(bond_dims)),
-                                   g.perm.data_ptr(), g.code.data_ptr(), None, 0))
-    else:
+    check(lib.gnx_pack_graph(h, edge_index.data_ptr(), E, N, _ptr(edge_attr), len(bond_dims),
+                             _carr(list(bond_dims)) if edge_attr is not None else None,
+                             _ptr(batch), g.B, g.rowptr.data_ptr(), g.perm.data_ptr(), g.src.data_ptr(),
+                             g.dst.data_ptr(), g.colptr.data_ptr(), g.cpos.data_ptr(), g.code.data_ptr(),
+                             g.graph_ptr.data_ptr() if batch is not None else None, ws.data_ptr(), ws_bytes))
+    if edge_attr is None:
         g.code.zero_()
-    if batch is not None:
-        if batch.dtype != torch.int64 or batch.dim() != 1 or batch.size(0) != N:
-            raise _lib.GnxError(_lib.GNX_E_INVALID, f"batch must be int64[N], got {batch.dtype} {tuple(batch.shape)}")
-        if num_graphs is None:
-            num_graphs = int(batch.max()) + 1 if N > 0 else 0
-        g.B = int(num_graphs)
-        g.has_batch = True
-        g.graph_ptr = torch.empty(g.B + 1, **i32)
-        check(lib.gnx_graph_ptr(h, batch.contiguous().data_ptr(), N, g.B, g.graph_ptr.data_ptr(), None, 0))
-    else:
-        g.B = 1
-        g.has_batch = False
-        g.graph_ptr = torch.arange(2, **i32) * N
     if validate:
         check_range(dev)
     return g
diff --git a/include/gnx.h b/include/gnx.h
--- a/include/gnx.h
+++ b/include/gnx.h
@@ -77,6 +77,10 @@
 size_t gnx_pack_csr_workspace_bytes(int64_t N, int64_t E);
 int32_t gnx_pack_csr(gnx_handle* h, const int64_t* edge_index, int64_t E, int64_t N, int32_t* rowptr, int32_t* perm,
                      int32_t* src, int32_t* dst, int32_t* colptr, int32_t* cpos, void* ws, size_t ws_bytes);
+int32_t gnx_pack_graph(gnx_handle* h, const int64_t* edge_index, int64_t E, int64_t N, const int64_t* feat, int32_t K,
+                       const int32_t* dims, const int64_t* batch, int64_t B, int32_t* rowptr, int32_t* perm,
+                       int32_t* src, int32_t* dst, int32_t* colptr, int32_t* cpos, int32_t* code, int32_t* graph_ptr,
+                       void* ws, size_t ws_bytes);
 int32_t gnx_feature_code(gnx_handle* h, const int64_t* feat, int64_t rows, int32_t K, const int32_t* dims,
                          const int32_t* perm, int32_t* code, void* ws, size_t ws_bytes);
 int32_t gnx_graph_ptr(gnx_handle* h, const int64_t* batch, int64_t N, int64_t B, int32_t* graph_ptr, void* ws,
@@ -159,6 +163,8 @@
                            int32_t* cls_ptr, void* ws, size_t ws_bytes);
 int32_t gnx_class_tiles(gnx_handle* h, const int32_t* cls_ptr, int32_t D, int32_t tile_rows, int32_t* tile_info,
                         int32_t* ntiles);
+int32_t gnx_class_tiles_multi(gnx_handle* h, const int32_t* cls_ptr, int32_t D, int32_t n, const int32_t* tile_rows,
+                              int32_t* const* tile_info, int32_t* const* ntiles);
 int32_t gnx_gemm_grouped(gnx_handle* h, int32_t nseg, const gnx_gemm_seg* segs, const int64_t* cls_strides,
                          int32_t num_classes, int64_t M, int32_t N, const float* bias, const float* mask,
                          int64_t ldmask, float* C, int64_t ldc, int32_t flags, const int32_t* row_index,
```

Result: faster. 631,600 graphs/s (median of 4 runs) (+1.3%).
